# polarsignals/frostdb

Measured on AMD Instinct MI355X. Metric: rows/sec filter+group-by on 1B-row Prometheus Arrow (HBM-resident); achieved HBM GB/s vs peak, higher is better.
Workload: dtype f64; 1 GPU; headline: Prometheus schema, labels.code=='200' + SUM(value) GROUP BY labels.path; total_rows=1000000000, rows_per_gpu=1000000000, records_per_gpu=40, groups=1025, parallelism=1 GPU

## Files before the change

### frostdb_amd/csrc/fdb_capi.cpp

```cpp
#include <cstring>
#include <new>
#include <string>
#include <vector>

#include "fdb_codec.h"
#include "fdb_comm.h"
#include "fdb_context.h"
#include "fdb_dynamic.h"
#include "fdb_jit.h"
#include "fdb_mergepath.h"
#include "fdb_mergerec.h"
#include "fdb_plan.h"
#include "fdb_pqwrite_host.h"
#include "fdb_regex.h"
#include "fdb_sort.h"
#include "fdb_sortkey.h"
#include "fdb_take.h"

struct fdb_plan {
  std::unique_ptr<fdb::DynamicAggs> dyn;
  fdb_plan_desc main_desc;
  fdb::Plan plan;
  fdb_plan(const fdb_plan_desc* d, int dev)
      : dyn(fdb::DynamicAggs::wanted(d) ? new fdb::DynamicAggs(d, dev) : nullptr),
        main_desc(dyn ? dyn->main_desc() : (d ? *d : fdb_plan_desc())),
        plan(d ? &main_desc : nullptr, dev) {}
  explicit fdb_plan(const fdb::Plan& proto) : main_desc(), plan(proto, fdb::Plan::CloneTag()) {}
};
struct fdb_comm { std::unique_ptr<fdb::Comm> c; };
struct fdb_batch { std::unique_ptr<fdb::DeviceBatch> b; };
struct fdb_osync { fdb::OrderedSync s; fdb_osync(int32_t inputs, const fdb_order_col* order, int32_t n_order) : s(inputs, order, n_order) {} };
struct fdb_sampler { fdb::Sampler s; fdb_sampler(int64_t size, uint64_t seed, int device) : s(size, seed, device) {} };

namespace {
thread_local std::string g_last_error;

template <typename F>
int guard(fdb_plan* p, F&& f) {
  try {
    f();
    return FDB_OK;
  } catch (const fdb::Error& e) {
    if (p) p->plan.error = e.what(); else g_last_error = e.what();
    return e.code;
  } catch (const std::bad_alloc&) {
    if (p) p->plan.error = "out of host memory"; else g_last_error = "out of host memory";
    return FDB_ERR_OOM;
  } catch (const std::exception& e) {
    if (p) p->plan.error = e.what(); else g_last_error = e.what();
    return FDB_ERR_INVALID;
  } catch (...) {
    if (p) p->plan.error = "unknown error"; else g_last_error = "unknown error";
    return FDB_ERR_INVALID;
  }
}
void single_table_only(const fdb_plan* p) {
  if (p->dyn) throw fdb::Error(FDB_ERR_UNSUPPORTED, "not available for a plan with aggregations over a dynamic column set (merge such plans with fdb_plan_merge)");
}
}

namespace {
template <typename F>
int comm_guard(fdb_comm* c, F&& f) {
  try {
    f();
    return FDB_OK;
  } catch (const fdb::Error& e) {
    if (c && c->c) c->c->error = e.what();
    g_last_error = e.what();
    return e.code;
  } catch (const std::bad_alloc&) {
    g_last_error = "out of host memory";
    return FDB_ERR_OOM;
  } catch (const std::exception& e) {
    if (c && c->c) c->c->error = e.what();
    g_last_error = e.what();
    return FDB_ERR_INVALID;
  }
}
int wrap_all(std::vector<std::unique_ptr<fdb::Comm>>&& v, fdb_comm** out) {
  for (size_t i = 0; i < v.size(); i++) { out[i] = new fdb_comm(); out[i]->c = std::move(v[i]); }
  return FDB_OK;
}
}

namespace fdb { void widen_indices(const void* src, int width, uint32_t* dst, size_t n); void widen_indices_mapped(const void* src, int width, const uint32_t* table, size_t table_len, uint32_t* dst, size_t n); }

extern "C" {

const char* fdb_version(void) { return "frostdb_amd 0.1.0 (gfx950)"; }
const char* fdb_last_error(void) { return g_last_error.c_str(); }

int fdb_device_count(int* n_devices) {
  return guard(nullptr, [&] {
    int n = 0;
    hipError_t e = hipGetDeviceCount(&n);
    if (e != hipSuccess) { n = 0; (void)hipGetLastError(); }
    *n_devices = n;
  });
}

int fdb_plan_explain(const fdb_plan_desc* desc, char* buf, int64_t capacity, int64_t* needed) {
  return guard(nullptr, [&] {
    std::string s;
    if (fdb::DynamicAggs::wanted(desc)) {
      fdb::DynamicAggs dyn(desc, 0);
      const fdb_plan_desc md = dyn.main_desc();
      fdb::Plan plan(&md, 0, true);
      s = dyn.draw(plan);
    } else {
      fdb::Plan plan(desc, 0, true);
      s = plan.draw();
    }
    if (needed != nullptr) *needed = (int64_t)s.size() + 1;
    if (buf != nullptr && capacity > 0) {
      const size_t n = std::min((size_t)capacity - 1, s.size());
      std::memcpy(buf, s.data(), n);
      buf[n] = 0;
    }
  });
}

int fdb_selftest_widen(const void* src, int32_t width, uint32_t* dst, int64_t n) {
  return guard(nullptr, [&] {
    if ((width != 1 && width != 2 && width != 4 && width != -2 && width != -4 && width != -12 && width != -14) || n < 0 || ((src == nullptr || dst == nullptr) && n > 0))
      throw fdb::Error(FDB_ERR_INVALID, "widen: width 1, 2, 4 (bytes) or -2, -4 (bits) and non-null buffers");
    if (width == -12 || width == -14) {
      uint32_t table[16];
      for (uint32_t r = 0; r < 16; r++) table[r] = 3 * r + 5;
      fdb::widen_indices_mapped(src, width + 10, table, width == -12 ? 4 : 16, dst, (size_t)n);
      return;
    }
    fdb::widen_indices(src, width, dst, (size_t)n);
  });
}

int fdb_selftest_exact_sum(const double* x, int64_t n, double* out) {
  return guard(nullptr, [&] {
    if (n < 0 || out == nullptr || (n > 0 && x == nullptr)) throw fdb::Error(FDB_ERR_INVALID, "exact sum: n >= 0 and non-null buffers");
    long long limbs[FDB_EXACT_LIMBS] = {0};
    unsigned long long flags = 0;
    int64_t since = 0;
    for (int64_t i = 0; i < n; i++) {
      unsigned long long bits;
      std::memcpy(&bits, x + i, 8);
      int k; long long d0, d1, d2;
      const unsigned long long f = fdb_exact_split(bits, &k, &d0, &d1, &d2);
      if (f != 0ull) { flags |= f; continue; }
      limbs[k] += d0; limbs[k + 1] += d1; limbs[k + 2] += d2;
      if (++since == ((int64_t)1 << 30)) { fdb_exact_normalize(limbs); since = 0; }
    }
    const unsigned long long r = fdb_exact_round(limbs, flags);
    std::memcpy(out, &r, 8);
  });
}

int fdb_arrow_roundtrip(struct ArrowArray* batch, struct ArrowSchema* schema, struct ArrowArray* out, struct ArrowSchema* out_schema) {
  return guard(nullptr, [&] {
    if (out == nullptr || out_schema == nullptr) throw fdb::Error(FDB_ERR_INVALID, "null output");
    fdb::HostRecordView view;
    fdb::view_record(batch, schema, &view);
    fdb::roundtrip_record(view, out, out_schema);
  });
}

int fdb_read_ceiling(int device, int64_t bytes, int32_t reps, double* gb_per_s) {
  return guard(nullptr, [&] {
    if (gb_per_s == nullptr || bytes < (1 << 20) || reps < 1) throw fdb::Error(FDB_ERR_INVALID, "fdb_read_ceiling: bytes >= 1 MiB, reps >= 1");
    *gb_per_s = 0;
    bytes &= ~(int64_t)4095;
    if (hipSetDevice(device) != hipSuccess) throw fdb::Error(FDB_ERR_DEVICE, "hipSetDevice failed");
    void* buf = nullptr;
    unsigned long long* out = nullptr;
    hipEvent_t e0 = nullptr, e1 = nullptr;
    auto cleanup = [&] { if (buf) (void)hipFree(buf); if (out) (void)hipFree(out); if (e0) (void)hipEventDestroy(e0); if (e1) (void)hipEventDestroy(e1); };
    auto ck = [&](hipError_t e, const char* what) { if (e != hipSuccess) { cleanup(); throw fdb::Error(e == hipErrorOutOfMemory ? FDB_ERR_OOM : FDB_ERR_DEVICE, std::string(what) + ": " + hipGetErrorString(e)); } };
    ck(hipMalloc(&buf, (size_t)bytes), "hipMalloc");
    ck(hipMalloc((void**)&out, 64), "hipMalloc");
    ck(hipMemset(buf, 0, (size_t)bytes), "hipMemset");
    ck(hipEventCreate(&e0), "hipEventCreate");
    ck(hipEventCreate(&e1), "hipEventCreate");
    ck(fdb_launch_stream_read(buf, bytes, out, nullptr), "launch");
    float best = 0;
    for (int r = 0; r < reps; r++) {
      ck(hipEventRecord(e0, nullptr), "hipEventRecord");
      ck(fdb_launch_stream_read(buf, bytes, out, nullptr), "launch");
      ck(hipEventRecord(e1, nullptr), "hipEventRecord");
      ck(hipEventSynchronize(e1), "hipEventSynchronize");
      float ms = 0;
      ck(hipEventElapsedTime(&ms, e0, e1), "hipEventElapsedTime");
      if (ms > 0 && (best == 0 || ms < best)) best = ms;
    }
    cleanup();
    if (best > 0) *gb_per_s = (double)bytes / (best * 1e-3) / 1e9;
  });
}

int fdb_plan_create(const fdb_plan_desc* desc, int device, fdb_plan** out) {
  return guard(nullptr, [&] {
    if (out == nullptr) throw fdb::Error(FDB_ERR_INVALID, "null out pointer");
    if (desc != nullptr && desc->ordered != 0 && fdb::DynamicAggs::wanted(desc))
      throw fdb::Error(FDB_ERR_UNSUPPORTED, "OrderedAggregate over a dynamic column set is not supported");
    *out = new fdb_plan(desc, device);
  });
}

int fdb_plan_push(fdb_plan* plan, struct ArrowArray* batch, struct ArrowSchema* schema) {
  if (!plan) return FDB_ERR_INVALID;
  return guard(plan, [&] { if (plan->dyn) plan->dyn->push(plan->plan, batch, schema); else plan->plan.push(batch, schema); });
}

int fdb_plan_push_many(fdb_plan* plan, struct ArrowArray* const* batches, struct ArrowSchema* const* schemas, int32_t n, int32_t* n_pushed) {
  if (n_pushed) *n_pushed = 0;
  if (!plan || n < 0 || (n > 0 && (!batches || !schemas))) return FDB_ERR_INVALID;
  for (int32_t i = 0; i < n; i++) {
    const int rc = fdb_plan_push(plan, batches[i], schemas[i]);
// ... 785 lines not shown
```

### frostdb_amd/csrc/fdb_jit.cpp

```cpp
#include <hip/hip_runtime_api.h>
#include <hip/hiprtc.h>
#include <sys/stat.h>
#include <unistd.h>

#include <algorithm>
#include <chrono>
#include <atomic>
#include <cstdio>
#include <cstdlib>
#include <cstring>
#include <fstream>
#include <condition_variable>
#include <functional>
#include <memory>
#include <mutex>
#include <thread>
#include <sstream>
#include <string>
#include <unordered_map>
#include <vector>

#include "fdb_jit.h"
#include "../../include/frostdb_amd.h"

// ... 2 lines not shown
namespace {

const char* kKernelsHeader =
#include "fdb_kernels_h.inc"
    ;

const char* kPreamble = R"HIP(
typedef uint32_t u32x4 __attribute__((ext_vector_type(4)));
typedef unsigned long long u64x2 __attribute__((ext_vector_type(2)));
typedef uint32_t u32x2 __attribute__((ext_vector_type(2)));
#define G1 __attribute__((address_space(1)))
template <typename T> __device__ __forceinline__ const G1 T* as_global(const T* p) { return (const G1 T*)p; }
__device__ __forceinline__ long long f64_to_ordered(double d) { long long b = __double_as_longlong(d); return b ^ ((b >> 63) & 0x7FFFFFFFFFFFFFFFLL); }
// (a NaN contributes the identity of MIN / MAX, −0.0 counts as +0.0: see f64_minmax_key in fdb_kernels.hip)
__device__ __forceinline__ long long f64_minmax_key(double d, bool is_min) {
  d += 0.0;
  const long long k = f64_to_ordered(d);
  return d != d ? (is_min ? 0x7FFFFFFFFFFFFFFFLL : (-0x7FFFFFFFFFFFFFFFLL - 1)) : k;
}
// (FDB_LD_TEMPORAL: the kernel reads its columns twice — wide run records — so the first pass must leave them in the L2)
#ifdef FDB_LD_TEMPORAL
__device__ __forceinline__ u32x4 ld4(const void* base, uint32_t byte_off) {
  return *as_global(reinterpret_cast<const u32x4*>(reinterpret_cast<const char*>(base) + byte_off));
}
__device__ __forceinline__ u64x2 ld8(const void* base, uint32_t byte_off) {
  return *as_global(reinterpret_cast<const u64x2*>(reinterpret_cast<const char*>(base) + byte_off));
}
// (narrow-index caches, fdb_record.h: a lane's four indices at 1 / 2 bytes each — one 4- / 8-byte load, contiguous across the wave)
__device__ __forceinline__ uint32_t ld1raw(const void* base, uint32_t byte_off) {
  return *as_global(reinterpret_cast<const uint32_t*>(reinterpret_cast<const char*>(base) + byte_off));
}
__device__ __forceinline__ u32x2 ld2raw(const void* base, uint32_t byte_off) {
  return *as_global(reinterpret_cast<const u32x2*>(reinterpret_cast<const char*>(base) + byte_off));
}
#else
__device__ __forceinline__ uint32_t ld1raw(const void* base, uint32_t byte_off) {
  return __builtin_nontemporal_load(as_global(reinterpret_cast<const uint32_t*>(reinterpret_cast<const char*>(base) + byte_off)));
}
__device__ __forceinline__ u32x2 ld2raw(const void* base, uint32_t byte_off) {
  return __builtin_nontemporal_load(as_global(reinterpret_cast<const u32x2*>(reinterpret_cast<const char*>(base) + byte_off)));
}
__device__ __forceinline__ u32x4 ld4(const void* base, uint32_t byte_off) {
  return __builtin_nontemporal_load(as_global(reinterpret_cast<const u32x4*>(reinterpret_cast<const char*>(base) + byte_off)));
}
__device__ __forceinline__ u64x2 ld8(const void* base, uint32_t byte_off) {
  return __builtin_nontemporal_load(as_global(reinterpret_cast<const u64x2*>(reinterpret_cast<const char*>(base) + byte_off)));
}
#endif
// … unpacked into the register form the rest of the kernel consumes
__device__ __forceinline__ u32x4 ld1x4(const void* base, uint32_t byte_off) {
  const uint32_t v = ld1raw(base, byte_off);
  u32x4 r; r.x = v & 0xFFu; r.y = (v >> 8) & 0xFFu; r.z = (v >> 16) & 0xFFu; r.w = v >> 24;
  return r;
}
__device__ __forceinline__ u32x4 ld2x4(const void* base, uint32_t byte_off) {
  const u32x2 v = ld2raw(base, byte_off);
  u32x4 r; r.x = v.x & 0xFFFFu; r.y = v.x >> 16; r.z = v.y & 0xFFFFu; r.w = v.y >> 16;
  return r;
}
__device__ __forceinline__ uint32_t ldv(const uint8_t* bm, uint32_t byte_off, uint32_t shift) { return (as_global(bm)[byte_off] >> shift) & 0xFu; }
// dictionary truth table in a 64-bit immediate: 4 rows → 4-bit mask (NULL rows look up entry `null_at`)
__device__ __forceinline__ uint32_t leaf_bits(u32x4 idx, uint32_t valid, unsigned long long bits, uint32_t null_at) {
  const uint32_t i0 = (valid & 1u) ? idx.x : null_at, i1 = (valid & 2u) ? idx.y : null_at, i2 = (valid & 4u) ? idx.z : null_at, i3 = (valid & 8u) ? idx.w : null_at;
  return (uint32_t)((bits >> i0) & 1ull) | ((uint32_t)((bits >> i1) & 1ull) << 1) | ((uint32_t)((bits >> i2) & 1ull) << 2) | ((uint32_t)((bits >> i3) & 1ull) << 3);
}
template <typename LUT>
__device__ __forceinline__ uint32_t leaf_lut(u32x4 idx, uint32_t valid, LUT lut, uint32_t null_at) {
  const uint32_t i0 = (valid & 1u) ? idx.x : null_at, i1 = (valid & 2u) ? idx.y : null_at, i2 = (valid & 4u) ? idx.z : null_at, i3 = (valid & 8u) ? idx.w : null_at;
  return (uint32_t)lut[i0] | ((uint32_t)lut[i1] << 1) | ((uint32_t)lut[i2] << 2) | ((uint32_t)lut[i3] << 3);
}
// pre-aggregate arithmetic (project.go:163-399): Go int64 semantics — wrap-around, quotient truncated toward zero,
// MinInt64 / -1 wraps; a division by zero yields NULL, whose raw slot reads 0.
__device__ __forceinline__ long long i64_add(long long a, long long b) { return (long long)((unsigned long long)a + (unsigned long long)b); }
__device__ __forceinline__ long long i64_sub(long long a, long long b) { return (long long)((unsigned long long)a - (unsigned long long)b); }
__device__ __forceinline__ long long i64_mul(long long a, long long b) { return (long long)((unsigned long long)a * (unsigned long long)b); }
__device__ __forceinline__ long long i64_div(long long a, long long b) { return b == 0 ? 0 : b == -1 ? (long long)(0ull - (unsigned long long)a) : a / b; }
__device__ __forceinline__ long long u64_div(long long a, long long b) { return b == 0 ? 0 : (long long)((unsigned long long)a / (unsigned long long)b); }  // DivUint64s (project.go:379-395)
__device__ __forceinline__ double f64_div(double a, double b) { return b == 0.0 ? 0.0 : a / b; }
template <int OP, typename T> __device__ __forceinline__ bool cmp1(T a, T b) {
  return OP == 1 ? a == b : OP == 2 ? a != b : OP == 3 ? a < b : OP == 4 ? a <= b : OP == 5 ? a > b : a >= b;
}
template <int OP, typename T> __device__ __forceinline__ uint32_t cmp4(T a, T b, T c, T d, T lit, uint32_t valid) {
  return ((uint32_t)cmp1<OP, T>(a, lit) | ((uint32_t)cmp1<OP, T>(b, lit) << 1) | ((uint32_t)cmp1<OP, T>(c, lit) << 2) | ((uint32_t)cmp1<OP, T>(d, lit) << 3)) & valid;
}
)HIP";

struct KernelEntry {
  std::mutex m;
  std::condition_variable cv;
  bool ready = false;
  hipFunction_t fn = nullptr;
};
std::mutex g_mu;
std::unordered_map<std::string, std::shared_ptr<KernelEntry>> g_cache;
bool g_disabled = false;

uint64_t fnv(const std::string& s) {
  uint64_t h = 1469598103934665603ull;
  for (unsigned char c : s) { h ^= c; h *= 1099511628211ull; }
  return h;
}

std::string cache_dir() {
  std::string d;
  if (const char* e = std::getenv("FDB_JIT_CACHE")) d = e;
  else if (const char* x = std::getenv("XDG_CACHE_HOME"); x != nullptr && *x) d = std::string(x) + "/frostdb_amd";
  else if (const char* h = std::getenv("HOME"); h != nullptr && *h) { ::mkdir((std::string(h) + "/.cache").c_str(), 0700); d = std::string(h) + "/.cache/frostdb_amd"; }
  else d = "/tmp/frostdb_amd_jit_" + std::to_string((long)getuid());
  if (d.empty()) return "";
  (void)::mkdir(d.c_str(), 0700);
  struct stat st;
  if (::lstat(d.c_str(), &st) != 0 || !S_ISDIR(st.st_mode) || st.st_uid != getuid() || (st.st_mode & 077) != 0) {
    static bool warned = false;
    if (!warned) { warned = true; std::fprintf(stderr, "[frostdb_amd] JIT disk cache disabled: %s is not a private directory of this user\n", d.c_str()); }
    return "";
  }
  return d;
}

bool compile(const std::string& src, std::vector<char>* code, std::string* log) {
  hiprtcProgram prog;
  const char* hdr_names[] = {"fdb_kernels.h"};
  const char* hdr_src[] = {kKernelsHeader};
  if (hiprtcCreateProgram(&prog, src.c_str(), "fdb_plan_kernel.hip", 1, hdr_src, hdr_names) != HIPRTC_SUCCESS) { *log = "hiprtcCreateProgram failed"; return false; }
  const char* opts[] = {"--offload-arch=gfx950", "-O3", "-std=c++17", "-munsafe-fp-atomics", "-DFDB_DEVICE_ONLY=1"};
  const hiprtcResult r = hiprtcCompileProgram(prog, 5, opts);
  size_t n = 0;
  hiprtcGetProgramLogSize(prog, &n);
  if (n > 1) { log->resize(n); hiprtcGetProgramLog(prog, &(*log)[0]); }
  if (r != HIPRTC_SUCCESS) { hiprtcDestroyProgram(&prog); return false; }
  size_t sz = 0;
  hiprtcGetCodeSize(prog, &sz);
  code->resize(sz);
  hiprtcGetCode(prog, code->data());
  hiprtcDestroyProgram(&prog);
  return true;
}

template <typename F, typename V>
std::string expr_valid(const std::vector<JitExprNode>& ex, int root, F col, V colvalid);
template <typename F, typename V>
std::string expr_value(const std::vector<JitExprNode>& ex, int ni, F col, V colvalid) {
  const JitExprNode& n = ex[(size_t)ni];
  const bool f = n.type == FDB_T_F64;
  if (n.kind == 0) return f ? ("__longlong_as_double((long long)" + col(ni) + ")") : ("(long long)" + col(ni));
  if (n.kind == 1) return f ? ("__longlong_as_double(K_elit" + std::to_string(ni) + ")") : ("K_elit" + std::to_string(ni));
  if (n.kind == 7) return "(long long)" + col(ni);
  if (n.kind == 4) return "(double)(" + expr_value(ex, n.left, col, colvalid) + ")";
  if (n.kind == 5) return "(" + colvalid(n.left) + " ? 0ll : 1ll)";
  if (n.kind == 6)
    return "((" + expr_value(ex, n.op, col, colvalid) + " != 0ll) ? " + expr_value(ex, n.left, col, colvalid) + " : " + expr_value(ex, n.right, col, colvalid) + ")";
  std::string a = expr_value(ex, n.left, col, colvalid), b = expr_value(ex, n.right, col, colvalid);
  if (n.kind == 3) {
    if (n.op == FDB_OP_AND || n.op == FDB_OP_OR) return "((" + a + (n.op == FDB_OP_AND ? " & " : " | ") + b + ") & 1ll)";
    if (ex[(size_t)n.left].type != ex[(size_t)n.right].type) { a = "(double)" + a; b = "(double)" + b; }
    const char* op = n.op == FDB_OP_EQ ? " == " : n.op == FDB_OP_NOT_EQ ? " != " : n.op == FDB_OP_LT ? " < " : n.op == FDB_OP_LT_EQ ? " <= " : n.op == FDB_OP_GT ? " > " : " >= ";
    return "((" + expr_valid(ex, n.left, col, colvalid) + " && " + expr_valid(ex, n.right, col, colvalid) + " && (" + a + op + b + ")) ? 1ll : 0ll)";
  }
  if (f) {
    if (n.op == FDB_OP_DIV) return "f64_div(" + a + ", " + b + ")";
    return "(" + a + (n.op == FDB_OP_ADD ? " + " : n.op == FDB_OP_SUB ? " - " : " * ") + b + ")";
  }
  return std::string(n.op == FDB_OP_ADD ? "i64_add(" : n.op == FDB_OP_SUB ? "i64_sub(" : n.op == FDB_OP_MUL ? "i64_mul(" : n.type == FDB_T_U64 ? "u64_div(" : "i64_div(") + a + ", " + b + ")";
}
template <typename F, typename V>
std::string expr_valid(const std::vector<JitExprNode>& ex, int root, F col, V colvalid) {
  const JitExprNode& n = ex[(size_t)root];
  if (n.kind == 0) return colvalid(root);
  if (n.kind == 2 && n.op == FDB_OP_DIV) {
    const std::string d = expr_value(ex, n.right, col, colvalid);
    return n.type == FDB_T_F64 ? ("(" + d + " != 0.0)") : ("(" + d + " != 0)");
  }
  return "true";
}
inline std::string expr_bits(const std::vector<JitExprNode>& ex, int root, const std::string& v) {
  if (ex[(size_t)root].type == FDB_T_BOOL) return "(unsigned long long)(" + v + " + 1ll)";
  return ex[(size_t)root].type == FDB_T_F64 ? ("(unsigned long long)__double_as_longlong(" + v + ")") : ("(unsigned long long)" + v);
}

struct Gen {
  std::ostringstream o;
  const JitShape& s;
  explicit Gen(const JitShape& sh) : s(sh) {}

  static std::string reg(bool wide, bool late, int slot) { return std::string(late ? "l" : "e") + (wide ? "8_" : "4_") + std::to_string(slot); }

  void loads(bool late) {
    const int n4 = late ? s.n_l4 : s.n_c4, n8 = late ? s.n_l8 : s.n_c8;
    for (int i = 0; i < n4; i++) {
      const JitSlot& c = late ? s.l4[i] : s.c4[i];
      const std::string r = reg(false, late, i);
      if (c.has_values && c.width == 1) o << "    const u32x4 " << r << " = ld1x4(P_" << r << "_v + tile_off1, lane_off1);\n";
      else if (c.has_values && c.width == 2) o << "    const u32x4 " << r << " = ld2x4(P_" << r << "_v + tile_off2, lane_off2);\n";
      else if (c.has_values) o << "    const u32x4 " << r << " = ld4(P_" << r << "_v + tile_off4, lane_off4);\n";
      mask(c, r);
    }
    for (int i = 0; i < n8; i++) {
      const JitSlot& c = late ? s.l8[i] : s.c8[i];
      const std::string r = reg(true, late, i);
      if (c.has_values) {
        o << "    const u64x2 " << r << "a = ld8(P_" << r << "_v + tile_off8, lane_off8);\n";
        o << "    const u64x2 " << r << "b = ld8(P_" << r << "_v + tile_off8, lane_off8 + 16u);\n";
      }
      mask(c, r);
    }
  }

  bool live_mask = false;
  void mask(const JitSlot& c, const std::string& r) {
    const char* all = live_mask ? "live" : "0xFu";
    const char* cut = live_mask ? " & live" : "";
    if (c.has_validity == 1) o << "    const uint32_t " << r << "_m = ldv(P_" << r << "_b + tile_offb, lane_offb, lane_shb)" << cut << ";\n";
    else if (c.has_validity == 2) o << "    const uint32_t " << r << "_m = P_" << r << "_b != nullptr ? ldv(P_" << r << "_b + tile_offb, lane_offb, lane_shb)" << cut << " : " << all << ";\n";
    else o << "    const uint32_t " << r << "_m = " << all << ";\n";
  }

  std::string leaf_expr(int l) { return leaf_expr_of(s.leaves[l], l, reg(s.leaves[l].wide, false, s.leaves[l].slot)); }

  static std::string leaf_expr_of(const JitLeaf& L, int l, const std::string& r) {
    const std::string li = std::to_string(l);
    std::ostringstream e;
    switch (L.kind) {
      case FDB_LEAF_CONST: e << "(K_op" << li << " ? 0xFu : 0u)"; break;
      case FDB_LEAF_VALIDITY: e << "(K_op" << li << " ? " << r << "_m : (~" << r << "_m & 0xFu))"; break;
      case FDB_LEAF_DICT_BITS: e << "leaf_bits(" << r << ", " << r << "_m, (unsigned long long)K_lit" << li << ", K_len" << li << " - 1u)"; break;
      case FDB_LEAF_DICT_LUT:
        if (L.lut_in_lds) e << "leaf_lut(" << r << ", " << r << "_m, smem + K_lds" << li << ", K_len" << li << " - 1u)";
        else e << "leaf_lut(" << r << ", " << r << "_m, as_global(K_lut" << li << "), K_len" << li << " - 1u)";
        break;
      case FDB_LEAF_CMP_I64:
        e << "cmp4<" << L.op << ", long long>((long long)" << r << "a.x, (long long)" << r << "a.y, (long long)" << r << "b.x, (long long)" << r << "b.y, K_lit" << li << ", " << r << "_m)";
        break;
      case FDB_LEAF_CMP_U64:
        e << "cmp4<" << L.op << ", unsigned long long>(" << r << "a.x, " << r << "a.y, " << r << "b.x, " << r << "b.y, (unsigned long long)K_lit" << li << ", " << r << "_m)";
        break;
      case FDB_LEAF_CMP_F64:
        e << "cmp4<" << L.op << ", double>(__longlong_as_double((long long)" << r << "a.x), __longlong_as_double((long long)" << r << "a.y), __longlong_as_double((long long)"
          << r << "b.x), __longlong_as_double((long long)" << r << "b.y), __longlong_as_double(K_lit" << li << "), " << r << "_m)";
        break;
      case FDB_LEAF_CMP_I64_F64:
        e << "cmp4<" << L.op << ", double>((double)(long long)" << r << "a.x, (double)(long long)" << r << "a.y, (double)(long long)" << r << "b.x, (double)(long long)" << r
          << "b.y, __longlong_as_double(K_lit" << li << "), " << r << "_m)";
        break;
    }
    return e.str();
  }

  std::string filter_expr() {
    return filter_expr_of(s.code, [&](int l) { return leaf_expr(l); });
  }
  template <typename F>
  static std::string filter_expr_of(const std::vector<uint8_t>& code, F leaf) {
    std::vector<std::string> st;
    for (uint8_t c : code) {
      if (c < 0x80) { st.push_back(leaf(c)); continue; }
      const std::string b = st.back(); st.pop_back();
      const std::string a = st.back(); st.pop_back();
      st.push_back("(" + a + (c == FDB_CODE_AND ? " & " : " | ") + b + ")");
    }
    return st.empty() ? "0xFu" : st.back();
  }

  std::string source() {
    const int BLK = s.block;
    o << "#include \"fdb_kernels.h\"\n" << kPreamble;
    o << "extern \"C\" __global__ __launch_bounds__(" << BLK << ") void fdb_plan_kernel(const FdbScanArgs* __restrict__ parts, const int n_parts, const long long total_tiles, const FdbScanArgs c) {\n";
    o << "  extern __shared__ __align__(16) unsigned char smem[];\n  const uint32_t tid = threadIdx.x;\n  const uint32_t n_slots = c.n_slots;\n";
    o << "  if (c.fill_state != nullptr)  // (a fresh table: its identity fill rides on this launch, see FdbScanArgs)\n";
    o << "    for (uint32_t i = blockIdx.x * " << BLK << "u + tid; i < c.fill_words; i += gridDim.x * " << BLK << "u) c.fill_state[i] = c.fill_idents[i / c.fill_alloc];\n";
    o << "  const size_t TB = (((size_t)n_slots * 4 + 15) & ~(size_t)15) + (size_t)n_slots * 8 * (size_t)c.n_aggs;\n  (void)TB;\n";
    const std::string tbl = s.wave_tables ? "smem + c.lds_lut_bytes + (size_t)(tid >> 6) * TB" : "smem + c.lds_lut_bytes";
    o << "  uint32_t* l_cnt = reinterpret_cast<uint32_t*>(" << tbl << ");\n";
    o << "  unsigned long long* l_acc = reinterpret_cast<unsigned long long*>(" << tbl << " + (((size_t)n_slots * 4 + 15) & ~(size_t)15));\n";
    if (s.lds_acc) {
      const std::string i0 = s.wave_tables ? "(tid & 63u)" : "tid", step = s.wave_tables ? "64" : std::to_string(BLK);
      o << "  for (uint32_t i = " << i0 << "; i < n_slots; i += " << step << ") l_cnt[i] = 0;\n";
      for (size_t j = 0; j < s.aggs.size(); j++) {
        const JitAgg& A = s.aggs[j];
        if (A.func == FDB_AGG_COUNT) continue;
        const char* ident = A.func == FDB_AGG_MIN ? "0x7FFFFFFFFFFFFFFFull" : A.func == FDB_AGG_MAX ? "0x8000000000000000ull" : "0ull";
        o << "  for (uint32_t i = " << i0 << "; i < n_slots; i += " << step << ") l_acc[(size_t)" << j << " * n_slots + i] = " << ident << ";\n";
      }
    }
    if (s.cache) {
      o << "  const uint32_t CS = (uint32_t)c.cache_slots;\n";
      o << "  uint32_t* t_tag = reinterpret_cast<uint32_t*>(smem + c.lds_lut_bytes);\n  uint32_t* t_cnt = t_tag + CS;\n";
      o << "  unsigned long long* t_acc = reinterpret_cast<unsigned long long*>(t_cnt + CS);\n";
      o << "  for (uint32_t i = tid; i < CS; i += " << BLK << ") { t_tag[i] = 0u; t_cnt[i] = 0u; }\n";
      for (size_t j = 0; j < s.aggs.size(); j++) {
        const JitAgg& A = s.aggs[j];
        if (A.func == FDB_AGG_COUNT) continue;
        const char* ident = A.func == FDB_AGG_MIN ? "0x7FFFFFFFFFFFFFFFull" : A.func == FDB_AGG_MAX ? "0x8000000000000000ull" : "0ull";
        o << "  for (uint32_t i = tid; i < CS; i += " << BLK << ") t_acc[(size_t)" << j << " * CS + i] = " << ident << ";\n";
      }
    }
    auto decl_slots = [&](bool late) {
      const int n4 = late ? s.n_l4 : s.n_c4, n8 = late ? s.n_l8 : s.n_c8;
      for (int i = 0; i < n4; i++) o << "  const char* P_" << reg(false, late, i) << "_v = nullptr; const uint8_t* P_" << reg(false, late, i) << "_b = nullptr;\n";
      for (int i = 0; i < n8; i++) o << "  const char* P_" << reg(true, late, i) << "_v = nullptr; const uint8_t* P_" << reg(true, late, i) << "_b = nullptr;\n";
    };
    decl_slots(false); decl_slots(true);
    for (size_t l = 0; l < s.leaves.size(); l++)
      o << "  long long K_lit" << l << " = 0; uint32_t K_len" << l << " = 1, K_lds" << l << " = 0; int K_op" << l << " = 0; const uint8_t* K_lut" << l << " = nullptr;\n";
    for (size_t g = 0; g < s.gcols.size(); g++) o << "  uint32_t G_lds" << g << " = 0, G_stride" << g << " = 0; const uint32_t* G_lut" << g << " = nullptr;\n";
    for (size_t i = 0; i < s.exprs.size(); i++) if (s.exprs[i].kind == 1) o << "  long long K_elit" << i << " = 0;\n";
    for (int t = 0; t < s.reg_slots; t++) {
      o << "  unsigned long long R_cnt" << t << " = 0ull;\n";
      for (size_t j = 0; j < s.aggs.size(); j++) {
        const JitAgg& A = s.aggs[j];
        if (A.func == FDB_AGG_COUNT) continue;
        if (A.func == FDB_AGG_SUM && A.type == FDB_T_F64) o << "  double R_a" << j << "_" << t << " = 0.0;\n";
        else if (A.func == FDB_AGG_SUM) o << "  unsigned long long R_a" << j << "_" << t << " = 0ull;\n";
        else o << "  long long R_a" << j << "_" << t << " = " << (A.func == FDB_AGG_MIN ? "0x7FFFFFFFFFFFFFFFLL" : "(-0x7FFFFFFFFFFFFFFFLL - 1)") << ";\n";
      }
    }
    o << "  long long n_rows = 0, tile_begin = 0, tile_end = 0; int part = -1, lut_class = -1;\n";
    o << "  const uint32_t lane_off4 = tid * 16u, lane_off8 = tid * 32u, lane_offb = tid >> 1, lane_shb = (tid & 1u) * 4u;\n";
    o << "  const uint32_t lane_off1 = tid * 4u, lane_off2 = tid * 8u; (void)lane_off1; (void)lane_off2;\n";
    o << "  for (long long tile = blockIdx.x; tile < total_tiles; tile += gridDim.x) {\n";
    o << "    if (part < 0 || tile >= tile_end) {\n      int np = part < 0 ? 0 : part;\n      while (np + 1 < n_parts && tile >= parts[np].tile_end) np++;\n      part = np;\n";
    o << "      const FdbScanArgs& pa = parts[part];\n      n_rows = pa.n_rows; tile_begin = pa.tile_begin; tile_end = pa.tile_end;\n";
    auto set_slots = [&](bool late) {
      const int n4 = late ? s.n_l4 : s.n_c4, n8 = late ? s.n_l8 : s.n_c8;
      const char* p4 = late ? "l4" : "c4"; const char* p8 = late ? "l8" : "c8";
      for (int i = 0; i < n4; i++)
        o << "      P_" << reg(false, late, i) << "_v = (const char*)pa." << p4 << "[" << i << "].values; P_" << reg(false, late, i) << "_b = pa." << p4 << "[" << i << "].validity;\n";
      for (int i = 0; i < n8; i++)
        o << "      P_" << reg(true, late, i) << "_v = (const char*)pa." << p8 << "[" << i << "].values; P_" << reg(true, late, i) << "_b = pa." << p8 << "[" << i << "].validity;\n";
    };
    set_slots(false); set_slots(true);
    for (size_t l = 0; l < s.leaves.size(); l++)
      o << "      K_lit" << l << " = pa.leaves[" << l << "].lit; K_len" << l << " = pa.leaves[" << l << "].lut_len; K_lds" << l << " = pa.leaves[" << l << "].lut_lds; K_op" << l
        << " = pa.leaves[" << l << "].op; K_lut" << l << " = pa.leaves[" << l << "].lut;\n";
    for (size_t g = 0; g < s.gcols.size(); g++)
      o << "      G_lds" << g << " = pa.gcols[" << g << "].lut_lds; G_stride" << g << " = pa.gcols[" << g << "].stride; G_lut" << g << " = pa.gcols[" << g << "].lut;\n";
    for (size_t i = 0; i < s.exprs.size(); i++) if (s.exprs[i].kind == 1) o << "      K_elit" << i << " = pa.expr[" << i << "].lit;\n";
    o << "      if (pa.lut_class != lut_class) {\n        lut_class = pa.lut_class;\n        __syncthreads();\n";
    for (size_t l = 0; l < s.leaves.size(); l++)
      if (s.leaves[l].kind == FDB_LEAF_DICT_LUT && s.leaves[l].lut_in_lds)
        o << "        for (uint32_t i = tid; i < K_len" << l << "; i += " << BLK << ") smem[K_lds" << l << " + i] = as_global(K_lut" << l << ")[i];\n";
    for (size_t g = 0; g < s.gcols.size(); g++)
      if (s.gcols[g].lut_in_lds)
        o << "        for (uint32_t i = tid; i < pa.gcols[" << g << "].lut_len; i += " << BLK << ") reinterpret_cast<uint32_t*>(smem + G_lds" << g << ")[i] = as_global(G_lut" << g << ")[i];\n";
    o << "        __syncthreads();\n      }\n    }\n";
    o << "    const long long r0 = (tile - tile_begin) * " << BLK * 4 << "LL;\n";
    o << "    const long long left = n_rows - r0 - (long long)tid * 4;\n    if (left <= 0) continue;\n";
    o << "    const size_t tile_off4 = (size_t)r0 * 4, tile_off8 = (size_t)r0 * 8, tile_offb = (size_t)(r0 >> 3);\n";
    o << "    const size_t tile_off1 = (size_t)r0, tile_off2 = (size_t)r0 * 2; (void)tile_off1; (void)tile_off2;\n";
    o << "    const uint32_t live = left >= 4 ? 0xFu : ((1u << (int)left) - 1u);\n";
    live_mask = true;
    loads(false);
    o << "    uint32_t sel = live;\n";
    if (!s.code.empty()) o << "    sel &= " << filter_expr() << ";\n";
    {
      std::vector<int> seen;
      for (const JitExprNode& e : s.exprs)
        if (e.kind == 7 && std::find(seen.begin(), seen.end(), e.slot) == seen.end()) { seen.push_back(e.slot); o << "    const uint32_t PM" << e.slot << " = " << leaf_expr(e.slot) << "; (void)PM" << e.slot << ";\n"; }
    }
    const bool uniform_fold = s.uniform_fold && s.lds_acc && !s.cache && s.reg_slots == 0 && !s.wave_tables && !s.two_phase && !s.gcols.empty();
    if (uniform_fold) o << "    const unsigned long long has = __ballot(sel != 0u);\n    if (has == 0ull) continue;\n";
    else o << "    if (sel == 0u) continue;\n";
    loads(true);
    o << "    uint32_t gid0 = 0, gid1 = 0, gid2 = 0, gid3 = 0;\n";
    for (size_t g = 0; g < s.gcols.size(); g++) {
      const JitGroup& G = s.gcols[g];
      const std::string r = reg(false, s.two_phase, G.slot);
      const std::string lut = G.lut_in_lds ? ("reinterpret_cast<const uint32_t*>(smem + G_lds" + std::to_string(g) + ")") : ("as_global(G_lut" + std::to_string(g) + ")");
      const char* comp[4] = {"x", "y", "z", "w"};
      for (int k = 0; k < 4; k++)
        o << "    gid" << k << " += ((" << r << "_m >> " << k << ") & 1u ? " << lut << "[" << r << "." << comp[k] << "] : 0u) * G_stride" << g << ";\n";
    }
    if (uniform_fold) {
      auto raw_of = [&](size_t j, int k) {
        const JitAgg& A = s.aggs[j];
        const std::string comp = std::string(k < 2 ? "a" : "b") + (k % 2 == 0 ? ".x" : ".y");
        if (A.expr != 0) {
          auto col = [&](int ni) -> std::string { if (s.exprs[(size_t)ni].kind == 7) return "((PM" + std::to_string(s.exprs[(size_t)ni].slot) + " >> " + std::to_string(k) + ") & 1u)"; return reg(true, s.two_phase, s.exprs[(size_t)ni].slot) + comp; };
          auto colvalid = [&](int ni) { return "((" + reg(true, s.two_phase, s.exprs[(size_t)ni].slot) + "_m >> " + std::to_string(k) + ") & 1u)"; };
          return "(" + expr_valid(s.exprs, A.expr - 1, col, colvalid) + " ? " + expr_bits(s.exprs, A.expr - 1, expr_value(s.exprs, A.expr - 1, col, colvalid)) + " : 0ull)";
        }
        const std::string r = reg(true, s.two_phase, A.slot);
        return "((" + r + "_m >> " + std::to_string(k) + ") & 1u ? " + r + comp + " : c.aggs[" + std::to_string(j) + "].null_value)";
      };
      o << "    {\n      const uint32_t my_first = (sel & 1u) ? gid0 : (sel & 2u) ? gid1 : (sel & 4u) ? gid2 : gid3;\n";
      o << "      const uint32_t g0 = (uint32_t)__builtin_amdgcn_readlane((int)my_first, __builtin_ctzll(has));\n";
      o << "      if (__ballot(sel != 0u && my_first != g0) == 0ull && __ballot(1) == ~0ull &&\n";
      o << "          __ballot(((sel & 1u) && gid0 != g0) || ((sel & 2u) && gid1 != g0) || ((sel & 4u) && gid2 != g0) || ((sel & 8u) && gid3 != g0)) == 0ull) {\n";
      o << "        uint32_t u_cnt = (uint32_t)__builtin_popcount(sel);\n";
      for (size_t j = 0; j < s.aggs.size(); j++) {
        const JitAgg& A = s.aggs[j];
        if (A.func == FDB_AGG_COUNT) continue;
        const std::string v = "u" + std::to_string(j);
        if (A.func == FDB_AGG_SUM && A.type == FDB_T_F64) {
          o << "        double " << v << " = 0.0;\n";
          for (int k = 0; k < 4; k++) o << "        if ((sel >> " << k << ") & 1u) " << v << " += __longlong_as_double((long long)" << raw_of(j, k) << ");\n";
        } else if (A.func == FDB_AGG_SUM) {
          o << "        unsigned long long " << v << " = 0ull;\n";
          for (int k = 0; k < 4; k++) o << "        if ((sel >> " << k << ") & 1u) " << v << " += " << raw_of(j, k) << ";\n";
        } else {
          o << "        long long " << v << " = " << (A.func == FDB_AGG_MIN ? "0x7FFFFFFFFFFFFFFFLL" : "(-0x7FFFFFFFFFFFFFFFLL - 1)") << ";\n";
          for (int k = 0; k < 4; k++) {
            const std::string key = A.type == FDB_T_F64 ? ("f64_minmax_key(__longlong_as_double((long long)" + raw_of(j, k) + "), " + (A.func == FDB_AGG_MIN ? "true" : "false") + ")") : ("(long long)" + raw_of(j, k));
            o << "        if ((sel >> " << k << ") & 1u) { const long long y = " << key << "; " << v << " = " << (A.func == FDB_AGG_MIN ? "y < " : "y > ") << v << " ? y : " << v << "; }\n";
          }
        }
      }
      o << "#pragma unroll\n        for (int sh = 32; sh > 0; sh >>= 1) {\n          u_cnt += (uint32_t)__shfl_xor((int)u_cnt, sh, 64);\n";
      for (size_t j = 0; j < s.aggs.size(); j++) {
        const JitAgg& A = s.aggs[j];
        if (A.func == FDB_AGG_COUNT) continue;
        const std::string v = "u" + std::to_string(j);
        if (A.func == FDB_AGG_SUM && A.type == FDB_T_F64) o << "          " << v << " += __shfl_xor(" << v << ", sh, 64);\n";
        else if (A.func == FDB_AGG_SUM) o << "          " << v << " += (unsigned long long)__shfl_xor((long long)" << v << ", sh, 64);\n";
        else o << "          { const long long y = __shfl_xor(" << v << ", sh, 64); " << v << " = " << (A.func == FDB_AGG_MIN ? "y < " : "y > ") << v << " ? y : " << v << "; }\n";
      }
      o << "        }\n        if ((tid & 63u) == 0u) {\n";
      if (s.need_count) o << "          atomicAdd(&l_cnt[g0], u_cnt);\n";
      else o << "          l_cnt[g0] = 1u;\n";
      for (size_t j = 0; j < s.aggs.size(); j++) {
        const JitAgg& A = s.aggs[j];
        if (A.func == FDB_AGG_COUNT) continue;
        const std::string v = "u" + std::to_string(j);
        const std::string acc = "(l_acc + (size_t)" + std::to_string(j) + " * n_slots + g0)";
        if (A.func == FDB_AGG_SUM && A.type == FDB_T_F64) o << "          atomicAdd(reinterpret_cast<double*>" << acc << ", " << v << ");\n";
        else if (A.func == FDB_AGG_SUM) o << "          atomicAdd(" << acc << ", " << v << ");\n";
        else o << "          " << (A.func == FDB_AGG_MIN ? "atomicMin" : "atomicMax") << "(reinterpret_cast<long long*>" << acc << ", " << v << ");\n";
      }
      o << "        }\n        continue;\n      }\n    }\n";
    }
    for (int k = 0; k < 4 && s.reg_slots > 0; k++) {
      const std::string comp = std::string(k < 2 ? "a" : "b") + (k % 2 == 0 ? ".x" : ".y");
      o << "    {\n      const bool on = (sel >> " << k << ") & 1u;\n";
      std::vector<std::string> val(s.aggs.size());
      for (size_t j = 0; j < s.aggs.size(); j++) {
        const JitAgg& A = s.aggs[j];
        if (A.func == FDB_AGG_COUNT) continue;
        std::string raw;
        if (A.expr != 0) {
          auto col = [&](int ni) -> std::string { if (s.exprs[(size_t)ni].kind == 7) return "((PM" + std::to_string(s.exprs[(size_t)ni].slot) + " >> " + std::to_string(k) + ") & 1u)"; return reg(true, s.two_phase, s.exprs[(size_t)ni].slot) + comp; };
          auto colvalid = [&](int ni) { return "((" + reg(true, s.two_phase, s.exprs[(size_t)ni].slot) + "_m >> " + std::to_string(k) + ") & 1u)"; };
          raw = "(" + expr_valid(s.exprs, A.expr - 1, col, colvalid) + " ? " + expr_bits(s.exprs, A.expr - 1, expr_value(s.exprs, A.expr - 1, col, colvalid)) + " : 0ull)";
        } else {
          const std::string r = reg(true, s.two_phase, A.slot);
          raw = "((" + r + "_m >> " + std::to_string(k) + ") & 1u ? " + r + comp + " : c.aggs[" + std::to_string(j) + "].null_value)";
        }
        const std::string v = "v" + std::to_string(j);
        if (A.func == FDB_AGG_SUM && A.type == FDB_T_F64) o << "      const double " << v << " = __longlong_as_double((long long)" << raw << ");\n";
        else if (A.func == FDB_AGG_SUM) o << "      const unsigned long long " << v << " = " << raw << ";\n";
        else o << "      const long long " << v << " = " << (A.type == FDB_T_F64 ? ("f64_minmax_key(__longlong_as_double((long long)" + raw + "), " + (A.func == FDB_AGG_MIN ? "true" : "false") + ")") : ("(long long)" + raw)) << ";\n";
        val[j] = v;
      }
      for (int t = 0; t < s.reg_slots; t++) {
        const std::string m = s.reg_slots == 1 ? std::string("on") : ("(on && gid" + std::to_string(k) + " == " + std::to_string(t) + "u)");
        o << "      R_cnt" << t << " += " << m << " ? 1ull : 0ull;\n";
        for (size_t j = 0; j < s.aggs.size(); j++) {
          const JitAgg& A = s.aggs[j];
          if (A.func == FDB_AGG_COUNT) continue;
          const std::string acc = "R_a" + std::to_string(j) + "_" + std::to_string(t);
          if (A.func == FDB_AGG_SUM && A.type == FDB_T_F64) o << "      " << acc << " += " << m << " ? " << val[j] << " : 0.0;\n";
          else if (A.func == FDB_AGG_SUM) o << "      " << acc << " += " << m << " ? " << val[j] << " : 0ull;\n";
          else if (A.func == FDB_AGG_MIN) o << "      " << acc << " = (" << m << " && " << val[j] << " < " << acc << ") ? " << val[j] << " : " << acc << ";\n";
          else o << "      " << acc << " = (" << m << " && " << val[j] << " > " << acc << ") ? " << val[j] << " : " << acc << ";\n";
        }
      }
      o << "    }\n";
    }
    for (int k = 0; k < 4 && s.reg_slots == 0; k++) {
      const std::string gidk = "gid" + std::to_string(k);
      o << "    if ((sel >> " << k << ") & 1u) {\n";
      if (s.cache) {
        o << "      const uint32_t ch = ((gid" << k << " * 0x9E3779B1u) >> 12) & (CS - 1u);\n";
        o << "      uint32_t tg = t_tag[ch];\n      if (tg == 0u) { tg = atomicCAS(&t_tag[ch], 0u, gid" << k << " + 1u); if (tg == 0u) tg = gid" << k << " + 1u; }\n";
        o << "      const bool cached = tg == gid" << k << " + 1u;\n";
        o << "      if (cached) atomicAdd(&t_cnt[ch], 1u);\n";
        if (s.need_count) o << "      else atomicAdd(&c.cnt[gid" << k << "], 1ull);\n";
        else o << "      else c.cnt[gid" << k << "] = 1ull;\n";
      } else if (s.lds_acc) {
        if (s.need_count) o << "      atomicAdd(&l_cnt[" << gidk << "], 1u);\n";
        else o << "      l_cnt[" << gidk << "] = 1u;\n";
      } else {
        o << "      atomicAdd(&c.cnt[gid" << k << "], 1ull);\n";
      }
      for (size_t j = 0; j < s.aggs.size(); j++) {
        const JitAgg& A = s.aggs[j];
        if (A.func == FDB_AGG_COUNT) continue;
        const std::string comp = std::string(k < 2 ? "a" : "b") + (k % 2 == 0 ? ".x" : ".y");
        std::string raw;
        if (A.expr != 0) {
          auto col = [&](int ni) -> std::string { if (s.exprs[(size_t)ni].kind == 7) return "((PM" + std::to_string(s.exprs[(size_t)ni].slot) + " >> " + std::to_string(k) + ") & 1u)"; return reg(true, s.two_phase, s.exprs[(size_t)ni].slot) + comp; };
          auto colvalid = [&](int ni) { return "((" + reg(true, s.two_phase, s.exprs[(size_t)ni].slot) + "_m >> " + std::to_string(k) + ") & 1u)"; };
          raw = "(" + expr_valid(s.exprs, A.expr - 1, col, colvalid) + " ? " + expr_bits(s.exprs, A.expr - 1, expr_value(s.exprs, A.expr - 1, col, colvalid)) + " : 0ull)";
        } else {
          const std::string r = reg(true, s.two_phase, A.slot);
          raw = "((" + r + "_m >> " + std::to_string(k) + ") & 1u ? " + r + comp + " : c.aggs[" + std::to_string(j) + "].null_value)";
        }
        const std::string gacc = "(c.aggs[" + std::to_string(j) + "].acc + gid" + std::to_string(k) + ")";
        const std::string acc = s.lds_acc ? ("(l_acc + (size_t)" + std::to_string(j) + " * n_slots + " + gidk + ")") : gacc;
        auto emit = [&](const std::string& where, const char* ind) {
          if (A.func == FDB_AGG_SUM) {
            if (A.type == FDB_T_F64) o << ind << "atomicAdd(reinterpret_cast<double*>" << where << ", __longlong_as_double((long long)" << raw << "));\n";
            else o << ind << "atomicAdd(" << where << ", " << raw << ");\n";
          } else {
            const std::string key = A.type == FDB_T_F64 ? ("f64_minmax_key(__longlong_as_double((long long)" + raw + "), " + (A.func == FDB_AGG_MIN ? "true" : "false") + ")") : ("(long long)" + raw);
            o << ind << (A.func == FDB_AGG_MIN ? "atomicMin" : "atomicMax") << "(reinterpret_cast<long long*>" << where << ", " << key << ");\n";
          }
        };
        if (s.cache) {
          o << "      if (cached) {\n";
          emit("(t_acc + (size_t)" + std::to_string(j) + " * CS + ch)", "        ");
          o << "      } else {\n";
          emit(gacc, "        ");
          o << "      }\n";
        } else {
          emit(acc, "      ");
        }
      }
      o << "    }\n";
    }
    o << "  }\n";
    if (s.reg_slots > 0) {
      o << "  for (int sh = 32; sh > 0; sh >>= 1) {\n";
      for (int t = 0; t < s.reg_slots; t++) {
        o << "    R_cnt" << t << " += (unsigned long long)__shfl_xor((long long)R_cnt" << t << ", sh, 64);\n";
        for (size_t j = 0; j < s.aggs.size(); j++) {
          const JitAgg& A = s.aggs[j];
          if (A.func == FDB_AGG_COUNT) continue;
          const std::string acc = "R_a" + std::to_string(j) + "_" + std::to_string(t);
          if (A.func == FDB_AGG_SUM && A.type == FDB_T_F64) o << "    " << acc << " += __shfl_xor(" << acc << ", sh, 64);\n";
          else if (A.func == FDB_AGG_SUM) o << "    " << acc << " += (unsigned long long)__shfl_xor((long long)" << acc << ", sh, 64);\n";
          else if (A.func == FDB_AGG_MIN) o << "    { const long long y = __shfl_xor(" << acc << ", sh, 64); " << acc << " = y < " << acc << " ? y : " << acc << "; }\n";
          else o << "    { const long long y = __shfl_xor(" << acc << ", sh, 64); " << acc << " = y > " << acc << " ? y : " << acc << "; }\n";
        }
      }
      o << "  }\n  if ((tid & 63u) == 0u) {\n";
      for (int t = 0; t < s.reg_slots; t++) {
        o << "    if (R_cnt" << t << " != 0ull) {\n";
        if (s.lds_acc) o << "      atomicAdd(&l_cnt[" << t << "], (uint32_t)(R_cnt" << t << " > 0xFFFFFFFFull ? 0xFFFFFFFFull : R_cnt" << t << "));\n";
        else o << "      atomicAdd(&c.cnt[" << t << "], R_cnt" << t << ");\n";
        for (size_t j = 0; j < s.aggs.size(); j++) {
          const JitAgg& A = s.aggs[j];
          if (A.func == FDB_AGG_COUNT) continue;
          const std::string v = "R_a" + std::to_string(j) + "_" + std::to_string(t);
          const std::string acc = s.lds_acc ? ("(l_acc + (size_t)" + std::to_string(j) + " * n_slots + " + std::to_string(t) + ")") : ("(c.aggs[" + std::to_string(j) + "].acc + " + std::to_string(t) + ")");
          if (A.func == FDB_AGG_SUM && A.type == FDB_T_F64) o << "      atomicAdd(reinterpret_cast<double*>" << acc << ", " << v << ");\n";
          else if (A.func == FDB_AGG_SUM) o << "      atomicAdd(" << acc << ", " << v << ");\n";
          else o << "      " << (A.func == FDB_AGG_MIN ? "atomicMin" : "atomicMax") << "(reinterpret_cast<long long*>" << acc << ", " << v << ");\n";
        }
        o << "    }\n";
      }
      o << "  }\n";
    }
    if (s.cache) {
      o << "  __syncthreads();\n  for (uint32_t i = tid; i < CS; i += " << BLK << ") {\n    const uint32_t tg = t_tag[i];\n    if (tg == 0u) continue;\n    const uint32_t g = tg - 1u;\n";
      if (s.need_count) o << "    atomicAdd(&c.cnt[g], (unsigned long long)t_cnt[i]);\n";
      else o << "    c.cnt[g] = 1ull;\n";
      for (size_t j = 0; j < s.aggs.size(); j++) {
        const JitAgg& A = s.aggs[j];
        if (A.func == FDB_AGG_COUNT) continue;
        const std::string v = "t_acc[(size_t)" + std::to_string(j) + " * CS + i]";
        const std::string dst = "c.aggs[" + std::to_string(j) + "].acc + g";
        if (A.func == FDB_AGG_SUM && A.type == FDB_T_F64) o << "    atomicAdd(reinterpret_cast<double*>(" << dst << "), __longlong_as_double((long long)" << v << "));\n";
        else if (A.func == FDB_AGG_SUM) o << "    atomicAdd(" << dst << ", " << v << ");\n";
        else o << "    " << (A.func == FDB_AGG_MIN ? "atomicMin" : "atomicMax") << "(reinterpret_cast<long long*>(" << dst << "), (long long)" << v << ");\n";
      }
      o << "  }\n";
    }
    if (s.lds_acc && s.wave_tables) {
      o << "  __syncthreads();\n  {\n    unsigned long long* out = c.partials + (size_t)blockIdx.x * (size_t)(1 + c.n_aggs) * n_slots;\n";
      o << "    const unsigned char* t0 = smem + c.lds_lut_bytes;\n";
      o << "    for (uint32_t i = tid; i < n_slots; i += " << BLK << ") {\n      unsigned long long n = 0;\n";
      o << "      for (int w = 0; w < " << BLK / 64 << "; w++) n += reinterpret_cast<const uint32_t*>(t0 + (size_t)w * TB)[i];\n      out[i] = n;\n";
      for (size_t j = 0; j < s.aggs.size(); j++) {
        const JitAgg& A = s.aggs[j];
        if (A.func == FDB_AGG_COUNT) continue;
        const std::string at = "reinterpret_cast<const unsigned long long*>(t0 + (size_t)w * TB + (((size_t)n_slots * 4 + 15) & ~(size_t)15))[(size_t)" + std::to_string(j) + " * n_slots + i]";
        if (A.func == FDB_AGG_SUM && A.type == FDB_T_F64) {
          o << "      { double v = 0.0; for (int w = 0; w < " << BLK / 64 << "; w++) v += __longlong_as_double((long long)" << at << "); out[(size_t)" << (1 + j) << " * n_slots + i] = (unsigned long long)__double_as_longlong(v); }\n";
        } else if (A.func == FDB_AGG_SUM) {
          o << "      { unsigned long long v = 0; for (int w = 0; w < " << BLK / 64 << "; w++) v += " << at << "; out[(size_t)" << (1 + j) << " * n_slots + i] = v; }\n";
        } else {
          o << "      { long long v = " << (A.func == FDB_AGG_MIN ? "0x7FFFFFFFFFFFFFFFLL" : "(-0x7FFFFFFFFFFFFFFFLL - 1)") << "; for (int w = 0; w < " << BLK / 64 << "; w++) { const long long y = (long long)" << at
            << "; v = " << (A.func == FDB_AGG_MIN ? "y < v" : "y > v") << " ? y : v; } out[(size_t)" << (1 + j) << " * n_slots + i] = (unsigned long long)v; }\n";
        }
      }
      o << "    }\n  }\n";
    } else if (s.lds_acc) {
      o << "  __syncthreads();\n";
      o << "  if (c.partials != nullptr) {\n    unsigned long long* out = c.partials + (size_t)blockIdx.x * (size_t)(1 + c.n_aggs) * n_slots;\n";
      o << "    for (uint32_t i = tid; i < n_slots; i += " << BLK << ") out[i] = (unsigned long long)l_cnt[i];\n";
      for (size_t j = 0; j < s.aggs.size(); j++)
        if (s.aggs[j].func != FDB_AGG_COUNT)
          o << "    for (uint32_t i = tid; i < n_slots; i += " << BLK << ") out[(size_t)" << (1 + j) << " * n_slots + i] = l_acc[(size_t)" << j << " * n_slots + i];\n";
      o << "  } else {\n    for (uint32_t i = tid; i < n_slots; i += " << BLK << ") {\n      const uint32_t n_sel = l_cnt[i];\n      if (n_sel == 0) continue;\n";
      o << "      atomicAdd(&c.cnt[i], (unsigned long long)n_sel);\n";
      for (size_t j = 0; j < s.aggs.size(); j++) {
        const JitAgg& A = s.aggs[j];
        if (A.func == FDB_AGG_COUNT) continue;
        const std::string v = "l_acc[(size_t)" + std::to_string(j) + " * n_slots + i]";
        const std::string dst = "c.aggs[" + std::to_string(j) + "].acc + i";
        if (A.func == FDB_AGG_SUM && A.type == FDB_T_F64) o << "      atomicAdd(reinterpret_cast<double*>(" << dst << "), __longlong_as_double((long long)" << v << "));\n";
// ... 719 lines not shown
      o << "        u32x4* stage = reinterpret_cast<u32x4*>(smem + a.lds_lut_bytes + (size_t)wv * " << FDB_RUN_WAVE_LDS << ");\n";
      o << "        const uint32_t n_act = (uint32_t)__popcll(act2), my_act = (uint32_t)__popcll(act2 & lt);\n";
      o << "        const bool sw = rp + n_w > " << FDB_RUN_CHUNK << "u;\n";
      o << "        if (sw || (rp - ps) + n_w > " << FDB_RUN_STAGE << "u) {\n";
      o << "          u32x4* out = reinterpret_cast<u32x4*>(h.runs.tuples) + (size_t)(rb + ps) * 3;\n";
      o << "          for (uint32_t q = my_act; q < (rp - ps) * 3u; q += n_act) out[q] = stage[q];\n";
      o << "          __builtin_amdgcn_wave_barrier();\n          ps = rp;\n        }\n";
      o << "        if (sw) {\n          uint32_t nc = 0u;\n          if (wl2 == first2) nc = atomicAdd(h.runs.chunk_cursor, 1u);\n          rb = (uint32_t)__shfl((int)nc, first2, 64) * " << FDB_RUN_CHUNK
        << "u; rp = 0u; ps = 0u;\n        }\n";
      o << "        const uint32_t base = rb + rp, sbase = rp - ps;\n        __builtin_amdgcn_wave_barrier();\n";
      o << "        if (wl2 == first2) { s_runs[wv * 4] = rb; s_runs[wv * 4 + 1] = rp + n_w; s_runs[wv * 4 + 2] = ps; *reinterpret_cast<uint2*>(h.runs.dir + ((size_t)tile * 4 + wv) * 2) = make_uint2(base, n_w); }\n";
      for (int k = 0; k < 4; k++) {
        o << "        if (sel & " << (1 << k) << "u) {\n          const uint32_t at = sbase + before + (uint32_t)__builtin_popcount(sel & " << ((1 << k) - 1) << "u);\n";
        o << "          stage[at * 3] = ta_" << k << "; stage[at * 3 + 1] = tb_" << k << ";\n";
        o << "          *reinterpret_cast<u64x2*>(stage + at * 3 + 2) = u64x2{cnt_" << k << ", "
          << (has_val ? (f64v ? "(unsigned long long)__double_as_longlong(v0_" + std::to_string(k) + ")" : "(unsigned long long)v0_" + std::to_string(k)) : std::string("0ull")) << "};\n        }\n";
      }
      o << "        __builtin_amdgcn_wave_barrier();\n      }\n    }\n    continue;\n";
    }
    for (int k = 0; k < 4; k++) o << "    uint64_t slot_" << k << " = h1_" << k << " & h.mask; unsigned long long p_" << k << " = 0, q_" << k << " = 0;\n";
    for (int k = 0; k < 4; k++)
      o << "    if ((sel >> " << k << ") & 1u) { const u64x2 pq = *as_global(reinterpret_cast<const u64x2*>(h.table + slot_" << k << " * (uint64_t)ew)); p_" << k << " = pq.x; q_" << k
        << " = pq.y; }\n";
    o << "    uint32_t ins_mask = 0;\n";
    for (int k = 0; k < 4; k++) o << "    unsigned long long c_" << k << " = ~0ull;\n";
    for (int k = 0; k < 4; k++)
      o << "    if (((sel >> " << k << ") & 1u) && p_" << k << " == 0ull) c_" << k << " = atomicCAS(h.table + slot_" << k << " * (uint64_t)ew, 0ull, h1_" << k << ");\n";
    for (int k = 0; k < 4; k++)
      o << "    if (c_" << k << " == 0ull) { __hip_atomic_store(h.table + slot_" << k << " * (uint64_t)ew + 1, h2_" << k << ", __ATOMIC_RELAXED, __HIP_MEMORY_SCOPE_AGENT); ins_mask |= " << (1 << k) << "u; }\n";
    for (int k = 0; k < 4; k++) {
      o << "    if ((sel >> " << k << ") & 1u) {\n";
      o << "      if (c_" << k << " != 0ull && !(p_" << k << " == h1_" << k << " && q_" << k << " == h2_" << k << ")) { bool ins; slot_" << k << " = hash_find_or_insert(h.table, h.mask, ew, h1_" << k << ", h2_" << k
        << ", ins); if (ins) ins_mask |= " << (1 << k) << "u; }\n";
      o << "      unsigned long long* e = h.table + slot_" << k << " * (uint64_t)ew;\n";
      if (s.need_count) o << "      atomicAdd(e + 2, cnt_" << k << ");\n";
      for (size_t j = 0; j < s.aggs.size(); j++) {
        const JitAgg& A = s.aggs[j];
        if (A.func == FDB_AGG_COUNT || exact_agg(j)) continue;
        const std::string v = "v" + std::to_string(j) + "_" + std::to_string(k);
        const std::string acc = "(e + " + std::to_string(3 + j) + ")";
        if (A.func == FDB_AGG_SUM && A.type == FDB_T_F64) o << "      atomicAdd(reinterpret_cast<double*>" << acc << ", " << v << ");\n";
        else if (A.func == FDB_AGG_SUM) o << "      atomicAdd(" << acc << ", " << v << ");\n";
        else o << "      " << (A.func == FDB_AGG_MIN ? "atomicMin" : "atomicMax") << "(reinterpret_cast<long long*>" << acc << ", " << v << ");\n";
      }
      o << "    }\n";
    }
    emit_tuple_stores(false);
    if (s.exact) {
      o << "    x_slot0 = slot_0; x_slot1 = slot_1; x_slot2 = slot_2; x_slot3 = slot_3; x_sel = sel;\n";
      o << "    } while (0);\n";
      for (size_t j = 0; j < s.aggs.size(); j++) {
        if (!exact_agg(j)) continue;
        o << "    {\n      unsigned long long* XL = a.aggs[" << j << "].acc;\n";
        for (int k = 0; k < 4; k++) o << "      fdb_exact_add_wave(XL, x_slot" << k << ", xv" << j << "_" << k << ", ((x_sel >> " << k << ") & 1u) != 0u);\n";
        o << "    }\n";
      }
    }
    o << "  }\n";
    if (wide || medium) {
      o << "  {  // the runs that still wait in the waves' stages\n    const int wv = (int)(tid >> 6), wl2 = (int)(tid & 63u);\n    __builtin_amdgcn_wave_barrier();\n";
      o << "    const uint32_t rb = s_runs[wv * 4], rp = s_runs[wv * 4 + 1], ps = s_runs[wv * 4 + 2], RQ = " << (medium ? std::to_string(FDB_RUN_MEDIUM_BYTES / 16) + "u" : std::string("(uint32_t)h.runs.run_words >> 2")) << ";\n";
      o << "    if (rp != " << FDB_RUN_CHUNK << "u || ps != " << FDB_RUN_CHUNK << "u) {\n";
      o << "      const u32x4* stage = reinterpret_cast<const u32x4*>(smem + a.lds_lut_bytes + (size_t)wv * " << FDB_RUN_WAVE_LDS << ");\n";
      o << "      u32x4* out = reinterpret_cast<u32x4*>(h.runs.tuples) + (size_t)(rb + ps) * RQ;\n";
      o << "      for (uint32_t q = (uint32_t)wl2; q < (rp - ps) * RQ; q += 64u) out[q] = stage[q];\n    }\n  }\n";
    }
    if (narrow) {
      o << "  {  // the runs that still wait in the waves' stages\n    const int wv = (int)(tid >> 6), wl2 = (int)(tid & 63u);\n    __builtin_amdgcn_wave_barrier();\n";
      o << "    const uint32_t rb = s_runs[wv * 4], rp = s_runs[wv * 4 + 1], ps = s_runs[wv * 4 + 2];\n";
      o << "    if (rp != " << FDB_RUN_CHUNK << "u || ps != " << FDB_RUN_CHUNK << "u) {\n";
      o << "      const u32x4* stage = reinterpret_cast<const u32x4*>(smem + a.lds_lut_bytes + (size_t)wv * " << FDB_RUN_WAVE_LDS << ");\n";
      o << "      u32x4* out = reinterpret_cast<u32x4*>(h.runs.tuples) + (size_t)(rb + ps) * 3;\n";
      o << "      for (uint32_t q = (uint32_t)wl2; q < (rp - ps) * 3u; q += 64u) out[q] = stage[q];\n    }\n  }\n";
    }
    o << "  __syncthreads();\n  if (tid == 0 && s_new != 0) atomicAdd(h.n_groups, (unsigned long long)s_new);\n}\n";
    return o.str();
  }
};

}

std::string JitShape::key(bool with_validity) const {
  std::ostringstream k;
  k << "b" << block << "l" << lds_acc << "c" << need_count << "t" << two_phase << "r" << reg_slots << "h" << cache << (wave_tables ? "w" : "") << (uniform_fold ? "u" : "") << "|";
  auto slots = [&](const JitSlot* p, int n) { for (int i = 0; i < n; i++) { k << (p[i].has_values ? 'v' : '-') << (with_validity ? p[i].has_validity : 0); if (p[i].width != 4) k << 'w' << p[i].width; } k << '|'; };
  slots(c4, n_c4); slots(c8, n_c8); slots(l4, n_l4); slots(l8, n_l8);
  for (const JitLeaf& L : leaves) k << L.kind << ',' << L.slot << ',' << L.wide << ',' << (L.kind >= FDB_LEAF_CMP_I64 && L.kind <= FDB_LEAF_CMP_I64_F64 ? L.op : 0) << ',' << L.lut_in_lds << ';';
  k << '|';
  for (uint8_t c : code) k << (int)c << ',';
  k << '|';
  for (const JitGroup& G : gcols) k << G.slot << ',' << G.lut_in_lds << ';';
  k << '|';
  for (const JitAgg& A : aggs) k << A.func << ',' << A.type << ',' << A.slot << ',' << A.expr << ';';
  k << '|';
  for (const JitExprNode& e : exprs) k << e.kind << ',' << e.op << ',' << e.left << ',' << e.right << ',' << e.slot << ',' << e.type << ';';
  return k.str();
}

std::string jit_source(const JitShape& shape) { return Gen(shape).source(); }

JitShape jit_shape(const FdbScanArgs& a, bool two_phase, int block) {
  JitShape s;
  s.block = block;
  s.lds_acc = a.lds_acc != 0;
  s.need_count = a.need_count != 0;
  s.two_phase = two_phase;
  s.n_c4 = a.n_c4; s.n_c8 = a.n_c8;
  s.n_l4 = two_phase ? a.n_l4 : 0; s.n_l8 = two_phase ? a.n_l8 : 0;
  auto slots = [](JitSlot* dst, const FdbColSlot* src, int n) {
    for (int i = 0; i < n; i++) { dst[i].has_values = src[i].values != nullptr; dst[i].has_validity = src[i].validity != nullptr ? 1 : 0; }
  };
  slots(s.c4, a.c4, s.n_c4); slots(s.c8, a.c8, s.n_c8); slots(s.l4, a.l4, s.n_l4); slots(s.l8, a.l8, s.n_l8);
  for (int i = 0; i < s.n_c4; i++) s.c4[i].width = a.w4[i] == 1 || a.w4[i] == 2 ? a.w4[i] : 4;
  for (int i = 0; i < s.n_l4; i++) s.l4[i].width = a.wl4[i] == 1 || a.wl4[i] == 2 ? a.wl4[i] : 4;
  for (int l = 0; l < a.n_leaves; l++) {
    const FdbLeaf& L = a.leaves[l];
    s.leaves.push_back({L.kind, L.slot, L.wide, L.op, L.kind == FDB_LEAF_DICT_LUT && L.lut_lds != FDB_NO_LDS});
  }
  s.code.assign(a.code, a.code + a.n_code);
  for (int g = 0; g < a.n_gcols; g++) s.gcols.push_back({a.gcols[g].slot, a.gcols[g].lut_lds != FDB_NO_LDS});
  for (int j = 0; j < a.n_aggs; j++) s.aggs.push_back({a.aggs[j].func, a.aggs[j].type, a.aggs[j].slot, a.aggs[j].expr});
  for (int i = 0; i < a.n_expr; i++) s.exprs.push_back({a.expr[i].kind, a.expr[i].op, a.expr[i].left, a.expr[i].right, a.expr[i].slot, a.expr[i].type});
  s.cache = !s.lds_acc && a.cache_slots > 0;
  return s;
}

bool jit_shape_merge(JitShape* into, const JitShape& other) {
  if (into->key(false) != other.key(false)) return false;
  auto slots = [](JitSlot* a, const JitSlot* b, int n) { for (int i = 0; i < n; i++) if (a[i].has_validity != b[i].has_validity) a[i].has_validity = 2; };
  slots(into->c4, other.c4, into->n_c4); slots(into->c8, other.c8, into->n_c8); slots(into->l4, other.l4, into->n_l4); slots(into->l8, other.l8, into->n_l8);
  return true;
}

bool jit_shape_merge_args(JitShape* into, const FdbScanArgs& a, const FdbScanArgs& b, bool two_phase) {
  if (a.lds_acc != b.lds_acc || a.need_count != b.need_count || a.n_c4 != b.n_c4 || a.n_c8 != b.n_c8) return false;
  if (two_phase && (a.n_l4 != b.n_l4 || a.n_l8 != b.n_l8)) return false;
  if ((a.lds_acc == 0 && a.cache_slots > 0) != (b.lds_acc == 0 && b.cache_slots > 0)) return false;
  auto values_same = [](const FdbColSlot* x, const FdbColSlot* y, int n) { for (int i = 0; i < n; i++) if ((x[i].values != nullptr) != (y[i].values != nullptr)) return false; return true; };
  if (!values_same(a.c4, b.c4, a.n_c4) || !values_same(a.c8, b.c8, a.n_c8)) return false;
  if (two_phase && (!values_same(a.l4, b.l4, a.n_l4) || !values_same(a.l8, b.l8, a.n_l8))) return false;
  if (std::memcmp(a.w4, b.w4, sizeof a.w4) != 0 || (two_phase && std::memcmp(a.wl4, b.wl4, sizeof a.wl4) != 0)) return false;
  if (a.n_leaves != b.n_leaves || a.n_code != b.n_code || a.n_gcols != b.n_gcols || a.n_aggs != b.n_aggs || a.n_expr != b.n_expr) return false;
  for (int l = 0; l < a.n_leaves; l++) {
    const FdbLeaf& x = a.leaves[l]; const FdbLeaf& y = b.leaves[l];
    if (x.kind != y.kind || x.slot != y.slot || x.wide != y.wide) return false;
    if (x.kind >= FDB_LEAF_CMP_I64 && x.kind <= FDB_LEAF_CMP_I64_F64 && x.op != y.op) return false;
    if ((x.kind == FDB_LEAF_DICT_LUT && x.lut_lds != FDB_NO_LDS) != (y.kind == FDB_LEAF_DICT_LUT && y.lut_lds != FDB_NO_LDS)) return false;
  }
  if (std::memcmp(a.code, b.code, (size_t)a.n_code) != 0) return false;
  for (int g = 0; g < a.n_gcols; g++)
    if (a.gcols[g].slot != b.gcols[g].slot || (a.gcols[g].lut_lds != FDB_NO_LDS) != (b.gcols[g].lut_lds != FDB_NO_LDS)) return false;
  for (int j = 0; j < a.n_aggs; j++)
    if (a.aggs[j].func != b.aggs[j].func || a.aggs[j].type != b.aggs[j].type || a.aggs[j].slot != b.aggs[j].slot || a.aggs[j].expr != b.aggs[j].expr) return false;
  for (int i = 0; i < a.n_expr; i++) {
    const auto& x = a.expr[i]; const auto& y = b.expr[i];
    if (x.kind != y.kind || x.op != y.op || x.left != y.left || x.right != y.right || x.slot != y.slot || x.type != y.type) return false;
  }
  auto merge = [](JitSlot* s, const FdbColSlot* y, int n) { for (int i = 0; i < n; i++) if (s[i].has_validity != (y[i].validity != nullptr ? 1 : 0)) s[i].has_validity = 2; };
  merge(into->c4, b.c4, into->n_c4); merge(into->c8, b.c8, into->n_c8); merge(into->l4, b.l4, into->n_l4); merge(into->l8, b.l8, into->n_l8);
  return true;
}

int jit_blocks_per_cu(hipFunction_t fn, int block, size_t lds_bytes) {
  int occ = 0;
  if (hipModuleOccupancyMaxActiveBlocksPerMultiprocessor(&occ, fn, block, lds_bytes) != hipSuccess || occ < 1) { (void)hipGetLastError(); occ = 1; }
  if (occ > 2048 / block) occ = 2048 / block;
  return occ;
}

namespace {
std::atomic<int64_t> g_stat_compiled{0}, g_stat_compile_us{0}, g_stat_disk_loads{0};

hipFunction_t build_kernel(KernelEntry* entry, const std::string& kernel_name_s, const std::string& src) {
  const char* kernel_name = kernel_name_s.c_str();
  struct Publish {
    KernelEntry* e; hipFunction_t fn = nullptr;
    ~Publish() { { std::lock_guard<std::mutex> lk(e->m); e->fn = fn; e->ready = true; } e->cv.notify_all(); }
  } publish{entry};
  std::vector<char> code;
  char name[64];
  std::snprintf(name, sizeof name, "/k_%016llx_%zu.hsaco", (unsigned long long)(fnv(src) ^ (fnv(kKernelsHeader) * 31)), src.size());
  const std::string dir = cache_dir();
  const std::string path = dir.empty() ? std::string() : dir + name;
  bool from_disk = false;
  if (!path.empty()) {
    std::ifstream f(path, std::ios::binary);
    if (f) code.assign(std::istreambuf_iterator<char>(f), std::istreambuf_iterator<char>());
    from_disk = !code.empty();
  }
  auto load = [&](hipFunction_t* fn) {
    hipModule_t mod = nullptr;
    *fn = nullptr;
    if (hipModuleLoadData(&mod, code.data()) == hipSuccess && hipModuleGetFunction(fn, mod, kernel_name) == hipSuccess) return true;
    (void)hipGetLastError();
    *fn = nullptr;
    return false;
  };
// ... 117 lines not shown
std::string jit_project_source(const JitShape& shape) { return Gen(shape).project_source(); }
hipFunction_t jit_project_get(const JitShape& shape) {
  std::string roots;
  for (int r : shape.proj_roots) roots += std::to_string(r) + ",";
  return get_kernel("project|" + shape.key() + "|r" + roots, "fdb_project_kernel", [&] { return jit_project_source(shape); });
}
hipError_t jit_project_launch(hipFunction_t fn, const FdbScanArgs* d_parts, int n_parts, int64_t total_tiles, int grid, size_t lds_bytes, const FdbProjectPart* d_outs,
                              unsigned long long* d_nulls, hipStream_t stream) {
  long long tt = total_tiles;
  void* args[] = {(void*)&d_parts, (void*)&n_parts, (void*)&tt, (void*)&d_outs, (void*)&d_nulls};
  return hipModuleLaunchKernel(fn, (unsigned)grid, 1, 1, 256u, 1, 1, (unsigned)lds_bytes, stream, args, nullptr);
}

void jit_stats(int64_t* n_compiled, double* compile_ms, int64_t* n_disk_loads) {
  if (n_compiled) *n_compiled = g_stat_compiled.load();
  if (compile_ms) *compile_ms = (double)g_stat_compile_us.load() / 1000.0;
  if (n_disk_loads) *n_disk_loads = g_stat_disk_loads.load();
}

JitDeferScope::JitDeferScope(bool may_defer) : prev_(t_may_defer) { t_may_defer = may_defer; }
JitDeferScope::~JitDeferScope() { t_may_defer = prev_; }

hipFunction_t jit_get(const JitShape& shape) {
  return get_kernel(shape.key(), "fdb_plan_kernel", [&] { return jit_source(shape); });
}

std::string JitHashShape::key() const {
  std::ostringstream k;
  k << "c" << need_count << (runs == 1 ? "R" : runs == 2 ? "W" : runs == 3 ? "M" : "") << (exact ? "X" : "") << "|";
  for (const JitHashCol& C : cols) k << C.kind << (C.has_validity ? 'n' : '-') << (C.lut_identity ? 'i' : C.lut_in_lds ? 'l' : 'g') << (C.kind == 2 ? std::to_string(C.expr_root) : std::string());
  k << '|';
  for (size_t l = 0; l < leaves.size(); l++) {
    const JitLeaf& L = leaves[l];
    k << L.kind << ',' << L.wide << ',' << (L.kind >= FDB_LEAF_CMP_I64 && L.kind <= FDB_LEAF_CMP_I64_F64 ? L.op : 0) << ',' << L.lut_in_lds << ',' << leaf_validity[l] << ';';
  }
  k << '|';
  for (uint8_t c : code) k << (int)c << ',';
  k << '|';
  for (size_t j = 0; j < aggs.size(); j++) k << aggs[j].func << ',' << aggs[j].type << ',' << agg_validity[j] << ',' << aggs[j].expr << ';';
  k << '|' << n_expr_cols << '|';
  for (const JitExprNode& e : exprs) k << e.kind << ',' << e.op << ',' << e.left << ',' << e.right << ',' << e.slot << ',' << e.type << ';';
  return k.str();
}

JitHashShape jit_hash_shape(const FdbHashArgs& h, const FdbHashCol* hcols) {
  JitHashShape s;
  const FdbScanArgs& a = h.base;
  for (int c = 0; c < h.n_hcols; c++)
    s.cols.push_back({hcols[c].kind, hcols[c].validity != nullptr, hcols[c].kind == 0 && hcols[c].lut_lds != FDB_NO_LDS, hcols[c].kind == 2 ? hcols[c].src_word : -1,
                      hcols[c].kind == 0 && hcols[c].lut == nullptr});
  for (int i = 0; i < a.n_expr; i++) s.exprs.push_back({a.expr[i].kind, a.expr[i].op, a.expr[i].left, a.expr[i].right, a.expr[i].slot, a.expr[i].type});
  s.n_expr_cols = a.n_l8;
  s.need_count = a.need_count != 0;
  s.runs = h.runs.tuples == nullptr ? 0 : h.runs.run_words == 0 ? 1 : h.runs.run_words == FDB_RUN_MEDIUM_WORDS ? 3 : 2;
  for (int l = 0; l < a.n_leaves; l++) {
    const FdbLeaf& L = a.leaves[l];
    const bool wide = L.kind >= FDB_LEAF_CMP_I64 && L.kind <= FDB_LEAF_CMP_I64_F64;
    s.leaves.push_back({L.kind, 0, wide ? 1 : 0, L.op, L.kind == FDB_LEAF_DICT_LUT && L.lut_lds != FDB_NO_LDS});
    s.leaf_validity.push_back(L.validity != nullptr);
  }
  s.code.assign(a.code, a.code + a.n_code);
  for (int j = 0; j < a.n_aggs; j++) {
    s.aggs.push_back({a.aggs[j].func, a.aggs[j].type, -1, a.aggs[j].expr});
    s.agg_validity.push_back(a.aggs[j].validity != nullptr);
    if (a.aggs[j].func == FDB_AGG_SUM && a.aggs[j].type == FDB_T_F64 && a.aggs[j].acc != nullptr) s.exact = true;
  }
  return s;
}

std::string jit_hash_source(const JitHashShape& shape) { return HashGen(shape).source(); }

hipFunction_t jit_hash_get(const JitHashShape& shape) {
  return get_kernel(shape.key(), "fdb_hash_kernel", [&] { return jit_hash_source(shape); });
}

hipError_t jit_hash_launch(hipFunction_t fn, const FdbHashArgs& args, int grid, size_t lds_bytes, hipStream_t stream) {
  void* kargs[] = {(void*)&args};
  return hipModuleLaunchKernel(fn, (unsigned)grid, 1, 1, 256, 1, 1, (unsigned)lds_bytes, stream, kargs, nullptr);
}

hipFunction_t jit_select(JitShape shape, size_t lds_bytes, int row_bytes, int* block_out, int* blocks_per_cu_out) {
  int waves = row_bytes > 0 ? (65536 / (64 * 4)) / row_bytes : 16;
  waves = std::max(8, std::min(32, waves));
  const int block = waves % 8 == 0 ? 512 : 256;
  shape.block = block;
  hipFunction_t fn = jit_get(shape);
  if (fn == nullptr) return nullptr;
  const int fit = jit_blocks_per_cu(fn, block, lds_bytes);
  *block_out = block;
  *blocks_per_cu_out = std::max(1, std::min(fit, (waves + block / 128) / (block / 64)));
  if (std::getenv("FDB_JIT_DEBUG"))
    std::fprintf(stderr, "[frostdb_amd] plan kernel %s: %d B/row, %zu B LDS -> %d-thread workgroups, %d per CU (%d fit)\n", shape.key().c_str(), row_bytes,
                 lds_bytes, block, *blocks_per_cu_out, fit);
  return fn;
}

hipError_t jit_launch(hipFunction_t fn, const FdbScanArgs* d_parts, int n_parts, int64_t total_tiles, const FdbScanArgs& common, int grid, int block,
                      size_t lds_bytes, hipStream_t stream) {
  long long tt = total_tiles;
  void* args[] = {(void*)&d_parts, (void*)&n_parts, (void*)&tt, (void*)&common};
  return hipModuleLaunchKernel(fn, (unsigned)grid, 1, 1, (unsigned)block, 1, 1, (unsigned)lds_bytes, stream, args, nullptr);
}

}
```

### frostdb_amd/csrc/fdb_jit.h

```cpp
#pragma once
#include <cstdlib>

#include <hip/hip_runtime_api.h>

#include <cstdint>
#include <string>
#include <vector>

#include "fdb_kernels.h"

namespace fdb {

struct JitSlot { bool has_values = false; int has_validity = 0; int width = 4; };
struct JitLeaf { int kind = 0, slot = -1, wide = 0, op = 0; bool lut_in_lds = false; };
struct JitGroup { int slot = -1; bool lut_in_lds = false; };
struct JitAgg { int func = 0, type = 0, slot = -1; int expr = 0; };
struct JitExprNode { int kind = 0, op = 0, left = -1, right = -1, slot = -1, type = 0; };

struct JitShape {
  int block = 512;
  bool lds_acc = true, need_count = false, two_phase = false;
  int n_c4 = 0, n_c8 = 0, n_l4 = 0, n_l8 = 0;
  JitSlot c4[FDB_ARG_C4], c8[FDB_ARG_C8], l4[FDB_ARG_L4], l8[FDB_ARG_L8];
  std::vector<JitLeaf> leaves;
  std::vector<uint8_t> code;
  std::vector<JitGroup> gcols;
  std::vector<JitAgg> aggs;
  std::vector<JitExprNode> exprs;
  int reg_slots = 0;
  bool cache = false;
  bool wave_tables = false;
  bool uniform_fold = true;
  int fuse4 = 0, fuse8 = 0;
  std::vector<int> proj_roots;
  std::string key(bool with_validity = true) const;
};

struct JitHashCol { int kind = 0; bool has_validity = false, lut_in_lds = false; int expr_root = -1; bool lut_identity = false; };
struct JitHashShape {
  std::vector<JitHashCol> cols;
  std::vector<JitLeaf> leaves;
  std::vector<bool> leaf_validity;
  std::vector<uint8_t> code;
  std::vector<JitAgg> aggs;
  std::vector<bool> agg_validity;
  std::vector<JitExprNode> exprs;
  int n_expr_cols = 0;
  bool need_count = true;
  int runs = 0;
  bool exact = false;
  std::string key() const;
};
JitHashShape jit_hash_shape(const FdbHashArgs& args, const FdbHashCol* hcols);
std::string jit_hash_source(const JitHashShape& shape);
hipFunction_t jit_hash_get(const JitHashShape& shape);
hipError_t jit_hash_launch(hipFunction_t fn, const FdbHashArgs& args, int grid, size_t lds_bytes, hipStream_t stream);

JitShape jit_shape(const FdbScanArgs& a, bool two_phase, int block);
bool jit_shape_merge(JitShape* into, const JitShape& other);
bool jit_shape_merge_args(JitShape* into, const FdbScanArgs& a, const FdbScanArgs& b, bool two_phase);
int jit_blocks_per_cu(hipFunction_t fn, int block, size_t lds_bytes);

void jit_stats(int64_t* n_compiled, double* compile_ms, int64_t* n_disk_loads);

std::string jit_flags_source(const JitShape& shape);
hipFunction_t jit_flags_get(const JitShape& shape);
hipError_t jit_flags_launch(hipFunction_t fn, const FdbScanArgs* d_parts, int n_parts, int64_t total_super_tiles, const FdbScanArgs& common, int grid, size_t lds_bytes,
                            uint32_t* masks, uint32_t* tile_counts, hipStream_t stream);

std::string jit_select_source(const JitShape& shape);
hipFunction_t jit_select_kernel_get(const JitShape& shape);
size_t jit_select_stage_bytes(const JitShape& shape);
int jit_select_block();
hipError_t jit_select_launch(hipFunction_t fn, const FdbScanArgs* d_parts, int n_parts, int64_t total_super_tiles, const FdbScanArgs& common, int grid, size_t lds_bytes,
                             uint32_t* masks, uint32_t* offsets, const FdbSelectArgs& sel, hipStream_t stream);

std::string jit_project_source(const JitShape& shape);
hipFunction_t jit_project_get(const JitShape& shape);
hipError_t jit_project_launch(hipFunction_t fn, const FdbScanArgs* d_parts, int n_parts, int64_t total_tiles, int grid, size_t lds_bytes, const FdbProjectPart* d_outs,
                              unsigned long long* d_nulls, hipStream_t stream);

std::string jit_source(const JitShape& shape);
class JitDeferScope {
 public:
  explicit JitDeferScope(bool may_defer);
  ~JitDeferScope();
  JitDeferScope(const JitDeferScope&) = delete;
  JitDeferScope& operator=(const JitDeferScope&) = delete;
 private:
  bool prev_;
};
hipFunction_t jit_get(const JitShape& shape);
hipFunction_t jit_select(JitShape shape, size_t lds_bytes, int row_bytes, int* block_out, int* blocks_per_cu_out);
hipError_t jit_launch(hipFunction_t fn, const FdbScanArgs* d_parts, int n_parts, int64_t total_tiles, const FdbScanArgs& common, int grid, int block,
                      size_t lds_bytes, hipStream_t stream);

}
```

### frostdb_amd/csrc/fdb_kernels.hip

```cpp
#include <hip/hip_runtime.h>

#define FDB_DEVICE_HELPERS 1
#include <cstdlib>
#include <cstring>

#include "fdb_kernels.h"

namespace {

constexpr int OP_EQ = 1, OP_NOT_EQ = 2, OP_LT = 3, OP_LT_EQ = 4, OP_GT = 5, OP_GT_EQ = 6;
constexpr int AGG_SUM = 1, AGG_MIN = 2, AGG_MAX = 3, AGG_COUNT = 4;

__device__ __forceinline__ long long f64_to_ordered(double d) {
  long long b = __double_as_longlong(d);
  return b ^ ((b >> 63) & 0x7FFFFFFFFFFFFFFFLL);
}
__device__ __forceinline__ long long f64_minmax_key(double d, bool is_min) {
  d += 0.0;
  const long long k = f64_to_ordered(d);
  return d != d ? (is_min ? FDB_I64_MAX : FDB_I64_MIN) : k;
}

typedef uint32_t u32x4 __attribute__((ext_vector_type(4)));
typedef unsigned long long u64x2 __attribute__((ext_vector_type(2)));

#define FDB_GLOBAL __attribute__((address_space(1)))
template <typename T>
__device__ __forceinline__ const FDB_GLOBAL T* as_global(const T* p) {
  return (const FDB_GLOBAL T*)p;
}

template <int R>
__device__ __forceinline__ void load_u32(const uint32_t* __restrict__ p, uint32_t (&v)[R]) {
  if (R == 1) { v[0] = __builtin_nontemporal_load(as_global(p)); return; }
#pragma unroll
  for (int j = 0; j < R / 4; j++) {
    const u32x4 q = __builtin_nontemporal_load(as_global(reinterpret_cast<const u32x4*>(p)) + j);
    v[4 * j + 0] = q.x; v[4 * j + 1] = q.y; v[4 * j + 2] = q.z; v[4 * j + 3] = q.w;
  }
}

template <int R>
__device__ __forceinline__ void load_u64(const unsigned long long* __restrict__ p, unsigned long long (&v)[R]) {
  if (R == 1) { v[0] = __builtin_nontemporal_load(as_global(p)); return; }
#pragma unroll
  for (int j = 0; j < R / 2; j++) {
    const u64x2 q = __builtin_nontemporal_load(as_global(reinterpret_cast<const u64x2*>(p)) + j);
    v[2 * j + 0] = q.x; v[2 * j + 1] = q.y;
  }
}

template <int R>
__device__ __forceinline__ uint32_t load_valid(const uint8_t* __restrict__ bm, int64_t row0) {
  const uint32_t b = as_global(bm)[row0 >> 3];
  if (R == 1) return (b >> (row0 & 7)) & 1u;
  if (R == 8) return b;
  return (b >> (row0 & 4)) & 0xFu;
}

template <int R, typename T>
__device__ __forceinline__ uint32_t cmp_mask(const T (&v)[R], T lit, int op) {
  uint32_t m = 0;
  switch (op) {
    case OP_EQ:
#pragma unroll
      for (int r = 0; r < R; r++) m |= (uint32_t)(v[r] == lit) << r;
      break;
    case OP_NOT_EQ:
#pragma unroll
      for (int r = 0; r < R; r++) m |= (uint32_t)(v[r] != lit) << r;
      break;
    case OP_LT:
#pragma unroll
      for (int r = 0; r < R; r++) m |= (uint32_t)(v[r] < lit) << r;
      break;
    case OP_LT_EQ:
#pragma unroll
      for (int r = 0; r < R; r++) m |= (uint32_t)(v[r] <= lit) << r;
      break;
    case OP_GT:
#pragma unroll
      for (int r = 0; r < R; r++) m |= (uint32_t)(v[r] > lit) << r;
      break;
    case OP_GT_EQ:
#pragma unroll
      for (int r = 0; r < R; r++) m |= (uint32_t)(v[r] >= lit) << r;
      break;
    default: break;
  }
// ... 1894 lines not shown
  return hipGetLastError();
}

namespace {
typedef void (*SlotKernel)(const FdbScanArgs*, int, int64_t, FdbScanArgs);
struct SlotVariant { SlotKernel lds, nolds; int block; };
#define FDB_SV(NC4, NC8, L4, L8, BLK) {scan_slots_kernel<true, NC4, NC8, L4, L8, BLK>, scan_slots_kernel<false, NC4, NC8, L4, L8, BLK>, BLK}
const SlotVariant kSingle[] = {FDB_SV(2, 1, 0, 0, 512), FDB_SV(2, 1, 0, 0, 256), FDB_SV(2, 1, 0, 0, 1024)};
const SlotVariant kTwoPhase[] = {FDB_SV(FDB_MAX_C4, FDB_MAX_C8, FDB_MAX_L4, FDB_MAX_L8, 512), FDB_SV(FDB_MAX_C4, FDB_MAX_C8, FDB_MAX_L4, FDB_MAX_L8, 256),
                                  FDB_SV(FDB_MAX_C4, FDB_MAX_C8, FDB_MAX_L4, FDB_MAX_L8, 1024)};
#undef FDB_SV
const SlotVariant& slot_variant(int two_phase, int mode) {
  const int m = (mode >= 1 && mode <= 3) ? mode - 1 : 0;
  return two_phase ? kTwoPhase[m] : kSingle[m];
}
}

int fdb_slot_geometry(int two_phase, int mode, int lds_acc, size_t lds_bytes, int device, int* tile_rows, int* blocks_per_cu) {
  const SlotVariant& v = slot_variant(two_phase, mode);
  *tile_rows = v.block * 4;
  const void* fn = reinterpret_cast<const void*>(lds_acc ? v.lds : v.nolds);
  (void)hipFuncSetAttribute(fn, hipFuncAttributeMaxDynamicSharedMemorySize, 160 * 1024);
  int occ = 0;
  if (hipOccupancyMaxActiveBlocksPerMultiprocessor(&occ, fn, v.block, lds_bytes) != hipSuccess || occ < 1) { (void)hipGetLastError(); occ = 1; }
  if (occ > 2048 / v.block) occ = 2048 / v.block;
  *blocks_per_cu = occ;
  return 0;
}

hipError_t fdb_launch_scan_slots(const FdbScanArgs* d_parts, int n_parts, const FdbScanArgs& common, int64_t total_tiles, int grid_blocks,
                                 size_t lds_bytes, int two_phase, int mode, hipStream_t stream) {
  if (total_tiles <= 0 || grid_blocks <= 0) return hipSuccess;
  const SlotVariant& v = slot_variant(two_phase, mode);
  SlotKernel fn = common.lds_acc ? v.lds : v.nolds;
  hipLaunchKernelGGL(fn, dim3(grid_blocks), dim3(v.block), lds_bytes, stream, d_parts, n_parts, total_tiles, common);
  return hipGetLastError();
}

hipError_t fdb_launch_scan_dense(const FdbScanArgs& args, int grid_blocks, size_t lds_bytes, int rows_per_thread, hipStream_t stream) {
  const int64_t tile_rows = (int64_t)FDB_BLOCK * rows_per_thread;
  const int64_t n_tiles = (args.n_rows + tile_rows - 1) / tile_rows;
  if (n_tiles == 0) return hipSuccess;
  if (grid_blocks > n_tiles) grid_blocks = (int)n_tiles;
  dim3 grid(grid_blocks), block(FDB_BLOCK);
  if (rows_per_thread == 8) {
    if (args.lds_acc) {
      (void)hipFuncSetAttribute(reinterpret_cast<const void*>(&scan_dense_kernel<8, true>), hipFuncAttributeMaxDynamicSharedMemorySize, 160 * 1024);
      hipLaunchKernelGGL((scan_dense_kernel<8, true>), grid, block, lds_bytes, stream, args);
    } else {
      hipLaunchKernelGGL((scan_dense_kernel<8, false>), grid, block, lds_bytes, stream, args);
    }
  } else {
    if (args.lds_acc) {
      (void)hipFuncSetAttribute(reinterpret_cast<const void*>(&scan_dense_kernel<4, true>), hipFuncAttributeMaxDynamicSharedMemorySize, 160 * 1024);
      hipLaunchKernelGGL((scan_dense_kernel<4, true>), grid, block, lds_bytes, stream, args);
    } else {
      hipLaunchKernelGGL((scan_dense_kernel<4, false>), grid, block, lds_bytes, stream, args);
    }
  }
  return hipGetLastError();
}

__global__ __launch_bounds__(256) void stream_read_kernel(const u32x4* __restrict__ src, int64_t n_vec, unsigned long long* out) {
  const int64_t i = (int64_t)blockIdx.x * 256 + threadIdx.x;
  if (i >= n_vec) return;
  const u32x4 v = __builtin_nontemporal_load(as_global(src + i));
  if ((v.x ^ v.y ^ v.z ^ v.w) == 0x9E3779B9u) out[0] = 1;
}

hipError_t fdb_launch_stream_read(const void* src, int64_t bytes, unsigned long long* out, hipStream_t stream) {
  const int64_t n_vec = bytes / 16;
  if (n_vec <= 0) return hipSuccess;
  hipLaunchKernelGGL(stream_read_kernel, dim3((unsigned)((n_vec + 255) / 256)), dim3(256), 0, stream, reinterpret_cast<const u32x4*>(src), n_vec, out);
  return hipGetLastError();
}

namespace {
template <int W>
__global__ __launch_bounds__(256) void narrow_indices_kernel(const u32x4* __restrict__ src, u32x4* __restrict__ dst, int64_t rows, int64_t n_vec) {
  const int64_t i = (int64_t)blockIdx.x * 256 + threadIdx.x;
  if (i >= n_vec) return;
  constexpr int PER = 16 / W;
  constexpr int NV = PER / 4;
  const int64_t r0 = i * PER;
  uint32_t w[4] = {0u, 0u, 0u, 0u};
#pragma unroll
  for (int k = 0; k < NV; k++) {
    const u32x4 v = __builtin_nontemporal_load(as_global(src + i * NV + k));
    const uint32_t e[4] = {v.x, v.y, v.z, v.w};
#pragma unroll
    for (int q = 0; q < 4; q++) {
      const int r = k * 4 + q;
      const uint32_t x = r0 + r < rows ? (e[q] & (W == 1 ? 0xFFu : 0xFFFFu)) : 0u;
      w[(r * W) / 4] |= x << (8 * ((r * W) % 4));
    }
  }
  u32x4 out; out.x = w[0]; out.y = w[1]; out.z = w[2]; out.w = w[3];
  dst[i] = out;
}
}

hipError_t fdb_launch_narrow_indices(const uint32_t* src, void* dst, int64_t rows, int width, hipStream_t stream) {
  if (rows <= 0) return hipSuccess;
  if (width != 1 && width != 2) return hipErrorInvalidValue;
  const int64_t per = 16 / width, n_vec = (rows + per - 1) / per;
  const unsigned grid = (unsigned)((n_vec + 255) / 256);
  if (width == 1) hipLaunchKernelGGL(narrow_indices_kernel<1>, dim3(grid), dim3(256), 0, stream, reinterpret_cast<const u32x4*>(src), reinterpret_cast<u32x4*>(dst), rows, n_vec);
  else hipLaunchKernelGGL(narrow_indices_kernel<2>, dim3(grid), dim3(256), 0, stream, reinterpret_cast<const u32x4*>(src), reinterpret_cast<u32x4*>(dst), rows, n_vec);
  return hipGetLastError();
}

namespace {
__global__ void ordered_to_f64_kernel(unsigned long long* v, int64_t n) {
  for (int64_t i = (int64_t)blockIdx.x * blockDim.x + threadIdx.x; i < n; i += (int64_t)gridDim.x * blockDim.x) {
    const long long k = (long long)v[i];
    v[i] = (unsigned long long)(k ^ ((k >> 63) & 0x7FFFFFFFFFFFFFFFLL));
  }
}
}

hipError_t fdb_launch_ordered_to_f64(unsigned long long* v, int64_t n, hipStream_t stream) {
  if (n <= 0) return hipSuccess;
  int blocks = (int)((n + 255) / 256);
  if (blocks > 4096) blocks = 4096;
  hipLaunchKernelGGL(ordered_to_f64_kernel, dim3(blocks), dim3(256), 0, stream, v, n);
  return hipGetLastError();
}

hipError_t fdb_launch_fill_state(unsigned long long* base, int64_t n, int n_arrays, const unsigned long long* idents, hipStream_t stream) {
  if (n <= 0 || n_arrays <= 0) return hipSuccess;
  FillIdents f;
  for (int a = 0; a < 1 + FDB_MAX_AGGS; a++) f.v[a] = a < n_arrays ? idents[a] : 0ull;
  int blocks = (int)((n * n_arrays + 255) / 256);
  if (blocks > 2048) blocks = 2048;
  hipLaunchKernelGGL(fill_state_kernel, dim3(blocks), dim3(256), 0, stream, base, n, n_arrays, f);
  return hipGetLastError();
}

hipError_t fdb_launch_state_to_host(const unsigned long long* state, unsigned long long* host_out, uint32_t n_slots, uint64_t stride, int n_arrays, hipStream_t stream) {
  if (n_slots == 0 || n_arrays <= 0) return hipSuccess;
  hipLaunchKernelGGL(state_to_host_kernel, dim3((n_slots + 255) / 256, n_arrays), dim3(256), 0, stream, state, host_out, n_slots, stride);
  return hipGetLastError();
}

hipError_t fdb_launch_state_pack(const unsigned long long* state, unsigned long long* packed, uint32_t n_slots, uint64_t stride, int n_arrays, hipStream_t stream) {
  if (n_slots == 0 || n_arrays <= 0) return hipSuccess;
  hipLaunchKernelGGL(state_pack_kernel, dim3((n_slots + 255) / 256, n_arrays), dim3(256), 0, stream, state, packed, n_slots, stride);
  return hipGetLastError();
}
hipError_t fdb_launch_state_fold_ranks(const unsigned long long* gathered, int n_ranks, uint32_t n_slots, int n_arrays, const int32_t* ops, unsigned long long* state,
                                       uint64_t stride, unsigned long long* host_out, hipStream_t stream) {
  if (n_slots == 0 || n_arrays <= 0) return hipSuccess;
  FillIdents f;
  for (int a = 0; a < 1 + FDB_MAX_AGGS; a++) f.v[a] = a < n_arrays ? (unsigned long long)ops[a] : 0ull;
  hipLaunchKernelGGL(state_fold_ranks_kernel, dim3((n_slots + 255) / 256, n_arrays), dim3(256), 0, stream, gathered, n_ranks, n_slots, n_arrays, f, state, stride, host_out);
  return hipGetLastError();
}

hipError_t fdb_launch_merge_u64(unsigned long long* dst, const unsigned long long* src, const uint32_t* map, int64_t n, int32_t func,
                                int32_t is_f64, hipStream_t stream, const unsigned long long* src_cnt) {
  if (n <= 0) return hipSuccess;
  int blocks = (int)((n + 255) / 256);
  if (blocks > 2048) blocks = 2048;
  hipLaunchKernelGGL(merge_u64_kernel, dim3(blocks), dim3(256), 0, stream, dst, src, map, n, func, is_f64, src_cnt);
  return hipGetLastError();
}

hipError_t fdb_launch_pq_validity(const uint8_t* chunk, const FdbPqRun* def_runs, int32_t n_runs, int64_t n_rows, uint32_t* validity, uint32_t* counts,
                                  hipStream_t stream) {
  const int64_t n_words = (n_rows + 31) / 32;
  if (n_words == 0) return hipSuccess;
  int64_t blocks = (n_words + 255) / 256;
  if (blocks > 8192) blocks = 8192;
  hipLaunchKernelGGL(pq_validity_kernel, dim3((unsigned)blocks), dim3(256), 0, stream, chunk, def_runs, n_runs, n_rows, validity, counts);
  return hipGetLastError();
}
// ... 766 lines not shown
```

### frostdb_amd/csrc/fdb_plan.cpp

```cpp
#include "fdb_plan.h"
#include "fdb_jit.h"

#include "fdb_context.h"
#include "fdb_hostpool.h"
#include "fdb_plan_internal.h"

#include <algorithm>
#include <cstring>
#include <functional>

#include <atomic>
#include <chrono>
#include <cstdio>
#include <cstdlib>

namespace fdb {


void hip_check(hipError_t e, const char* what) {
  if (e != hipSuccess) throw Error(e == hipErrorOutOfMemory ? FDB_ERR_OOM : FDB_ERR_DEVICE, std::string(what) + ": " + hipGetErrorString(e));
}

void copy_stream(void* dst, const void* src, size_t n);
uint32_t copy_stream_max_u32(uint32_t* dst, const uint32_t* src, size_t n);
// ... 1332 lines not shown
  {
    std::vector<int> reps;
    for (int i : live) {
      const Resolved& R = Rs[(size_t)i];
      int found = -1;
      for (int r : reps) if (same_lut_set(Rs[(size_t)r], R)) { found = r; break; }
      if (found >= 0) { blob_base[(size_t)i] = blob_base[(size_t)found]; lut_class[(size_t)i] = lut_class[(size_t)found]; }
      else { blob_base[(size_t)i] = blob.add(R.blob.bytes.data(), R.blob.bytes.size()); lut_class[(size_t)i] = (int)reps.size(); reps.push_back(i); }
    }
  }
  StageScope stage_scope(ctx_);
  unsigned char* d_blob = blob.bytes.empty() ? nullptr : (unsigned char*)upload(blob.bytes.data(), blob.bytes.size());

  const size_t acc_bytes = align_up((size_t)n_slots_ * 4, 16) + (size_t)n_slots_ * 8 * aggs_.size();
  size_t lut_lds_max = 0;
  bool slots_ok = rows_per_thread == 0;
  const bool jit_possible = this->jit_possible();
  bool interp_ok = true;
  std::vector<int> layouts;
  for (int i : live) {
    Resolved& R = Rs[(size_t)i];
    FdbScanArgs& a = R.args;
    for (int g = 0; g < a.n_gcols; g++) a.gcols[g].stride = gcols_[(size_t)part_gcols[(size_t)i][(size_t)g]].stride;
    for (size_t j = 0; j < aggs_.size(); j++) a.aggs[j].acc = aggs_[j].d_acc;
    a.cnt = d_cnt_;
    a.n_slots = n_slots_;
    a.need_count = 0;
    for (size_t j = 0; j < aggs_.size(); j++) if (a.aggs[j].func == FDB_AGG_COUNT) a.need_count = 1;
    a.lut_class = lut_class[(size_t)i];
    lut_lds_max = std::max(lut_lds_max, place_luts(R.luts, d_blob + blob_base[(size_t)i], 0, &a));
    if (slots_ok) {
      bool strict = true;
      const int layout = assign_slots(*bs[i], R, 1, jit_possible, &strict);
      if (layout == 0) slots_ok = false;
      interp_ok = interp_ok && strict;
      layouts.push_back(layout);
    }
  }
  int lds_acc = 0;
  size_t lds_bytes = lut_lds_max;
  int base_grid = grid_override > 0 ? grid_override : fdb_scan_default_grid(device_);
  if (fixed_order) {
    if (!jit_possible || !slots_ok || !use_partials) throw Error(FDB_ERR_UNSUPPORTED, "deterministic float sums need the run-time specialised dense kernel");
    if (lut_lds_max + 4 * acc_bytes > 150 * 1024) throw Error(FDB_ERR_UNSUPPORTED, "deterministic float sums: four per-wave tables of " + std::to_string(acc_bytes) + " bytes do not fit LDS");
    lds_acc = 1; lds_bytes += 4 * acc_bytes;
  }
  else if (lut_lds_max + acc_bytes <= FDB_LDS_BUDGET) { lds_acc = 1; lds_bytes += acc_bytes; }
  else if (lut_lds_max + acc_bytes <= 150 * 1024) { lds_acc = 1; lds_bytes += acc_bytes; if (grid_override <= 0) base_grid /= 2; }
  int cache_slots = 0;
  if (!lds_acc && jit_possible) {
    const size_t entry = 8 + 8 * aggs_.size();
    cache_slots = 1;
    while ((size_t)cache_slots * 2 * entry <= 48 * 1024) cache_slots *= 2;
    lds_bytes = lut_lds_max + (size_t)cache_slots * entry;
  }
  for (int i : live) {
    Rs[(size_t)i].args.lds_lut_bytes = (uint32_t)lut_lds_max; Rs[(size_t)i].args.lds_acc = lds_acc; Rs[(size_t)i].args.cache_slots = cache_slots;
  }
  pt.mark("lut upload");

  int32_t funcs[1 + FDB_MAX_AGGS] = {0};
  funcs[0] = 1;
  {
    const FdbScanArgs& a0 = Rs[(size_t)live[0]].args;
    for (size_t j = 0; j < aggs_.size(); j++) {
      const int32_t f = a0.aggs[j].func;
      const int32_t ty = aggs_[j].type;
      funcs[1 + j] = f == FDB_AGG_COUNT ? 0 : f == FDB_AGG_SUM ? (ty == FDB_T_F64 ? 2 : 1) : f == FDB_AGG_MIN ? 3 : 4;
    }
  }
  auto alloc_partials = [&](int grid) -> unsigned long long* {
    if (!lds_acc || !use_partials || grid <= 0) return nullptr;
    void* p = ctx_->dev_alloc((size_t)grid * (1 + aggs_.size()) * n_slots_ * 8);
    scratch_.push_back(p);
    return (unsigned long long*)p;
  };

  int two_phase = 0, tile_rows_i = 0, per_cu = 1;
  const int sub = sub_tiles == 4 ? 0 : sub_tiles;
  struct Narrowed { int part, k, col; bool late; const void* wide; int64_t saved; };
  std::vector<Narrowed> narrowed;
  hipFunction_t jit_fn = nullptr;
  int jit_block = sub == 1 ? 512 : sub == 2 ? 256 : sub == 3 ? 1024 : 0;
  if (fixed_order) jit_block = 256;
  if (slots_ok) {
    for (int l : layouts) if (l == 2) two_phase = 1;
    if (two_phase) {
      size_t k = 0;
      for (int i : live)
        if (layouts[k++] == 1 && assign_slots(*bs[i], Rs[(size_t)i], 2, jit_possible) != 2) throw Error(FDB_ERR_INVALID, "internal: slot re-assignment failed");
    }
    if (sub_tiles != 4 && lds_bytes <= 150 * 1024) {
      auto narrow_pool = [&](bool late) {
        const FdbScanArgs& a0 = Rs[(size_t)live[0]].args;
        const int n4 = late ? a0.n_l4 : a0.n_c4;
        for (int i : live) if ((late ? Rs[(size_t)i].args.n_l4 : Rs[(size_t)i].args.n_c4) != n4) return;
        for (int k = 0; k < n4; k++) {
          int w = 0;
          for (int i : live) {
            const Resolved& R = Rs[(size_t)i];
            const int ci = late ? R.l4_col[k] : R.c4_col[k];
            const int wi = (late ? R.args.l4[k] : R.args.c4[k]).values == nullptr || ci < 0 ? 4 : scan_cache_width(*bs[i], (size_t)ci);
            w = w == 0 || w == wi ? wi : 4;
            if (w == 4) break;
          }
          if (w >= 4) continue;
          for (int i : live) {
            Resolved& R = Rs[(size_t)i];
            const int ci = late ? R.l4_col[k] : R.c4_col[k];
            FdbColSlot& sl = late ? R.args.l4[k] : R.args.c4[k];
            bool counted = false;
            for (const Narrowed& nw : narrowed) if (nw.part == i && nw.col == ci) counted = true;
            const int64_t saved = counted ? 0 : bs[i]->rows * (int64_t)(4 - w);
            narrowed.push_back(Narrowed{i, k, ci, late, sl.values, saved});
            sl.values = scan_cache_get(*bs[i], (size_t)ci, stream_);
            (late ? R.args.wl4 : R.args.w4)[k] = (uint8_t)w;
            R.bytes -= saved;
          }
        }
      };
      if (jit_possible) { narrow_pool(false); if (two_phase) narrow_pool(true); }
      JitShape shape;
      bool same = true, first = true;
      const FdbScanArgs& args0 = Rs[(size_t)live[0]].args;
      for (int i : live) {
        if (first) { shape = jit_shape(args0, two_phase != 0, jit_block ? jit_block : 256); first = false; }
        else if (!jit_shape_merge_args(&shape, args0, Rs[(size_t)i].args, two_phase != 0)) { same = false; break; }
      }
      if (!same && live.size() > 1 && jit_possible) {
        std::vector<std::string> keys;
        std::vector<std::vector<const DeviceBatch*>> groups;
        for (int i : live) {
          const std::string k = jit_shape(Rs[(size_t)i].args, two_phase != 0, 256).key(false);
          size_t g = 0;
          for (; g < keys.size(); g++) if (keys[g] == k) break;
          if (g == keys.size()) { keys.push_back(k); groups.emplace_back(); }
          groups[g].push_back(bs[i]);
        }
        if (groups.size() > 1) {
          ctx_->defer_staging(false);
          for (auto& g : groups) push_batches(g.data(), (int)g.size());
          return;
        }
      }
      {
        int regs_per_slot = 2;
        for (const AggState& A : aggs_) if (A.func != FDB_AGG_COUNT || final_stage_) regs_per_slot += 2;
        if (n_slots_ >= 1 && n_slots_ <= 8 && (int)n_slots_ * regs_per_slot <= 48) shape.reg_slots = (int)n_slots_;
      }
      shape.wave_tables = fixed_order;
      shape.uniform_fold = !knobs_.no_uniform_fold;
      if (same) {
        JitDeferScope defer(interp_ok && !fixed_order);
        if (jit_block != 0) { jit_fn = jit_get(shape); if (jit_fn != nullptr) per_cu = jit_blocks_per_cu(jit_fn, jit_block, lds_bytes); }
        else {
          int row_bytes = 0;
          for (int k = 0; k < shape.n_c4; k++) row_bytes += shape.c4[k].has_values ? shape.c4[k].width : 0;
          for (int k = 0; k < shape.n_l4; k++) row_bytes += shape.l4[k].has_values ? shape.l4[k].width : 0;
          for (int k = 0; k < shape.n_c8; k++) row_bytes += shape.c8[k].has_values ? 8 : 0;
          for (int k = 0; k < shape.n_l8; k++) row_bytes += shape.l8[k].has_values ? 8 : 0;
          jit_fn = jit_select(shape, lds_bytes, row_bytes, &jit_block, &per_cu);
        }
      }
    }
    if (jit_fn == nullptr) {
      for (const Narrowed& nw : narrowed) {
        Resolved& R = Rs[(size_t)nw.part];
        (nw.late ? R.args.l4 : R.args.c4)[nw.k].values = nw.wide;
        (nw.late ? R.args.wl4 : R.args.w4)[nw.k] = 0;
        R.bytes += nw.saved;
      }
      narrowed.clear();
    }
    if (jit_fn == nullptr && !interp_ok) slots_ok = false;
  }
  if (fixed_order && jit_fn == nullptr) throw Error(FDB_ERR_UNSUPPORTED, "deterministic float sums need the run-time specialised dense kernel (records of one shape, hiprtc available)");

  pt.mark("kernel select");
  if (slots_ok) {
    if (jit_fn != nullptr) {
      tile_rows_i = jit_block * 4;
    } else {
      fdb_slot_geometry(two_phase, sub, lds_acc, lds_bytes, device_, &tile_rows_i, &per_cu);
    }
    int grid = grid_override > 0 ? grid_override : (fdb_scan_default_grid(device_) / 2) * per_cu;
    const int64_t tile_rows = tile_rows_i;
    int64_t total_tiles = 0;
    std::vector<FdbScanArgs> parts;
    parts.reserve(live.size());
    for (int i : live) {
      FdbScanArgs& a = Rs[(size_t)i].args;
      a.tile_begin = total_tiles;
      total_tiles += (a.n_rows + tile_rows - 1) / tile_rows;
      a.tile_end = total_tiles;
      parts.push_back(a);
    }
    if (grid > total_tiles) grid = (int)total_tiles;
    unsigned long long* partials = alloc_partials(grid);
    for (FdbScanArgs& a : parts) a.partials = partials;
    bool fill_rides = false;
    if (state_virgin_ && jit_fn != nullptr && partials != nullptr && (uint64_t)slots_alloc_ * (1 + aggs_.size()) < (1ull << 32)) {
      FdbScanArgs& a0 = parts[0];
      a0.fill_state = d_state_;
      a0.fill_words = (uint32_t)(slots_alloc_ * (1 + aggs_.size()));
      a0.fill_alloc = (uint32_t)slots_alloc_;
      state_idents(a0.fill_idents);
      fill_rides = true;
    } else {
      materialize_state();
    }
    trace("before scan");
    pt.mark("parts build");
    const FdbScanArgs* d_parts = (const FdbScanArgs*)upload(parts.data(), parts.size() * sizeof(FdbScanArgs));
    ctx_->flush_staging();
    pt.mark("parts upload");
    trace("after upload");
    timed([&] {
      if (jit_fn != nullptr) hip_check(jit_launch(jit_fn, d_parts, (int)parts.size(), total_tiles, parts[0], grid, jit_block, lds_bytes, stream_), "scan launch");
      else hip_check(fdb_launch_scan_slots(d_parts, (int)parts.size(), parts[0], total_tiles, grid, lds_bytes, two_phase, sub, stream_), "scan launch");
    });
    if (fill_rides) state_virgin_ = false;
    last_kernel_ = jit_fn != nullptr ? "fdb_plan_kernel" : "scan_slots_kernel";
    pt.mark("scan launch");
    trace("after scan");
    if (partials != nullptr) {
      unsigned long long* host_out = mirror_target();
      hip_check(fdb_launch_reduce_partials(partials, grid, (int)(1 + aggs_.size()), n_slots_, d_state_, slots_alloc_, funcs, host_out, stream_), "reduce partials");
      mirror_valid_ = host_out != nullptr;
    }
    trace("after reduce");
    stat_launches += 1;
  } else {
    const int rpt = rows_per_thread == 8 ? 8 : 4;
    materialize_state();
    ctx_->flush_staging();
    for (int i : live) {
      FdbScanArgs& a = Rs[(size_t)i].args;
      if (a.n_expr > 0) throw Error(FDB_ERR_UNSUPPORTED, "computed (projected) columns are not supported by the sequential kernel (too many referenced columns)");
      a.n_c4 = a.n_c8 = 0;
      const int grid = fdb_scan_grid(a, base_grid, rpt);
      a.partials = alloc_partials(grid);
      timed([&] { hip_check(fdb_launch_scan_dense(a, grid, lds_bytes, rpt, stream_), "scan launch"); });
      last_kernel_ = "scan_dense_kernel";
      mirror_valid_ = false;
      if (a.partials != nullptr) {
        unsigned long long* host_out = mirror_target();
        hip_check(fdb_launch_reduce_partials(a.partials, grid, (int)(1 + aggs_.size()), n_slots_, d_state_, slots_alloc_, funcs, host_out, stream_), "reduce partials");
        mirror_valid_ = host_out != nullptr;
      }
      stat_launches += 1;
    }
  }
  pt.mark("reduce launch");
  state_dirty_ = true;
  for (int i : live) { stat_bytes += Rs[(size_t)i].bytes; stat_rows += bs[i]->rows; }
}

void Plan::fetch_state(std::vector<unsigned long long>* cnt, std::vector<std::vector<unsigned long long>>* acc) {
  hip_check(hipSetDevice(device_), "hipSetDevice");
  acc->assign(aggs_.size(), {});
  if (d_state_ == nullptr) { sync(); cnt->clear(); return; }
  materialize_state();
  if (mirror_valid_ && h_mirror_ != nullptr) {
    sync();
// ... 478 lines not shown
```

### frostdb_amd/csrc/fdb_record.h

```cpp
#pragma once

#include <cstddef>
#include <cstdint>
#include <memory>
#include <string>
#include <vector>

#include "fdb_arrow.h"

namespace fdb {

inline size_t align_up(size_t v, size_t a) { return (v + a - 1) / a * a; }
constexpr size_t kTailPad = 256;
constexpr size_t kNoSlot = (size_t)-1;

inline size_t value_width(ColKind kind) { return kind == ColKind::DICT || kind == ColKind::STR ? 4 : 8; }
inline size_t values_slot(size_t rows, size_t width) { return align_up(rows * width + kTailPad, 256); }
inline size_t bitmap_slot(size_t rows) { return align_up((rows + 63) / 64 * 8 + kTailPad, 256); }

struct RecordLayout {
  struct Col { size_t val_off, bit_off; };
  std::vector<Col> cols;
  size_t total = 0;
  void add(size_t rows, size_t width, bool bitmap) {
    Col c{total, kNoSlot};
    total += values_slot(rows, width);
    if (bitmap) { c.bit_off = total; total += bitmap_slot(rows); }
    cols.push_back(c);
  }
};

struct DevColumn {
  std::string name;
  std::string format;
  ColKind kind = ColKind::OTHER;
  int64_t length = 0;
  int64_t null_count = 0;
  void* d_values = nullptr;
  uint8_t* d_validity = nullptr;
  std::shared_ptr<HostDict> dict;
  int64_t value_bytes = 0;
  int64_t validity_bytes = 0;
};

inline int64_t finish_column(DevColumn* d, int64_t rows, int64_t nulls, void* values, void* bitmap) {
  d->length = rows;
  d->null_count = nulls;
  d->d_values = values;
  d->value_bytes = d->kind == ColKind::BOOL ? (rows + 7) / 8 : rows * (int64_t)value_width(d->kind);
  if (nulls > 0 && bitmap != nullptr) { d->d_validity = (uint8_t*)bitmap; d->validity_bytes = (rows + 7) / 8; }
  return d->value_bytes + d->validity_bytes;
}

}

#ifndef FDB_RECORD_HOST_ONLY
#include <exception>

#include <hip/hip_runtime_api.h>

namespace fdb {

class Context;
struct DeviceBatch;

struct DrainOnUnwind {
  hipStream_t s; int n = std::uncaught_exceptions();
  ~DrainOnUnwind() { if (std::uncaught_exceptions() > n) (void)hipStreamSynchronize(s); }
};

struct CallScope {
  Context* ctx = nullptr;
  std::vector<void*> scratch;
  explicit CallScope(int device);
  ~CallScope();
  CallScope(const CallScope&) = delete;
  void* alloc(size_t bytes);
};

constexpr int64_t kScanCacheMinRows = (int64_t)1 << 20;
inline int narrow_width(size_t entries) { return entries <= 256 ? 1 : entries <= 65536 ? 2 : 4; }
struct ScanCache {
  struct Col { void* d = nullptr; int width = 0; size_t bytes = 0; };
  std::vector<Col> cols;
  int64_t bytes = 0;
};
int scan_cache_width(const DeviceBatch& b, size_t c);
const void* scan_cache_get(const DeviceBatch& b, size_t c, hipStream_t stream);

void require_values(const DeviceBatch& in, const char* what);

void finish_column(DeviceBatch* b, size_t c, int64_t nulls, void* values, void* bitmap);

class RecordBuilder {
 public:
  RecordBuilder(int device, int64_t rows);
  RecordBuilder(RecordBuilder&&) noexcept;
  ~RecordBuilder();
  void add(const std::string& name, const std::string& format, ColKind kind, std::shared_ptr<HostDict> dict, bool may_have_nulls);
  void allocate();
  void* values(size_t c) const;
// ... 14 lines not shown
```

### frostdb_amd/physicalplan.py

```python
from __future__ import annotations

import ctypes
import os
import threading
from typing import Any, Callable, List, Optional, Sequence

import pyarrow as pa

from .arrow_c import ArrowArray, ArrowSchema, ExportedBatch, import_batch
from .logicalplan import AggregationFunction, Column, Expr, expr_name, to_desc

_HERE = os.path.dirname(os.path.abspath(__file__))
LIB_PATH = os.path.join(_HERE, "libfrostdb_amd.so")

FDB_OK, FDB_ERR_INVALID, FDB_ERR_UNSUPPORTED, FDB_ERR_NOT_FOUND, FDB_ERR_DEVICE, FDB_ERR_OOM, FDB_ERR_STATE = range(7)


class FdbError(RuntimeError):
    def __init__(self, code: int, msg: str):
        super().__init__(f"frostdb_amd error {code}: {msg}")
        self.code = code
        self.msg = msg


class UnsupportedError(FdbError):
    """≙ ErrUnsupportedBooleanExpression / ErrUnsupportedBinaryOperation / ErrUnsupportedSumType."""


_lib: Optional[ctypes.CDLL] = None


def lib() -> ctypes.CDLL:
    global _lib
    if _lib is not None:
        return _lib
    path = os.environ.get("FDB_LIB_PATH") or LIB_PATH
    if not os.path.exists(path):
        raise ImportError(f"{path} is missing: run `python -m frostdb_amd.build` (hipcc, gfx950). There is no CPU fallback.")
    L = ctypes.CDLL(path)
    vp, i32, i64 = ctypes.c_void_p, ctypes.c_int32, ctypes.c_int64
    P = ctypes.POINTER
    L.fdb_version.restype = ctypes.c_char_p
    L.fdb_last_error.restype = ctypes.c_char_p
    L.fdb_device_count.argtypes = [P(ctypes.c_int)]
    L.fdb_plan_create.argtypes = [vp, ctypes.c_int, P(vp)]
    L.fdb_plan_push.argtypes = [vp, vp, vp]
    L.fdb_plan_push_batch.argtypes = [vp, vp]
    L.fdb_plan_push_batches.argtypes = [vp, P(vp), i32]
    L.fdb_plan_finish.argtypes = [vp, vp, vp, P(i64)]
    L.fdb_plan_finish_next.argtypes = [vp, vp, vp, P(i64), P(i32)]
    L.fdb_plan_merge.argtypes = [vp, vp]
    L.fdb_plan_filter.argtypes = [vp, vp, vp, vp, vp, P(i64)]
    L.fdb_plan_select.argtypes = [vp, vp, vp, vp, i64, P(i64)]
    L.fdb_plan_draw.restype = ctypes.c_char_p
    L.fdb_plan_draw.argtypes = [vp]
    L.fdb_plan_last_error.restype = ctypes.c_char_p
    L.fdb_plan_last_error.argtypes = [vp]
    L.fdb_plan_close.argtypes = [vp]
    L.fdb_plan_close.restype = None
    L.fdb_plan_num_groups.argtypes = [vp, P(i64)]
    L.fdb_plan_partial_keys.argtypes = [vp, vp, vp]
    L.fdb_plan_partial_state.argtypes = [vp, i32, vp, i64]
    L.fdb_plan_agg_type.argtypes = [vp, i32, ctypes.c_char_p]
    L.fdb_plan_state_signature.argtypes = [vp, P(ctypes.c_uint64), P(i64)]
    L.fdb_plan_state_pointers.argtypes = [vp, P(vp), P(i64), P(i64)]
    L.fdb_plan_state_read.argtypes = [vp, i32, vp, i64]
    L.fdb_plan_state_write.argtypes = [vp, i32, vp, i64]
    L.fdb_batch_import.argtypes = [vp, vp, ctypes.c_int, P(vp)]
    L.fdb_batch_num_rows.restype = i64
    L.fdb_batch_num_rows.argtypes = [vp]
    L.fdb_batch_device_bytes.restype = i64
    L.fdb_batch_device_bytes.argtypes = [vp]
    L.fdb_batch_scan_cache_bytes.restype = i64
    L.fdb_batch_scan_cache_bytes.argtypes = [vp]
    L.fdb_batch_release.argtypes = [vp]
    L.fdb_batch_release.restype = None
    L.fdb_plan_stats.argtypes = [vp, P(i64), P(ctypes.c_double), P(i64), P(i64)]
    L.fdb_regex_match.argtypes = [ctypes.c_char_p, i64, ctypes.c_char_p, i64, P(i32)]
    L.fdb_parquet_stats.argtypes = [P(i64), P(ctypes.c_double), P(ctypes.c_double), P(i64), P(i64)]
    L.fdb_jit_stats.argtypes = [P(i64), P(ctypes.c_double), P(i64)]
    L.fdb_plan_merge_ms.argtypes = [vp, P(ctypes.c_double)]
    L.fdb_plan_set_timing.argtypes = [vp, i32]
    L.fdb_plan_stream.argtypes = [vp, P(vp)]
    L.fdb_plan_set_tuning.argtypes = [vp, i32, i32]
    L.fdb_plan_set_deterministic.argtypes = [vp, i32]
    L.fdb_plan_set_exact_sums.argtypes = [vp, i32]
    L.fdb_selftest_exact_sum.argtypes = [vp, i64, vp]
    L.fdb_snappy_decode_pages.argtypes = [vp, i64, vp, i32, vp, i64, ctypes.c_int, vp, P(ctypes.c_double)]
    L.fdb_lz4_decode_pages.argtypes = [vp, i64, vp, i32, vp, i64, ctypes.c_int, vp, P(ctypes.c_double)]
    L.fdb_parquet_device_pages.argtypes = [ctypes.c_int, P(i64), P(i64)]
    L.fdb_plan_state_arrays.argtypes = [vp, P(i32)]
    L.fdb_plan_state_array_op.argtypes = [vp, i32, P(i32)]
    L.fdb_plan_group_schema.argtypes = [vp, vp, vp]
    L.fdb_plan_seed_groups.argtypes = [vp, vp, vp]
    L.fdb_plan_hash_export.argtypes = [vp, vp, i32, ctypes.POINTER(ctypes.c_void_p), ctypes.POINTER(ctypes.c_int64), ctypes.POINTER(i32)]
    L.fdb_plan_hash_import.argtypes = [vp, vp, ctypes.c_int64]
    L.fdb_read_ceiling.argtypes = [ctypes.c_int, ctypes.c_int64, i32, ctypes.POINTER(ctypes.c_double)]
    L.fdb_plan_last_kernel.argtypes = [vp]
    L.fdb_arrow_roundtrip.argtypes = [vp, vp, vp, vp]
    L.fdb_selftest_widen.argtypes = [vp, i32, vp, i64]
    L.fdb_plan_explain.argtypes = [vp, ctypes.c_char_p, i64, P(i64)]
    L.fdb_plan_last_kernel.restype = ctypes.c_char_p
    L.fdb_comm_unique_id.argtypes = [vp]
    L.fdb_comm_init_rank.argtypes = [vp, i32, i32, ctypes.c_int, P(vp)]
    L.fdb_comm_init_all.argtypes = [P(ctypes.c_int), i32, P(vp)]
    L.fdb_comm_init_local.argtypes = [P(ctypes.c_int), i32, P(vp)]
    L.fdb_comm_rank.argtypes = [vp]
    L.fdb_comm_rank.restype = i32
    L.fdb_comm_size.argtypes = [vp]
    L.fdb_comm_size.restype = i32
    L.fdb_plan_push_many.argtypes = [vp, vp, vp, i32, P(i32)]
    L.fdb_plan_push_many.restype = i32
    L.fdb_comm_transport_ranks.argtypes = [vp]
    L.fdb_comm_transport_ranks.restype = i32
    L.fdb_comm_last_error.argtypes = [vp]
    L.fdb_comm_last_error.restype = ctypes.c_char_p
    L.fdb_comm_destroy.argtypes = [vp]
    L.fdb_comm_destroy.restype = None
    L.fdb_plan_allreduce.argtypes = [vp, vp, P(i32)]
    L.fdb_plan_exchange.argtypes = [vp, vp, P(vp)]
    L.fdb_live_allocations.argtypes = [P(i64), P(i64), P(i64)]
    L.fdb_plan_filter_batch.argtypes = [vp, vp, P(vp), P(i64)]
    L.fdb_plan_finish_batch.argtypes = [vp, P(vp), P(i64)]
    L.fdb_plan_filter_batches.argtypes = [vp, P(vp), i32, P(vp), P(i64)]
    L.fdb_plan_select_batch.argtypes = [vp, vp, vp, i64, P(i64)]
    L.fdb_batch_export.argtypes = [vp, vp, vp]
    L.fdb_plan_project_batch.argtypes = [vp, vp, i32, vp, P(vp)]
    L.fdb_plan_project_batches.argtypes = [vp, vp, i32, P(vp), i32, P(vp)]
    L.fdb_plan_project.argtypes = [vp, vp, i32, vp, vp, vp, vp]
    L.fdb_batch_from_parquet.argtypes = [vp, i32, i64, ctypes.c_int, P(vp)]
    L.fdb_batches_from_parquet.argtypes = [vp, i32, ctypes.c_int, P(vp)]
    L.fdb_batch_take.argtypes = [vp, vp, i64, P(vp)]
    L.fdb_batch_limit.argtypes = [vp, ctypes.c_uint64, P(vp)]
    L.fdb_sampler_create.argtypes = [i64, ctypes.c_uint64, ctypes.c_int, P(vp)]
    L.fdb_sampler_push_batch.argtypes = [vp, vp]
    L.fdb_sampler_push.argtypes = [vp, vp, vp]
    L.fdb_sampler_finish_batch.argtypes = [vp, P(vp), P(i64)]
    L.fdb_sampler_finish.argtypes = [vp, vp, vp, P(i64)]
    L.fdb_sampler_close.argtypes = [vp]
    L.fdb_sampler_close.restype = None
    L.fdb_selftest_reservoir.argtypes = [ctypes.c_uint64, i64, vp, i32, vp]
    L.fdb_batch_sort_indices.argtypes = [vp, vp, i32, vp]
    L.fdb_batch_sort.argtypes = [vp, vp, i32, P(vp)]
    L.fdb_selftest_sort_key.argtypes = [i32, ctypes.c_uint32, ctypes.c_uint64, P(ctypes.c_uint64)]
    L.fdb_sort_bench.argtypes = [vp, vp, i32, i32, i32, P(ctypes.c_double), P(ctypes.c_double), P(i32)]
    L.fdb_batches_merge.argtypes = [P(vp), i32, vp, i32, ctypes.c_uint64, P(vp)]
    L.fdb_batches_merge_named.argtypes = [P(vp), i32, vp, i32, ctypes.c_uint64, P(vp)]
    L.fdb_selftest_merge_schema.argtypes = [P(ctypes.c_char_p), P(i32), P(i32), i32, vp, i32, P(i32), P(i32), i32, P(i32), P(i32)]
    L.fdb_osync_create.argtypes = [i32, vp, i32, P(vp)]
    L.fdb_osync_push.argtypes = [vp, i32, vp, P(vp)]
    L.fdb_osync_finish.argtypes = [vp, i32, P(vp), P(i32)]
    L.fdb_osync_close.argtypes = [vp]
    L.fdb_osync_close.restype = None
    L.fdb_merge_tile_rows.argtypes = [i32]
    L.fdb_merge_tile_rows.restype = i32
    L.fdb_selftest_merge_path.argtypes = [vp, i64, vp, i64, i32, vp]
    L.fdb_merge_bench.argtypes = [P(vp), i32, vp, i32, i32, i32, P(ctypes.c_double), P(ctypes.c_double), P(ctypes.c_double), i32, P(i32), P(i32)]
    L.fdb_batch_column_name.argtypes = [vp, i32]
    L.fdb_batch_column_name.restype = ctypes.c_char_p
    L.fdb_batch_column_format.argtypes = [vp, i32]
    L.fdb_batch_column_format.restype = ctypes.c_char_p
    for suffix, takes in PARQUET_WRITE_ENTRIES:
        optional_args = [vp, i32, vp, i32, vp, vp, vp, vp][:takes + min(takes, 2)]
        getattr(L, "fdb_batch_to_parquet" + suffix).argtypes = [vp, vp] + optional_args + [P(vp), P(i64)]
        getattr(L, "fdb_selftest_parquet_write" + suffix).argtypes = [vp, vp, vp] + optional_args + [P(vp), P(i64)]
    L.fdb_bytes_free.argtypes = [vp]
    L.fdb_bytes_free.restype = None
    _lib = L
    return L


def jit_stats() -> dict:
    n, ms, d = ctypes.c_int64(), ctypes.c_double(), ctypes.c_int64()
    lib().fdb_jit_stats(ctypes.byref(n), ctypes.byref(ms), ctypes.byref(d))
    return {"compiled": n.value, "compile_ms": ms.value, "disk_loads": d.value}


def regex_match(pattern, value: bytes) -> bool:
    pat = pattern.encode() if isinstance(pattern, str) else bytes(pattern)
    m = ctypes.c_int32()
    rc = lib().fdb_regex_match(pat, len(pat), value, len(value), ctypes.byref(m))
    if rc != 0:
        _raise(rc, lib().fdb_last_error().decode("utf-8", "replace"))
# ... 1152 lines not shown
```

### include/frostdb_amd.h

```cpp
#ifndef FROSTDB_AMD_H
#define FROSTDB_AMD_H

#include <stdint.h>
#include "arrow_c_data.h"

#ifdef __cplusplus
extern "C" {
#endif

#if defined(__GNUC__) || defined(__clang__)
#define FDB_API __attribute__((visibility("default")))
#else
#define FDB_API
#endif

typedef enum fdb_status {
  FDB_OK = 0,
  FDB_ERR_INVALID = 1,
  FDB_ERR_UNSUPPORTED = 2,
  FDB_ERR_NOT_FOUND = 3,
  FDB_ERR_DEVICE = 4,
  FDB_ERR_OOM = 5,
  FDB_ERR_STATE = 6
} fdb_status;
// ... 36 lines not shown
  FDB_LIT_FLOAT64 = 3,
  FDB_LIT_STRING = 4,
  FDB_LIT_BINARY = 5,
  FDB_LIT_BOOL = 6
} fdb_literal_type;

typedef struct fdb_literal {
  int32_t type;
  int32_t _pad;
  int64_t i64;
  uint64_t u64;
  double f64;
  const char* data;
  int64_t len;
} fdb_literal;

typedef struct fdb_expr {
  int32_t op;
  int32_t left;
  int32_t right;
  int32_t _pad;
  const char* column;
  fdb_literal literal;
} fdb_expr;

typedef struct fdb_aggregation {
  int32_t func;
  int32_t dynamic;
  const char* column;
} fdb_aggregation;

typedef struct fdb_group_expr {
  const char* name;
  int32_t dynamic;
  int32_t _pad;
} fdb_group_expr;

typedef struct fdb_proj_node {
  int32_t kind;
  int32_t op;
  int32_t left;
  int32_t right;
  const char* column;
  fdb_literal literal;
} fdb_proj_node;

typedef struct fdb_projection {
  const char* name;
  const fdb_proj_node* nodes;
  int32_t n_nodes;
  int32_t root;
} fdb_projection;

typedef int32_t (*fdb_regex_match_fn)(void* user, const char* pattern, int64_t pattern_len, const uint8_t* value, int64_t value_len);

typedef struct fdb_plan_desc {
  const fdb_expr* filter;
  int32_t n_filter;
  int32_t filter_root;
  const fdb_aggregation* aggs;
  int32_t n_aggs;
  int32_t n_groups;
  const fdb_group_expr* groups;
  int32_t final_stage;
  int32_t n_projections;
  const fdb_projection* projections;
  fdb_regex_match_fn regex_match;
  void* regex_user;
  int32_t ordered;
  int32_t _pad2;
} fdb_plan_desc;

typedef struct fdb_plan fdb_plan;
typedef struct fdb_batch fdb_batch;

FDB_API const char* fdb_version(void);
FDB_API const char* fdb_last_error(void);
FDB_API int fdb_device_count(int* n_devices);
FDB_API int fdb_read_ceiling(int device, int64_t bytes, int32_t reps, double* gb_per_s);

FDB_API int fdb_arrow_roundtrip(struct ArrowArray* batch, struct ArrowSchema* schema, struct ArrowArray* out, struct ArrowSchema* out_schema);
FDB_API int fdb_regex_match(const char* pattern, int64_t pattern_len, const uint8_t* value, int64_t value_len, int32_t* matched);
FDB_API int fdb_selftest_widen(const void* src, int32_t width, uint32_t* dst, int64_t n);

FDB_API int fdb_plan_create(const fdb_plan_desc* desc, int device, fdb_plan** out);
FDB_API int fdb_plan_push(fdb_plan* plan, struct ArrowArray* batch, struct ArrowSchema* schema);
FDB_API int fdb_plan_push_many(fdb_plan* plan, struct ArrowArray* const* batches, struct ArrowSchema* const* schemas, int32_t n, int32_t* n_pushed);
FDB_API int fdb_plan_push_batch(fdb_plan* plan, const fdb_batch* batch);
FDB_API int fdb_plan_push_batches(fdb_plan* plan, const fdb_batch* const* batches, int32_t n);
FDB_API int fdb_plan_finish(fdb_plan* plan, struct ArrowArray* out, struct ArrowSchema* out_schema, int64_t* n_rows);
FDB_API int fdb_plan_finish_next(fdb_plan* plan, struct ArrowArray* out, struct ArrowSchema* out_schema, int64_t* n_rows, int32_t* emitted);
FDB_API int fdb_plan_merge(fdb_plan* dst, fdb_plan* src);
FDB_API int fdb_plan_filter(fdb_plan* plan, struct ArrowArray* batch, struct ArrowSchema* schema,
                    struct ArrowArray* out, struct ArrowSchema* out_schema, int64_t* n_selected);
FDB_API int fdb_plan_select(fdb_plan* plan, struct ArrowArray* batch, struct ArrowSchema* schema,
                    uint32_t* indices, int64_t capacity, int64_t* n_selected);
FDB_API int fdb_plan_filter_batch(fdb_plan* plan, const fdb_batch* batch, fdb_batch** out, int64_t* n_selected);
FDB_API int fdb_plan_finish_batch(fdb_plan* plan, fdb_batch** out, int64_t* n_rows);
FDB_API int fdb_plan_filter_batches(fdb_plan* plan, const fdb_batch* const* batches, int32_t n, fdb_batch** out, int64_t* n_selected);
FDB_API int fdb_plan_select_batch(fdb_plan* plan, const fdb_batch* batch, uint32_t* dev_indices, int64_t capacity, int64_t* n_selected);

typedef struct fdb_project_col {
  int32_t kind;
  int32_t _pad;
  const char* name;
} fdb_project_col;
FDB_API int fdb_plan_project_batch(fdb_plan* plan, const fdb_project_col* cols, int32_t n_cols, const fdb_batch* in, fdb_batch** out);
FDB_API int fdb_plan_project_batches(fdb_plan* plan, const fdb_project_col* cols, int32_t n_cols, const fdb_batch* const* in, int32_t n, fdb_batch** out);
FDB_API int fdb_plan_project(fdb_plan* plan, const fdb_project_col* cols, int32_t n_cols, struct ArrowArray* batch, struct ArrowSchema* schema,
                             struct ArrowArray* out, struct ArrowSchema* out_schema);
FDB_API const char* fdb_plan_draw(fdb_plan* plan);
FDB_API int fdb_plan_explain(const fdb_plan_desc* desc, char* buf, int64_t capacity, int64_t* needed);
FDB_API const char* fdb_plan_last_error(const fdb_plan* plan);
FDB_API void fdb_plan_close(fdb_plan* plan);

FDB_API int fdb_plan_num_groups(fdb_plan* plan, int64_t* n_groups);
FDB_API int fdb_plan_partial_keys(fdb_plan* plan, struct ArrowArray* out, struct ArrowSchema* out_schema);
FDB_API int fdb_plan_partial_state(fdb_plan* plan, int32_t agg, void* dst, int64_t capacity_bytes);
FDB_API int fdb_plan_state_signature(fdb_plan* plan, uint64_t* signature, int64_t* n_slots);
FDB_API int fdb_plan_state_pointers(fdb_plan* plan, void** base, int64_t* array_stride, int64_t* n_slots);
FDB_API int fdb_plan_state_read(fdb_plan* plan, int32_t array, void* dst, int64_t capacity_bytes);
FDB_API int fdb_plan_state_write(fdb_plan* plan, int32_t array, const void* src, int64_t bytes);
FDB_API int fdb_plan_state_arrays(fdb_plan* plan, int32_t* n_arrays);
FDB_API int fdb_plan_state_array_op(fdb_plan* plan, int32_t array, int32_t* op);
FDB_API int fdb_plan_agg_type(fdb_plan* plan, int32_t agg, char* format_out);

FDB_API int fdb_plan_group_schema(fdb_plan* plan, struct ArrowArray* out, struct ArrowSchema* out_schema);
FDB_API int fdb_plan_seed_groups(fdb_plan* plan, struct ArrowArray* schema_record, struct ArrowSchema* schema);
FDB_API int fdb_plan_hash_export(fdb_plan* src, fdb_plan* layout, int32_t n_parts, void** dev_rows, int64_t* counts, int32_t* row_words32);
FDB_API int fdb_plan_hash_import(fdb_plan* plan, const void* dev_rows, int64_t n_rows);

typedef struct fdb_comm fdb_comm;
#define FDB_COMM_ID_BYTES 128
FDB_API int fdb_comm_unique_id(uint8_t id[FDB_COMM_ID_BYTES]);
FDB_API int fdb_comm_init_rank(const uint8_t id[FDB_COMM_ID_BYTES], int32_t n_ranks, int32_t rank, int device, fdb_comm** out);
FDB_API int fdb_comm_init_all(const int* devices, int32_t n, fdb_comm** out );
FDB_API int fdb_comm_init_local(const int* devices, int32_t n, fdb_comm** out );
FDB_API int32_t fdb_comm_rank(const fdb_comm* comm);
FDB_API int32_t fdb_comm_size(const fdb_comm* comm);
FDB_API int32_t fdb_comm_transport_ranks(fdb_comm* comm);
FDB_API const char* fdb_comm_last_error(const fdb_comm* comm);
FDB_API void fdb_comm_destroy(fdb_comm* comm);
FDB_API int fdb_plan_allreduce(fdb_plan* plan, fdb_comm* comm, int32_t* aligned);
FDB_API int fdb_plan_exchange(fdb_plan* plan, fdb_comm* comm, fdb_plan** shard);

FDB_API int fdb_live_allocations(int64_t* device_blocks, int64_t* device_bytes, int64_t* pinned_blocks);

FDB_API int fdb_batch_import(struct ArrowArray* batch, struct ArrowSchema* schema, int device, fdb_batch** out);
FDB_API int64_t fdb_batch_num_rows(const fdb_batch* batch);
FDB_API int64_t fdb_batch_device_bytes(const fdb_batch* batch);
FDB_API int64_t fdb_batch_scan_cache_bytes(const fdb_batch* batch);
FDB_API void fdb_batch_release(fdb_batch* batch);
FDB_API int fdb_batch_export(const fdb_batch* batch, struct ArrowArray* out, struct ArrowSchema* out_schema);

typedef struct fdb_parquet_chunk {
  const char* name;
  int32_t physical_type;
  int32_t optional;
  int32_t utf8;
  int32_t codec;
  const uint8_t* data;
  int64_t n_bytes;
} fdb_parquet_chunk;
FDB_API int fdb_batch_from_parquet(const fdb_parquet_chunk* chunks, int32_t n_chunks, int64_t n_rows, int device, fdb_batch** out);
typedef struct fdb_parquet_row_group {
  const fdb_parquet_chunk* chunks;
// ... 113 lines not shown
```

Measured before the change: 519.7 billion rows/s.

## Interleave narrowed dictionary indices per 1024-row block and load whole blocks per wave

The narrow-index builder now writes 1- and 2-byte dictionary indices in a 1024-row interleaved layout. The JIT scan kernel gains a 'quad' mode in which each wave covers four 256-row sub-tiles and fetches each narrow column with one or two full 16-byte nontemporal loads per lane. Wide columns and validity bits for those sub-tiles are prefetched into register arrays before the unrolled loop. The aim is to replace sub-16-byte narrow loads with full-width vector loads and increase memory-level parallelism. In exchange it raises register pressure, changes block and wave sizing, and makes the narrow layout position-dependent, which adds a self-test.

After: 531.7 billion rows/s (median of 6 runs). 2.3% higher.

```diff
diff --git a/frostdb_amd/csrc/fdb_capi.cpp b/frostdb_amd/csrc/fdb_capi.cpp
--- a/frostdb_amd/csrc/fdb_capi.cpp
+++ b/frostdb_amd/csrc/fdb_capi.cpp
@@ -12,6 +12,7 @@
 #include "fdb_mergerec.h"
 #include "fdb_plan.h"
 #include "fdb_pqwrite_host.h"
+#include "fdb_record.h"
 #include "fdb_regex.h"
 #include "fdb_sort.h"
 #include "fdb_sortkey.h"
@@ -132,6 +133,25 @@
       return;
     }
     fdb::widen_indices(src, width, dst, (size_t)n);
+  });
+}
+
+int fdb_selftest_scan_cache(const uint32_t* indices, int64_t rows, int32_t width, int device, uint8_t* out, int64_t out_bytes) {
+  return guard(nullptr, [&] {
+    if (indices == nullptr || out == nullptr || rows <= 0 || rows > ((int64_t)1 << 28) || (width != 1 && width != 2) || out_bytes != (rows * width + 15) / 16 * 16)
+      throw fdb::Error(FDB_ERR_INVALID, "scan cache: 1 to 2^28 rows, width 1 or 2, out_bytes = rows * width rounded up to 16");
+    fdb::CallScope call(device);
+    void* d_src = call.alloc(fdb::values_slot((size_t)rows, 4));
+    void* d_dst = call.alloc(fdb::values_slot((size_t)rows, (size_t)width));
+    fdb::hip_check(hipMemcpyAsync(d_src, indices, (size_t)rows * 4, hipMemcpyHostToDevice, call.ctx->stream), "scan cache: copy in");
+    fdb::hip_check(fdb_launch_narrow_indices((const uint32_t*)d_src, d_dst, rows, width, call.ctx->stream), "scan cache: builder");
+    fdb::hip_check(hipMemcpyAsync(out, d_dst, (size_t)out_bytes, hipMemcpyDeviceToHost, call.ctx->stream), "scan cache: copy out");
+    fdb::hip_check(hipStreamSynchronize(call.ctx->stream), "scan cache: wait");
+    for (int64_t i = 0; i < rows; i++) {
+      const int64_t at = fdb::scan_cache_position(i, rows, width);
+      const uint32_t got = width == 1 ? out[at] : (uint32_t)out[2 * at] | ((uint32_t)out[2 * at + 1] << 8);
+      if (got != (indices[i] & (width == 1 ? 0xFFu : 0xFFFFu))) throw fdb::Error(FDB_ERR_INVALID, "scan cache: row " + std::to_string(i) + " is not at its position");
+    }
   });
 }
 
diff --git a/frostdb_amd/csrc/fdb_jit.cpp b/frostdb_amd/csrc/fdb_jit.cpp
--- a/frostdb_amd/csrc/fdb_jit.cpp
+++ b/frostdb_amd/csrc/fdb_jit.cpp
@@ -108,6 +108,25 @@
 }
 template <int OP, typename T> __device__ __forceinline__ uint32_t cmp4(T a, T b, T c, T d, T lit, uint32_t valid) {
   return ((uint32_t)cmp1<OP, T>(a, lit) | ((uint32_t)cmp1<OP, T>(b, lit) << 1) | ((uint32_t)cmp1<OP, T>(c, lit) << 2) | ((uint32_t)cmp1<OP, T>(d, lit) << 3)) & valid;
+}
+)HIP";
+
+const char* kQuadPreamble = R"HIP(
+__device__ __forceinline__ u32x4 ldblock(const void* base, uint32_t byte_off) {
+#ifdef FDB_LD_TEMPORAL
+  return *as_global(reinterpret_cast<const u32x4*>(reinterpret_cast<const char*>(base) + byte_off));
+#else
+  return __builtin_nontemporal_load(as_global(reinterpret_cast<const u32x4*>(reinterpret_cast<const char*>(base) + byte_off)));
+#endif
+}
+__device__ __forceinline__ uint32_t dword_of(u32x4 q, int k) { return k == 0 ? q.x : k == 1 ? q.y : k == 2 ? q.z : q.w; }
+__device__ __forceinline__ u32x4 idx1x4(uint32_t v) {
+  u32x4 r; r.x = v & 0xFFu; r.y = (v >> 8) & 0xFFu; r.z = (v >> 16) & 0xFFu; r.w = v >> 24;
+  return r;
+}
+__device__ __forceinline__ u32x4 idx2x4(uint32_t lo, uint32_t hi) {
+  u32x4 r; r.x = lo & 0xFFFFu; r.y = lo >> 16; r.z = hi & 0xFFFFu; r.w = hi >> 16;
+  return r;
 }
 )HIP";
 
@@ -211,29 +230,73 @@
 
   static std::string reg(bool wide, bool late, int slot) { return std::string(late ? "l" : "e") + (wide ? "8_" : "4_") + std::to_string(slot); }
 
+  bool full_block = false;
+  void block_loads() {
+    auto narrow = [&](const JitSlot& c, const std::string& r) {
+      if (!c.has_values || c.width >= 4) return;
+      if (c.width == 1) o << "      const u32x4 Q_" << r << " = ldblock(P_" << r << "_v + (size_t)wb, lane * 16u);\n";
+      else o << "      const u32x4 Q_" << r << "a = ldblock(P_" << r << "_v + (size_t)wb * 2, lane * 16u), Q_" << r << "b = ldblock(P_" << r << "_v + (size_t)wb * 2 + 1024, lane * 16u);\n";
+    };
+    for (int i = 0; i < s.n_c4; i++) narrow(s.c4[i], reg(false, false, i));
+    for (int i = 0; i < s.n_l4; i++) narrow(s.l4[i], reg(false, true, i));
+    for (int i = 0; i < s.n_c4; i++) {
+      const std::string r = reg(false, false, i);
+      if (s.c4[i].has_values && s.c4[i].width >= 4) o << "      u32x4 A_" << r << "[4];\n";
+      if (s.c4[i].has_validity != 0) o << "      uint32_t M_" << r << "[4];\n";
+    }
+    for (int i = 0; i < s.n_c8; i++) {
+      const std::string r = reg(true, false, i);
+      if (s.c8[i].has_values) o << "      u64x2 A_" << r << "a[4], A_" << r << "b[4];\n";
+      if (s.c8[i].has_validity != 0) o << "      uint32_t M_" << r << "[4];\n";
+    }
+    o << "#pragma unroll\n      for (int u = 0; u < 4; u++) {\n        const size_t o0 = (size_t)(wb + 256 * u); (void)o0;\n";
+    auto valid = [&](const JitSlot& c, const std::string& r) {
+      if (c.has_validity == 1) o << "        M_" << r << "[u] = ldv(P_" << r << "_b + (o0 >> 3), lane_offb, lane_shb);\n";
+      else if (c.has_validity == 2) o << "        M_" << r << "[u] = P_" << r << "_b != nullptr ? ldv(P_" << r << "_b + (o0 >> 3), lane_offb, lane_shb) : 0xFu;\n";
+    };
+    for (int i = 0; i < s.n_c4; i++) {
+      const std::string r = reg(false, false, i);
+      if (s.c4[i].has_values && s.c4[i].width >= 4) o << "        A_" << r << "[u] = ld4(P_" << r << "_v + o0 * 4, lane_off4);\n";
+      valid(s.c4[i], r);
+    }
+    for (int i = 0; i < s.n_c8; i++) {
+      const std::string r = reg(true, false, i);
+      if (s.c8[i].has_values) o << "        A_" << r << "a[u] = ld8(P_" << r << "_v + o0 * 8, lane_off8);\n        A_" << r << "b[u] = ld8(P_" << r << "_v + o0 * 8, lane_off8 + 16u);\n";
+      valid(s.c8[i], r);
+    }
+    o << "      }\n";
+  }
+
   void loads(bool late) {
     const int n4 = late ? s.n_l4 : s.n_c4, n8 = late ? s.n_l8 : s.n_c8;
     for (int i = 0; i < n4; i++) {
       const JitSlot& c = late ? s.l4[i] : s.c4[i];
       const std::string r = reg(false, late, i);
-      if (c.has_values && c.width == 1) o << "    const u32x4 " << r << " = ld1x4(P_" << r << "_v + tile_off1, lane_off1);\n";
+      if (full_block && c.has_values && c.width == 1) o << "    const u32x4 " << r << " = idx1x4(dword_of(Q_" << r << ", u));\n";
+      else if (full_block && c.has_values && c.width == 2)
+        o << "    const u32x4 " << r << " = idx2x4(dword_of(u < 2 ? Q_" << r << "a : Q_" << r << "b, 2 * (u & 1)), dword_of(u < 2 ? Q_" << r << "a : Q_" << r << "b, 2 * (u & 1) + 1));\n";
+      else if (full_block && !late && c.has_values) o << "    const u32x4 " << r << " = A_" << r << "[u];\n";
+      else if (c.has_values && c.width == 1) o << "    const u32x4 " << r << " = ld1x4(P_" << r << "_v + tile_off1, lane_off1);\n";
       else if (c.has_values && c.width == 2) o << "    const u32x4 " << r << " = ld2x4(P_" << r << "_v + tile_off2, lane_off2);\n";
       else if (c.has_values) o << "    const u32x4 " << r << " = ld4(P_" << r << "_v + tile_off4, lane_off4);\n";
-      mask(c, r);
+      mask(c, r, late);
     }
     for (int i = 0; i < n8; i++) {
       const JitSlot& c = late ? s.l8[i] : s.c8[i];
       const std::string r = reg(true, late, i);
-      if (c.has_values) {
+      if (full_block && !late && c.has_values) {
+        o << "    const u64x2 " << r << "a = A_" << r << "a[u], " << r << "b = A_" << r << "b[u];\n";
+      } else if (c.has_values) {
         o << "    const u64x2 " << r << "a = ld8(P_" << r << "_v + tile_off8, lane_off8);\n";
         o << "    const u64x2 " << r << "b = ld8(P_" << r << "_v + tile_off8, lane_off8 + 16u);\n";
       }
-      mask(c, r);
+      mask(c, r, late);
     }
   }
 
   bool live_mask = false;
-  void mask(const JitSlot& c, const std::string& r) {
+  void mask(const JitSlot& c, const std::string& r, bool late = false) {
+    if (full_block && !late && c.has_validity != 0) { o << "    const uint32_t " << r << "_m = M_" << r << "[u];\n"; return; }
     const char* all = live_mask ? "live" : "0xFu";
     const char* cut = live_mask ? " & live" : "";
     if (c.has_validity == 1) o << "    const uint32_t " << r << "_m = ldv(P_" << r << "_b + tile_offb, lane_offb, lane_shb)" << cut << ";\n";
@@ -290,6 +353,7 @@
   std::string source() {
     const int BLK = s.block;
     o << "#include \"fdb_kernels.h\"\n" << kPreamble;
+    if (s.quad) o << kQuadPreamble;
     o << "extern \"C\" __global__ __launch_bounds__(" << BLK << ") void fdb_plan_kernel(const FdbScanArgs* __restrict__ parts, const int n_parts, const long long total_tiles, const FdbScanArgs c) {\n";
     o << "  extern __shared__ __align__(16) unsigned char smem[];\n  const uint32_t tid = threadIdx.x;\n  const uint32_t n_slots = c.n_slots;\n";
     o << "  if (c.fill_state != nullptr)  // (a fresh table: its identity fill rides on this launch, see FdbScanArgs)\n";
@@ -341,8 +405,14 @@
       }
     }
     o << "  long long n_rows = 0, tile_begin = 0, tile_end = 0; int part = -1, lut_class = -1;\n";
-    o << "  const uint32_t lane_off4 = tid * 16u, lane_off8 = tid * 32u, lane_offb = tid >> 1, lane_shb = (tid & 1u) * 4u;\n";
-    o << "  const uint32_t lane_off1 = tid * 4u, lane_off2 = tid * 8u; (void)lane_off1; (void)lane_off2;\n";
+    if (s.quad) {
+      o << "  const uint32_t lane = tid & 63u, wave = (uint32_t)__builtin_amdgcn_readfirstlane((int)(tid >> 6));\n";
+      o << "  const uint32_t lane_off4 = lane * 16u, lane_off8 = lane * 32u, lane_offb = lane >> 1, lane_shb = (lane & 1u) * 4u; (void)lane_off4;\n";
+      o << "  const uint32_t lane_off1 = lane * 4u, lane_off2 = lane * 8u; (void)lane_off1; (void)lane_off2;\n";
+    } else {
+      o << "  const uint32_t lane_off4 = tid * 16u, lane_off8 = tid * 32u, lane_offb = tid >> 1, lane_shb = (tid & 1u) * 4u;\n";
+      o << "  const uint32_t lane_off1 = tid * 4u, lane_off2 = tid * 8u; (void)lane_off1; (void)lane_off2;\n";
+    }
     o << "  for (long long tile = blockIdx.x; tile < total_tiles; tile += gridDim.x) {\n";
     o << "    if (part < 0 || tile >= tile_end) {\n      int np = part < 0 ? 0 : part;\n      while (np + 1 < n_parts && tile >= parts[np].tile_end) np++;\n      part = np;\n";
     o << "      const FdbScanArgs& pa = parts[part];\n      n_rows = pa.n_rows; tile_begin = pa.tile_begin; tile_end = pa.tile_end;\n";
@@ -369,179 +439,205 @@
       if (s.gcols[g].lut_in_lds)
         o << "        for (uint32_t i = tid; i < pa.gcols[" << g << "].lut_len; i += " << BLK << ") reinterpret_cast<uint32_t*>(smem + G_lds" << g << ")[i] = as_global(G_lut" << g << ")[i];\n";
     o << "        __syncthreads();\n      }\n    }\n";
-    o << "    const long long r0 = (tile - tile_begin) * " << BLK * 4 << "LL;\n";
-    o << "    const long long left = n_rows - r0 - (long long)tid * 4;\n    if (left <= 0) continue;\n";
-    o << "    const size_t tile_off4 = (size_t)r0 * 4, tile_off8 = (size_t)r0 * 8, tile_offb = (size_t)(r0 >> 3);\n";
-    o << "    const size_t tile_off1 = (size_t)r0, tile_off2 = (size_t)r0 * 2; (void)tile_off1; (void)tile_off2;\n";
-    o << "    const uint32_t live = left >= 4 ? 0xFu : ((1u << (int)left) - 1u);\n";
-    live_mask = true;
-    loads(false);
-    o << "    uint32_t sel = live;\n";
-    if (!s.code.empty()) o << "    sel &= " << filter_expr() << ";\n";
-    {
-      std::vector<int> seen;
-      for (const JitExprNode& e : s.exprs)
-        if (e.kind == 7 && std::find(seen.begin(), seen.end(), e.slot) == seen.end()) { seen.push_back(e.slot); o << "    const uint32_t PM" << e.slot << " = " << leaf_expr(e.slot) << "; (void)PM" << e.slot << ";\n"; }
-    }
-    const bool uniform_fold = s.uniform_fold && s.lds_acc && !s.cache && s.reg_slots == 0 && !s.wave_tables && !s.two_phase && !s.gcols.empty();
-    if (uniform_fold) o << "    const unsigned long long has = __ballot(sel != 0u);\n    if (has == 0ull) continue;\n";
-    else o << "    if (sel == 0u) continue;\n";
-    loads(true);
-    o << "    uint32_t gid0 = 0, gid1 = 0, gid2 = 0, gid3 = 0;\n";
-    for (size_t g = 0; g < s.gcols.size(); g++) {
-      const JitGroup& G = s.gcols[g];
-      const std::string r = reg(false, s.two_phase, G.slot);
-      const std::string lut = G.lut_in_lds ? ("reinterpret_cast<const uint32_t*>(smem + G_lds" + std::to_string(g) + ")") : ("as_global(G_lut" + std::to_string(g) + ")");
-      const char* comp[4] = {"x", "y", "z", "w"};
-      for (int k = 0; k < 4; k++)
-        o << "    gid" << k << " += ((" << r << "_m >> " << k << ") & 1u ? " << lut << "[" << r << "." << comp[k] << "] : 0u) * G_stride" << g << ";\n";
-    }
-    if (uniform_fold) {
-      auto raw_of = [&](size_t j, int k) {
-        const JitAgg& A = s.aggs[j];
-        const std::string comp = std::string(k < 2 ? "a" : "b") + (k % 2 == 0 ? ".x" : ".y");
-        if (A.expr != 0) {
-          auto col = [&](int ni) -> std::string { if (s.exprs[(size_t)ni].kind == 7) return "((PM" + std::to_string(s.exprs[(size_t)ni].slot) + " >> " + std::to_string(k) + ") & 1u)"; return reg(true, s.two_phase, s.exprs[(size_t)ni].slot) + comp; };
-          auto colvalid = [&](int ni) { return "((" + reg(true, s.two_phase, s.exprs[(size_t)ni].slot) + "_m >> " + std::to_string(k) + ") & 1u)"; };
-          return "(" + expr_valid(s.exprs, A.expr - 1, col, colvalid) + " ? " + expr_bits(s.exprs, A.expr - 1, expr_value(s.exprs, A.expr - 1, col, colvalid)) + " : 0ull)";
-        }
-        const std::string r = reg(true, s.two_phase, A.slot);
-        return "((" + r + "_m >> " + std::to_string(k) + ") & 1u ? " + r + comp + " : c.aggs[" + std::to_string(j) + "].null_value)";
-      };
-      o << "    {\n      const uint32_t my_first = (sel & 1u) ? gid0 : (sel & 2u) ? gid1 : (sel & 4u) ? gid2 : gid3;\n";
-      o << "      const uint32_t g0 = (uint32_t)__builtin_amdgcn_readlane((int)my_first, __builtin_ctzll(has));\n";
-      o << "      if (__ballot(sel != 0u && my_first != g0) == 0ull && __ballot(1) == ~0ull &&\n";
-      o << "          __ballot(((sel & 1u) && gid0 != g0) || ((sel & 2u) && gid1 != g0) || ((sel & 4u) && gid2 != g0) || ((sel & 8u) && gid3 != g0)) == 0ull) {\n";
-      o << "        uint32_t u_cnt = (uint32_t)__builtin_popcount(sel);\n";
-      for (size_t j = 0; j < s.aggs.size(); j++) {
-        const JitAgg& A = s.aggs[j];
-        if (A.func == FDB_AGG_COUNT) continue;
-        const std::string v = "u" + std::to_string(j);
-        if (A.func == FDB_AGG_SUM && A.type == FDB_T_F64) {
-          o << "        double " << v << " = 0.0;\n";
-          for (int k = 0; k < 4; k++) o << "        if ((sel >> " << k << ") & 1u) " << v << " += __longlong_as_double((long long)" << raw_of(j, k) << ");\n";
-        } else if (A.func == FDB_AGG_SUM) {
-          o << "        unsigned long long " << v << " = 0ull;\n";
-          for (int k = 0; k < 4; k++) o << "        if ((sel >> " << k << ") & 1u) " << v << " += " << raw_of(j, k) << ";\n";
-        } else {
-          o << "        long long " << v << " = " << (A.func == FDB_AGG_MIN ? "0x7FFFFFFFFFFFFFFFLL" : "(-0x7FFFFFFFFFFFFFFFLL - 1)") << ";\n";
-          for (int k = 0; k < 4; k++) {
-            const std::string key = A.type == FDB_T_F64 ? ("f64_minmax_key(__longlong_as_double((long long)" + raw_of(j, k) + "), " + (A.func == FDB_AGG_MIN ? "true" : "false") + ")") : ("(long long)" + raw_of(j, k));
-            o << "        if ((sel >> " << k << ") & 1u) { const long long y = " << key << "; " << v << " = " << (A.func == FDB_AGG_MIN ? "y < " : "y > ") << v << " ? y : " << v << "; }\n";
+    auto tile_body = [&] {
+      loads(false);
+      o << "    uint32_t sel = live;\n";
+      if (!s.code.empty()) o << "    sel &= " << filter_expr() << ";\n";
+      {
+        std::vector<int> seen;
+        for (const JitExprNode& e : s.exprs)
+          if (e.kind == 7 && std::find(seen.begin(), seen.end(), e.slot) == seen.end()) { seen.push_back(e.slot); o << "    const uint32_t PM" << e.slot << " = " << leaf_expr(e.slot) << "; (void)PM" << e.slot << ";\n"; }
+      }
+      const bool uniform_fold = s.uniform_fold && s.lds_acc && !s.cache && s.reg_slots == 0 && !s.wave_tables && !s.two_phase && !s.gcols.empty();
+      if (uniform_fold) o << "    const unsigned long long has = __ballot(sel != 0u);\n    if (has == 0ull) continue;\n";
+      else o << "    if (sel == 0u) continue;\n";
+      loads(true);
+      o << "    uint32_t gid0 = 0, gid1 = 0, gid2 = 0, gid3 = 0;\n";
+      for (size_t g = 0; g < s.gcols.size(); g++) {
+        const JitGroup& G = s.gcols[g];
+        const std::string r = reg(false, s.two_phase, G.slot);
+        const std::string lut = G.lut_in_lds ? ("reinterpret_cast<const uint32_t*>(smem + G_lds" + std::to_string(g) + ")") : ("as_global(G_lut" + std::to_string(g) + ")");
+        const char* comp[4] = {"x", "y", "z", "w"};
+        for (int k = 0; k < 4; k++)
+          o << "    gid" << k << " += ((" << r << "_m >> " << k << ") & 1u ? " << lut << "[" << r << "." << comp[k] << "] : 0u) * G_stride" << g << ";\n";
+      }
+      if (uniform_fold) {
+        auto raw_of = [&](size_t j, int k) {
+          const JitAgg& A = s.aggs[j];
+          const std::string comp = std::string(k < 2 ? "a" : "b") + (k % 2 == 0 ? ".x" : ".y");
+          if (A.expr != 0) {
+            auto col = [&](int ni) -> std::string { if (s.exprs[(size_t)ni].kind == 7) return "((PM" + std::to_string(s.exprs[(size_t)ni].slot) + " >> " + std::to_string(k) + ") & 1u)"; return reg(true, s.two_phase, s.exprs[(size_t)ni].slot) + comp; };
+            auto colvalid = [&](int ni) { return "((" + reg(true, s.two_phase, s.exprs[(size_t)ni].slot) + "_m >> " + std::to_string(k) + ") & 1u)"; };
+            return "(" + expr_valid(s.exprs, A.expr - 1, col, colvalid) + " ? " + expr_bits(s.exprs, A.expr - 1, expr_value(s.exprs, A.expr - 1, col, colvalid)) + " : 0ull)";
           }
-        }
-      }
-      o << "#pragma unroll\n        for (int sh = 32; sh > 0; sh >>= 1) {\n          u_cnt += (uint32_t)__shfl_xor((int)u_cnt, sh, 64);\n";
-      for (size_t j = 0; j < s.aggs.size(); j++) {
-        const JitAgg& A = s.aggs[j];
-        if (A.func == FDB_AGG_COUNT) continue;
-        const std::string v = "u" + std::to_string(j);
-        if (A.func == FDB_AGG_SUM && A.type == FDB_T_F64) o << "          " << v << " += __shfl_xor(" << v << ", sh, 64);\n";
-        else if (A.func == FDB_AGG_SUM) o << "          " << v << " += (unsigned long long)__shfl_xor((long long)" << v << ", sh, 64);\n";
-        else o << "          { const long long y = __shfl_xor(" << v << ", sh, 64); " << v << " = " << (A.func == FDB_AGG_MIN ? "y < " : "y > ") << v << " ? y : " << v << "; }\n";
-      }
-      o << "        }\n        if ((tid & 63u) == 0u) {\n";
-      if (s.need_count) o << "          atomicAdd(&l_cnt[g0], u_cnt);\n";
-      else o << "          l_cnt[g0] = 1u;\n";
-      for (size_t j = 0; j < s.aggs.size(); j++) {
-        const JitAgg& A = s.aggs[j];
-        if (A.func == FDB_AGG_COUNT) continue;
-        const std::string v = "u" + std::to_string(j);
-        const std::string acc = "(l_acc + (size_t)" + std::to_string(j) + " * n_slots + g0)";
-        if (A.func == FDB_AGG_SUM && A.type == FDB_T_F64) o << "          atomicAdd(reinterpret_cast<double*>" << acc << ", " << v << ");\n";
-        else if (A.func == FDB_AGG_SUM) o << "          atomicAdd(" << acc << ", " << v << ");\n";
-        else o << "          " << (A.func == FDB_AGG_MIN ? "atomicMin" : "atomicMax") << "(reinterpret_cast<long long*>" << acc << ", " << v << ");\n";
-      }
-      o << "        }\n        continue;\n      }\n    }\n";
-    }
-    for (int k = 0; k < 4 && s.reg_slots > 0; k++) {
-      const std::string comp = std::string(k < 2 ? "a" : "b") + (k % 2 == 0 ? ".x" : ".y");
-      o << "    {\n      const bool on = (sel >> " << k << ") & 1u;\n";
-      std::vector<std::string> val(s.aggs.size());
-      for (size_t j = 0; j < s.aggs.size(); j++) {
-        const JitAgg& A = s.aggs[j];
-        if (A.func == FDB_AGG_COUNT) continue;
-        std::string raw;
-        if (A.expr != 0) {
-          auto col = [&](int ni) -> std::string { if (s.exprs[(size_t)ni].kind == 7) return "((PM" + std::to_string(s.exprs[(size_t)ni].slot) + " >> " + std::to_string(k) + ") & 1u)"; return reg(true, s.two_phase, s.exprs[(size_t)ni].slot) + comp; };
-          auto colvalid = [&](int ni) { return "((" + reg(true, s.two_phase, s.exprs[(size_t)ni].slot) + "_m >> " + std::to_string(k) + ") & 1u)"; };
-          raw = "(" + expr_valid(s.exprs, A.expr - 1, col, colvalid) + " ? " + expr_bits(s.exprs, A.expr - 1, expr_value(s.exprs, A.expr - 1, col, colvalid)) + " : 0ull)";
-        } else {
           const std::string r = reg(true, s.two_phase, A.slot);
-          raw = "((" + r + "_m >> " + std::to_string(k) + ") & 1u ? " + r + comp + " : c.aggs[" + std::to_string(j) + "].null_value)";
-        }
-        const std::string v = "v" + std::to_string(j);
-        if (A.func == FDB_AGG_SUM && A.type == FDB_T_F64) o << "      const double " << v << " = __longlong_as_double((long long)" << raw << ");\n";
-        else if (A.func == FDB_AGG_SUM) o << "      const unsigned long long " << v << " = " << raw << ";\n";
-        else o << "      const long long " << v << " = " << (A.type == FDB_T_F64 ? ("f64_minmax_key(__longlong_as_double((long long)" + raw + "), " + (A.func == FDB_AGG_MIN ? "true" : "false") + ")") : ("(long long)" + raw)) << ";\n";
-        val[j] = v;
-      }
-      for (int t = 0; t < s.reg_slots; t++) {
-        const std::string m = s.reg_slots == 1 ? std::string("on") : ("(on && gid" + std::to_string(k) + " == " + std::to_string(t) + "u)");
-        o << "      R_cnt" << t << " += " << m << " ? 1ull : 0ull;\n";
+          return "((" + r + "_m >> " + std::to_string(k) + ") & 1u ? " + r + comp + " : c.aggs[" + std::to_string(j) + "].null_value)";
+        };
+        o << "    {\n      const uint32_t my_first = (sel & 1u) ? gid0 : (sel & 2u) ? gid1 : (sel & 4u) ? gid2 : gid3;\n";
+        o << "      const uint32_t g0 = (uint32_t)__builtin_amdgcn_readlane((int)my_first, __builtin_ctzll(has));\n";
+        o << "      if (__ballot(sel != 0u && my_first != g0) == 0ull && __ballot(1) == ~0ull &&\n";
+        o << "          __ballot(((sel & 1u) && gid0 != g0) || ((sel & 2u) && gid1 != g0) || ((sel & 4u) && gid2 != g0) || ((sel & 8u) && gid3 != g0)) == 0ull) {\n";
+        o << "        uint32_t u_cnt = (uint32_t)__builtin_popcount(sel);\n";
         for (size_t j = 0; j < s.aggs.size(); j++) {
           const JitAgg& A = s.aggs[j];
           if (A.func == FDB_AGG_COUNT) continue;
-          const std::string acc = "R_a" + std::to_string(j) + "_" + std::to_string(t);
-          if (A.func == FDB_AGG_SUM && A.type == FDB_T_F64) o << "      " << acc << " += " << m << " ? " << val[j] << " : 0.0;\n";
-          else if (A.func == FDB_AGG_SUM) o << "      " << acc << " += " << m << " ? " << val[j] << " : 0ull;\n";
-          else if (A.func == FDB_AGG_MIN) o << "      " << acc << " = (" << m << " && " << val[j] << " < " << acc << ") ? " << val[j] << " : " << acc << ";\n";
-          else o << "      " << acc << " = (" << m << " && " << val[j] << " > " << acc << ") ? " << val[j] << " : " << acc << ";\n";
-        }
-      }
-      o << "    }\n";
-    }
-    for (int k = 0; k < 4 && s.reg_slots == 0; k++) {
-      const std::string gidk = "gid" + std::to_string(k);
-      o << "    if ((sel >> " << k << ") & 1u) {\n";
-      if (s.cache) {
-        o << "      const uint32_t ch = ((gid" << k << " * 0x9E3779B1u) >> 12) & (CS - 1u);\n";
-        o << "      uint32_t tg = t_tag[ch];\n      if (tg == 0u) { tg = atomicCAS(&t_tag[ch], 0u, gid" << k << " + 1u); if (tg == 0u) tg = gid" << k << " + 1u; }\n";
-        o << "      const bool cached = tg == gid" << k << " + 1u;\n";
-        o << "      if (cached) atomicAdd(&t_cnt[ch], 1u);\n";
-        if (s.need_count) o << "      else atomicAdd(&c.cnt[gid" << k << "], 1ull);\n";
-        else o << "      else c.cnt[gid" << k << "] = 1ull;\n";
-      } else if (s.lds_acc) {
-        if (s.need_count) o << "      atomicAdd(&l_cnt[" << gidk << "], 1u);\n";
-        else o << "      l_cnt[" << gidk << "] = 1u;\n";
-      } else {
-        o << "      atomicAdd(&c.cnt[gid" << k << "], 1ull);\n";
-      }
-      for (size_t j = 0; j < s.aggs.size(); j++) {
-        const JitAgg& A = s.aggs[j];
-        if (A.func == FDB_AGG_COUNT) continue;
+          const std::string v = "u" + std::to_string(j);
+          if (A.func == FDB_AGG_SUM && A.type == FDB_T_F64) {
+            o << "        double " << v << " = 0.0;\n";
+            for (int k = 0; k < 4; k++) o << "        if ((sel >> " << k << ") & 1u) " << v << " += __longlong_as_double((long long)" << raw_of(j, k) << ");\n";
+          } else if (A.func == FDB_AGG_SUM) {
+            o << "        unsigned long long " << v << " = 0ull;\n";
+            for (int k = 0; k < 4; k++) o << "        if ((sel >> " << k << ") & 1u) " << v << " += " << raw_of(j, k) << ";\n";
+          } else {
+            o << "        long long " << v << " = " << (A.func == FDB_AGG_MIN ? "0x7FFFFFFFFFFFFFFFLL" : "(-0x7FFFFFFFFFFFFFFFLL - 1)") << ";\n";
+            for (int k = 0; k < 4; k++) {
+              const std::string key = A.type == FDB_T_F64 ? ("f64_minmax_key(__longlong_as_double((long long)" + raw_of(j, k) + "), " + (A.func == FDB_AGG_MIN ? "true" : "false") + ")") : ("(long long)" + raw_of(j, k));
+              o << "        if ((sel >> " << k << ") & 1u) { const long long y = " << key << "; " << v << " = " << (A.func == FDB_AGG_MIN ? "y < " : "y > ") << v << " ? y : " << v << "; }\n";
+            }
+          }
+        }
+        o << "#pragma unroll\n        for (int sh = 32; sh > 0; sh >>= 1) {\n          u_cnt += (uint32_t)__shfl_xor((int)u_cnt, sh, 64);\n";
+        for (size_t j = 0; j < s.aggs.size(); j++) {
+          const JitAgg& A = s.aggs[j];
+          if (A.func == FDB_AGG_COUNT) continue;
+          const std::string v = "u" + std::to_string(j);
+          if (A.func == FDB_AGG_SUM && A.type == FDB_T_F64) o << "          " << v << " += __shfl_xor(" << v << ", sh, 64);\n";
+          else if (A.func == FDB_AGG_SUM) o << "          " << v << " += (unsigned long long)__shfl_xor((long long)" << v << ", sh, 64);\n";
+          else o << "          { const long long y = __shfl_xor(" << v << ", sh, 64); " << v << " = " << (A.func == FDB_AGG_MIN ? "y < " : "y > ") << v << " ? y : " << v << "; }\n";
+        }
+        o << "        }\n        if ((tid & 63u) == 0u) {\n";
+        if (s.need_count) o << "          atomicAdd(&l_cnt[g0], u_cnt);\n";
+        else o << "          l_cnt[g0] = 1u;\n";
+        for (size_t j = 0; j < s.aggs.size(); j++) {
+          const JitAgg& A = s.aggs[j];
+          if (A.func == FDB_AGG_COUNT) continue;
+          const std::string v = "u" + std::to_string(j);
+          const std::string acc = "(l_acc + (size_t)" + std::to_string(j) + " * n_slots + g0)";
+          if (A.func == FDB_AGG_SUM && A.type == FDB_T_F64) o << "          atomicAdd(reinterpret_cast<double*>" << acc << ", " << v << ");\n";
+          else if (A.func == FDB_AGG_SUM) o << "          atomicAdd(" << acc << ", " << v << ");\n";
+          else o << "          " << (A.func == FDB_AGG_MIN ? "atomicMin" : "atomicMax") << "(reinterpret_cast<long long*>" << acc << ", " << v << ");\n";
+        }
+        o << "        }\n        continue;\n      }\n    }\n";
+      }
+      for (int k = 0; k < 4 && s.reg_slots > 0; k++) {
         const std::string comp = std::string(k < 2 ? "a" : "b") + (k % 2 == 0 ? ".x" : ".y");
-        std::string raw;
-        if (A.expr != 0) {
-          auto col = [&](int ni) -> std::string { if (s.exprs[(size_t)ni].kind == 7) return "((PM" + std::to_string(s.exprs[(size_t)ni].slot) + " >> " + std::to_string(k) + ") & 1u)"; return reg(true, s.two_phase, s.exprs[(size_t)ni].slot) + comp; };
-          auto colvalid = [&](int ni) { return "((" + reg(true, s.two_phase, s.exprs[(size_t)ni].slot) + "_m >> " + std::to_string(k) + ") & 1u)"; };
-          raw = "(" + expr_valid(s.exprs, A.expr - 1, col, colvalid) + " ? " + expr_bits(s.exprs, A.expr - 1, expr_value(s.exprs, A.expr - 1, col, colvalid)) + " : 0ull)";
+        o << "    {\n      const bool on = (sel >> " << k << ") & 1u;\n";
+        std::vector<std::string> val(s.aggs.size());
+        for (size_t j = 0; j < s.aggs.size(); j++) {
+          const JitAgg& A = s.aggs[j];
+          if (A.func == FDB_AGG_COUNT) continue;
+          std::string raw;
+          if (A.expr != 0) {
+            auto col = [&](int ni) -> std::string { if (s.exprs[(size_t)ni].kind == 7) return "((PM" + std::to_string(s.exprs[(size_t)ni].slot) + " >> " + std::to_string(k) + ") & 1u)"; return reg(true, s.two_phase, s.exprs[(size_t)ni].slot) + comp; };
+            auto colvalid = [&](int ni) { return "((" + reg(true, s.two_phase, s.exprs[(size_t)ni].slot) + "_m >> " + std::to_string(k) + ") & 1u)"; };
+            raw = "(" + expr_valid(s.exprs, A.expr - 1, col, colvalid) + " ? " + expr_bits(s.exprs, A.expr - 1, expr_value(s.exprs, A.expr - 1, col, colvalid)) + " : 0ull)";
+          } else {
+            const std::string r = reg(true, s.two_phase, A.slot);
+            raw = "((" + r + "_m >> " + std::to_string(k) + ") & 1u ? " + r + comp + " : c.aggs[" + std::to_string(j) + "].null_value)";
+          }
+          const std::string v = "v" + std::to_string(j);
+          if (A.func == FDB_AGG_SUM && A.type == FDB_T_F64) o << "      const double " << v << " = __longlong_as_double((long long)" << raw << ");\n";
+          else if (A.func == FDB_AGG_SUM) o << "      const unsigned long long " << v << " = " << raw << ";\n";
+          else o << "      const long long " << v << " = " << (A.type == FDB_T_F64 ? ("f64_minmax_key(__longlong_as_double((long long)" + raw + "), " + (A.func == FDB_AGG_MIN ? "true" : "false") + ")") : ("(long long)" + raw)) << ";\n";
+          val[j] = v;
+        }
+        for (int t = 0; t < s.reg_slots; t++) {
+          const std::string m = s.reg_slots == 1 ? std::string("on") : ("(on && gid" + std::to_string(k) + " == " + std::to_string(t) + "u)");
+          o << "      R_cnt" << t << " += " << m << " ? 1ull : 0ull;\n";
+          for (size_t j = 0; j < s.aggs.size(); j++) {
+            const JitAgg& A = s.aggs[j];
+            if (A.func == FDB_AGG_COUNT) continue;
+            const std::string acc = "R_a" + std::to_string(j) + "_" + std::to_string(t);
+            if (A.func == FDB_AGG_SUM && A.type == FDB_T_F64) o << "      " << acc << " += " << m << " ? " << val[j] << " : 0.0;\n";
+            else if (A.func == FDB_AGG_SUM) o << "      " << acc << " += " << m << " ? " << val[j] << " : 0ull;\n";
+            else if (A.func == FDB_AGG_MIN) o << "      " << acc << " = (" << m << " && " << val[j] << " < " << acc << ") ? " << val[j] << " : " << acc << ";\n";
+            else o << "      " << acc << " = (" << m << " && " << val[j] << " > " << acc << ") ? " << val[j] << " : " << acc << ";\n";
+          }
+        }
+        o << "    }\n";
+      }
+      for (int k = 0; k < 4 && s.reg_slots == 0; k++) {
+        const std::string gidk = "gid" + std::to_string(k);
+        o << "    if ((sel >> " << k << ") & 1u) {\n";
+        if (s.cache) {
+          o << "      const uint32_t ch = ((gid" << k << " * 0x9E3779B1u) >> 12) & (CS - 1u);\n";
+          o << "      uint32_t tg = t_tag[ch];\n      if (tg == 0u) { tg = atomicCAS(&t_tag[ch], 0u, gid" << k << " + 1u); if (tg == 0u) tg = gid" << k << " + 1u; }\n";
+          o << "      const bool cached = tg == gid" << k << " + 1u;\n";
+          o << "      if (cached) atomicAdd(&t_cnt[ch], 1u);\n";
+          if (s.need_count) o << "      else atomicAdd(&c.cnt[gid" << k << "], 1ull);\n";
+          else o << "      else c.cnt[gid" << k << "] = 1ull;\n";
+        } else if (s.lds_acc) {
+          if (s.need_count) o << "      atomicAdd(&l_cnt[" << gidk << "], 1u);\n";
+          else o << "      l_cnt[" << gidk << "] = 1u;\n";
         } else {
-          const std::string r = reg(true, s.two_phase, A.slot);
-          raw = "((" + r + "_m >> " + std::to_string(k) + ") & 1u ? " + r + comp + " : c.aggs[" + std::to_string(j) + "].null_value)";
-        }
-        const std::string gacc = "(c.aggs[" + std::to_string(j) + "].acc + gid" + std::to_string(k) + ")";
-        const std::string acc = s.lds_acc ? ("(l_acc + (size_t)" + std::to_string(j) + " * n_slots + " + gidk + ")") : gacc;
-        auto emit = [&](const std::string& where, const char* ind) {
-          if (A.func == FDB_AGG_SUM) {
-            if (A.type == FDB_T_F64) o << ind << "atomicAdd(reinterpret_cast<double*>" << where << ", __longlong_as_double((long long)" << raw << "));\n";
-            else o << ind << "atomicAdd(" << where << ", " << raw << ");\n";
+          o << "      atomicAdd(&c.cnt[gid" << k << "], 1ull);\n";
+        }
+        for (size_t j = 0; j < s.aggs.size(); j++) {
+          const JitAgg& A = s.aggs[j];
+          if (A.func == FDB_AGG_COUNT) continue;
+          const std::string comp = std::string(k < 2 ? "a" : "b") + (k % 2 == 0 ? ".x" : ".y");
+          std::string raw;
+          if (A.expr != 0) {
+            auto col = [&](int ni) -> std::string { if (s.exprs[(size_t)ni].kind == 7) return "((PM" + std::to_string(s.exprs[(size_t)ni].slot) + " >> " + std::to_string(k) + ") & 1u)"; return reg(true, s.two_phase, s.exprs[(size_t)ni].slot) + comp; };
+            auto colvalid = [&](int ni) { return "((" + reg(true, s.two_phase, s.exprs[(size_t)ni].slot) + "_m >> " + std::to_string(k) + ") & 1u)"; };
+            raw = "(" + expr_valid(s.exprs, A.expr - 1, col, colvalid) + " ? " + expr_bits(s.exprs, A.expr - 1, expr_value(s.exprs, A.expr - 1, col, colvalid)) + " : 0ull)";
           } else {
-            const std::string key = A.type == FDB_T_F64 ? ("f64_minmax_key(__longlong_as_double((long long)" + raw + "), " + (A.func == FDB_AGG_MIN ? "true" : "false") + ")") : ("(long long)" + raw);
-            o << ind << (A.func == FDB_AGG_MIN ? "atomicMin" : "atomicMax") << "(reinterpret_cast<long long*>" << where << ", " << key << ");\n";
+            const std::string r = reg(true, s.two_phase, A.slot);
+            raw = "((" + r + "_m >> " + std::to_string(k) + ") & 1u ? " + r + comp + " : c.aggs[" + std::to_string(j) + "].null_value)";
           }
-        };
-        if (s.cache) {
-          o << "      if (cached) {\n";
-          emit("(t_acc + (size_t)" + std::to_string(j) + " * CS + ch)", "        ");
-          o << "      } else {\n";
-          emit(gacc, "        ");
-          o << "      }\n";
-        } else {
-          emit(acc, "      ");
-        }
-      }
-      o << "    }\n";
+          const std::string gacc = "(c.aggs[" + std::to_string(j) + "].acc + gid" + std::to_string(k) + ")";
+          const std::string acc = s.lds_acc ? ("(l_acc + (size_t)" + std::to_string(j) + " * n_slots + " + gidk + ")") : gacc;
+          auto emit = [&](const std::string& where, const char* ind) {
+            if (A.func == FDB_AGG_SUM) {
+              if (A.type == FDB_T_F64) o << ind << "atomicAdd(reinterpret_cast<double*>" << where << ", __longlong_as_double((long long)" << raw << "));\n";
+              else o << ind << "atomicAdd(" << where << ", " << raw << ");\n";
+            } else {
+              const std::string key = A.type == FDB_T_F64 ? ("f64_minmax_key(__longlong_as_double((long long)" + raw + "), " + (A.func == FDB_AGG_MIN ? "true" : "false") + ")") : ("(long long)" + raw);
+              o << ind << (A.func == FDB_AGG_MIN ? "atomicMin" : "atomicMax") << "(reinterpret_cast<long long*>" << where << ", " << key << ");\n";
+            }
+          };
+          if (s.cache) {
+            o << "      if (cached) {\n";
+            emit("(t_acc + (size_t)" + std::to_string(j) + " * CS + ch)", "        ");
+            o << "      } else {\n";
+            emit(gacc, "        ");
+            o << "      }\n";
+          } else {
+            emit(acc, "      ");
+          }
+        }
+        o << "    }\n";
+      }
+    };
+    if (!s.quad) {
+      o << "    const long long r0 = (tile - tile_begin) * " << BLK * 4 << "LL;\n";
+      o << "    const long long left = n_rows - r0 - (long long)tid * 4;\n    if (left <= 0) continue;\n";
+      o << "    const size_t tile_off4 = (size_t)r0 * 4, tile_off8 = (size_t)r0 * 8, tile_offb = (size_t)(r0 >> 3);\n";
+      o << "    const size_t tile_off1 = (size_t)r0, tile_off2 = (size_t)r0 * 2; (void)tile_off1; (void)tile_off2;\n";
+      o << "    const uint32_t live = left >= 4 ? 0xFu : ((1u << (int)left) - 1u);\n";
+      live_mask = true;
+      tile_body();
+    } else {
+      o << "    const long long wb = (tile - tile_begin) * " << BLK * 16 << "LL + (long long)wave * 1024;\n";
+      o << "    if (wb + 1024 <= n_rows) {\n";
+      full_block = true; live_mask = false;
+      block_loads();
+      o << "#pragma unroll\n      for (int u = 0; u < 4; u++) {\n";
+      o << "    const long long r0 = wb + 256 * u;\n";
+      o << "    const size_t tile_off4 = (size_t)r0 * 4, tile_off8 = (size_t)r0 * 8, tile_offb = (size_t)(r0 >> 3); (void)tile_off4; (void)tile_off8; (void)tile_offb;\n";
+      o << "    const size_t tile_off1 = (size_t)r0, tile_off2 = (size_t)r0 * 2; (void)tile_off1; (void)tile_off2;\n";
+      o << "    const uint32_t live = 0xFu;\n";
+      tile_body();
+      o << "      }\n    } else {\n";
+      full_block = false; live_mask = true;
+      o << "#pragma unroll 1\n      for (int u = 0; u < 4; u++) {\n";
+      o << "    const long long r0 = wb + 256 * u;\n";
+      o << "    const long long left = n_rows - r0 - (long long)lane * 4;\n    if (left <= 0) continue;\n";
+      o << "    const size_t tile_off4 = (size_t)r0 * 4, tile_off8 = (size_t)r0 * 8, tile_offb = (size_t)(r0 >> 3);\n";
+      o << "    const size_t tile_off1 = (size_t)r0, tile_off2 = (size_t)r0 * 2; (void)tile_off1; (void)tile_off2;\n";
+      o << "    const uint32_t live = left >= 4 ? 0xFu : ((1u << (int)left) - 1u);\n";
+      tile_body();
+      o << "      }\n    }\n";
     }
     o << "  }\n";
     if (s.reg_slots > 0) {
@@ -1427,7 +1523,7 @@
 
 std::string JitShape::key(bool with_validity) const {
   std::ostringstream k;
-  k << "b" << block << "l" << lds_acc << "c" << need_count << "t" << two_phase << "r" << reg_slots << "h" << cache << (wave_tables ? "w" : "") << (uniform_fold ? "u" : "") << "|";
+  k << "b" << block << "l" << lds_acc << "c" << need_count << "t" << two_phase << "r" << reg_slots << "h" << cache << (wave_tables ? "w" : "") << (uniform_fold ? "u" : "") << (quad ? "q" : "") << "|";
   auto slots = [&](const JitSlot* p, int n) { for (int i = 0; i < n; i++) { k << (p[i].has_values ? 'v' : '-') << (with_validity ? p[i].has_validity : 0); if (p[i].width != 4) k << 'w' << p[i].width; } k << '|'; };
   slots(c4, n_c4); slots(c8, n_c8); slots(l4, n_l4); slots(l8, n_l8);
   for (const JitLeaf& L : leaves) k << L.kind << ',' << L.slot << ',' << L.wide << ',' << (L.kind >= FDB_LEAF_CMP_I64 && L.kind <= FDB_LEAF_CMP_I64_F64 ? L.op : 0) << ',' << L.lut_in_lds << ';';
@@ -1458,6 +1554,8 @@
   slots(s.c4, a.c4, s.n_c4); slots(s.c8, a.c8, s.n_c8); slots(s.l4, a.l4, s.n_l4); slots(s.l8, a.l8, s.n_l8);
   for (int i = 0; i < s.n_c4; i++) s.c4[i].width = a.w4[i] == 1 || a.w4[i] == 2 ? a.w4[i] : 4;
   for (int i = 0; i < s.n_l4; i++) s.l4[i].width = a.wl4[i] == 1 || a.wl4[i] == 2 ? a.wl4[i] : 4;
+  for (int i = 0; i < s.n_c4; i++) s.quad |= s.c4[i].has_values && s.c4[i].width < 4;
+  for (int i = 0; i < s.n_l4; i++) s.quad |= s.l4[i].has_values && s.l4[i].width < 4;
   for (int l = 0; l < a.n_leaves; l++) {
     const FdbLeaf& L = a.leaves[l];
     s.leaves.push_back({L.kind, L.slot, L.wide, L.op, L.kind == FDB_LEAF_DICT_LUT && L.lut_lds != FDB_NO_LDS});
@@ -1741,7 +1839,8 @@
 hipFunction_t jit_select(JitShape shape, size_t lds_bytes, int row_bytes, int* block_out, int* blocks_per_cu_out) {
   int waves = row_bytes > 0 ? (65536 / (64 * 4)) / row_bytes : 16;
   waves = std::max(8, std::min(32, waves));
-  const int block = waves % 8 == 0 ? 512 : 256;
+  if (shape.quad) waves = std::max(8, std::min(16, row_bytes > 0 ? 144 / row_bytes : 12));
+  const int block = shape.quad ? 256 : waves % 8 == 0 ? 512 : 256;
   shape.block = block;
   hipFunction_t fn = jit_get(shape);
   if (fn == nullptr) return nullptr;
diff --git a/frostdb_amd/csrc/fdb_jit.h b/frostdb_amd/csrc/fdb_jit.h
--- a/frostdb_amd/csrc/fdb_jit.h
+++ b/frostdb_amd/csrc/fdb_jit.h
@@ -31,6 +31,7 @@
   bool cache = false;
   bool wave_tables = false;
   bool uniform_fold = true;
+  bool quad = false;
   int fuse4 = 0, fuse8 = 0;
   std::vector<int> proj_roots;
   std::string key(bool with_validity = true) const;
diff --git a/frostdb_amd/csrc/fdb_kernels.hip b/frostdb_amd/csrc/fdb_kernels.hip
--- a/frostdb_amd/csrc/fdb_kernels.hip
+++ b/frostdb_amd/csrc/fdb_kernels.hip
@@ -5,6 +5,7 @@
 #include <cstring>
 
 #include "fdb_kernels.h"
+#include "fdb_record.h"
 
 namespace {
 
@@ -2065,16 +2066,20 @@
   if (i >= n_vec) return;
   constexpr int PER = 16 / W;
   constexpr int NV = PER / 4;
+  constexpr int64_t VB = fdb::kScanCacheBlock * W / 16;
   const int64_t r0 = i * PER;
+  const bool interleaved = r0 + PER <= rows / fdb::kScanCacheBlock * fdb::kScanCacheBlock;
+  const int64_t s0 = interleaved ? (i / VB) * (fdb::kScanCacheBlock / 4) + ((i % VB) / 64) * (64 * NV) + (i % 64) : i * NV;
+  const int64_t sd = interleaved ? 64 : 1;
   uint32_t w[4] = {0u, 0u, 0u, 0u};
 #pragma unroll
   for (int k = 0; k < NV; k++) {
-    const u32x4 v = __builtin_nontemporal_load(as_global(src + i * NV + k));
+    const u32x4 v = __builtin_nontemporal_load(as_global(src + s0 + k * sd));
     const uint32_t e[4] = {v.x, v.y, v.z, v.w};
 #pragma unroll
     for (int q = 0; q < 4; q++) {
       const int r = k * 4 + q;
-      const uint32_t x = r0 + r < rows ? (e[q] & (W == 1 ? 0xFFu : 0xFFFFu)) : 0u;
+      const uint32_t x = interleaved || r0 + r < rows ? (e[q] & (W == 1 ? 0xFFu : 0xFFFFu)) : 0u;
       w[(r * W) / 4] |= x << (8 * ((r * W) % 4));
     }
   }
diff --git a/frostdb_amd/csrc/fdb_plan.cpp b/frostdb_amd/csrc/fdb_plan.cpp
--- a/frostdb_amd/csrc/fdb_plan.cpp
+++ b/frostdb_amd/csrc/fdb_plan.cpp
@@ -1438,6 +1438,7 @@
   std::vector<Narrowed> narrowed;
   hipFunction_t jit_fn = nullptr;
   int jit_block = sub == 1 ? 512 : sub == 2 ? 256 : sub == 3 ? 1024 : 0;
+  bool quad_unit = false;
   if (fixed_order) jit_block = 256;
   if (slots_ok) {
     for (int l : layouts) if (l == 2) two_phase = 1;
@@ -1517,6 +1518,7 @@
           for (int k = 0; k < shape.n_l8; k++) row_bytes += shape.l8[k].has_values ? 8 : 0;
           jit_fn = jit_select(shape, lds_bytes, row_bytes, &jit_block, &per_cu);
         }
+        quad_unit = shape.quad;
       }
     }
     if (jit_fn == nullptr) {
@@ -1535,7 +1537,7 @@
   pt.mark("kernel select");
   if (slots_ok) {
     if (jit_fn != nullptr) {
-      tile_rows_i = jit_block * 4;
+      tile_rows_i = jit_block * (quad_unit ? 16 : 4);
     } else {
       fdb_slot_geometry(two_phase, sub, lds_acc, lds_bytes, device_, &tile_rows_i, &per_cu);
     }
diff --git a/frostdb_amd/csrc/fdb_record.h b/frostdb_amd/csrc/fdb_record.h
--- a/frostdb_amd/csrc/fdb_record.h
+++ b/frostdb_amd/csrc/fdb_record.h
@@ -17,6 +17,18 @@
 inline size_t value_width(ColKind kind) { return kind == ColKind::DICT || kind == ColKind::STR ? 4 : 8; }
 inline size_t values_slot(size_t rows, size_t width) { return align_up(rows * width + kTailPad, 256); }
 inline size_t bitmap_slot(size_t rows) { return align_up((rows + 63) / 64 * 8 + kTailPad, 256); }
+
+#if defined(__HIPCC__)
+#define FDB_RECORD_HD __host__ __device__
+#else
+#define FDB_RECORD_HD
+#endif
+constexpr int64_t kScanCacheBlock = 1024;
+FDB_RECORD_HD inline int64_t scan_cache_position(int64_t i, int64_t rows, int width) {
+  if (i >= rows / kScanCacheBlock * kScanCacheBlock) return i;
+  const int64_t b = i / kScanCacheBlock, j = i % kScanCacheBlock, u = j / 256, l = (j % 256) / 4, r = j % 4;
+  return width == 1 ? kScanCacheBlock * b + 16 * l + 4 * u + r : kScanCacheBlock * b + 512 * (u / 2) + 8 * l + 4 * (u % 2) + r;
+}
 
 struct RecordLayout {
   struct Col { size_t val_off, bit_off; };
diff --git a/frostdb_amd/physicalplan.py b/frostdb_amd/physicalplan.py
--- a/frostdb_amd/physicalplan.py
+++ b/frostdb_amd/physicalplan.py
@@ -99,6 +99,7 @@
     L.fdb_plan_last_kernel.argtypes = [vp]
     L.fdb_arrow_roundtrip.argtypes = [vp, vp, vp, vp]
     L.fdb_selftest_widen.argtypes = [vp, i32, vp, i64]
+    L.fdb_selftest_scan_cache.argtypes = [vp, i64, i32, ctypes.c_int, vp, i64]
     L.fdb_plan_explain.argtypes = [vp, ctypes.c_char_p, i64, P(i64)]
     L.fdb_plan_last_kernel.restype = ctypes.c_char_p
     L.fdb_comm_unique_id.argtypes = [vp]
diff --git a/include/frostdb_amd.h b/include/frostdb_amd.h
--- a/include/frostdb_amd.h
+++ b/include/frostdb_amd.h
@@ -142,6 +142,7 @@
 FDB_API int fdb_arrow_roundtrip(struct ArrowArray* batch, struct ArrowSchema* schema, struct ArrowArray* out, struct ArrowSchema* out_schema);
 FDB_API int fdb_regex_match(const char* pattern, int64_t pattern_len, const uint8_t* value, int64_t value_len, int32_t* matched);
 FDB_API int fdb_selftest_widen(const void* src, int32_t width, uint32_t* dst, int64_t n);
+FDB_API int fdb_selftest_scan_cache(const uint32_t* indices, int64_t rows, int32_t width, int device, uint8_t* out, int64_t out_bytes);
 
 FDB_API int fdb_plan_create(const fdb_plan_desc* desc, int device, fdb_plan** out);
 FDB_API int fdb_plan_push(fdb_plan* plan, struct ArrowArray* batch, struct ArrowSchema* schema);
```
